# microsoft/M3P

Hardware: AMD Instinct MI355X
Metric: pre-train samples/sec (whole node), 12L/768d seq=128+36 (higher is better)
Workload: dtype bf16; 1 GPU; cfg2: 12L/768d/12h, 36 regions + 128 tokens, V=250002, 19 MLM targets/seq + ITM BCE, dropout 0.10, adam_inverse_sqrt + clip 5; per_gpu_batch=256, global_batch=256, seq_len=164, parallelism=dp1, prewarm_steps=36

## Files before the change

### include/m3p_hip.h

```cpp
#ifndef M3P_HIP_H
#define M3P_HIP_H

#include <stddef.h>
#include <stdint.h>

#ifdef __cplusplus
extern "C" {
#endif

#define M3P_API __attribute__((visibility("default")))

#define M3P_OK 0
#define M3P_EINVAL (-1)
#define M3P_ENOTIMPL (-2)
#define M3P_ENOMEM (-3)

M3P_API const char* m3p_version(void);


enum {
  M3P_EPI_NONE = 0,
  M3P_EPI_BIAS = 1,
  M3P_EPI_BIAS_GELU = 2,
  M3P_EPI_BIAS_DROP_RES = 3,
  M3P_EPI_RES = 4,
  M3P_EPI_DGELU = 5,
  M3P_EPI_MUL = 6,
  M3P_EPI_MULQ = 7,
  M3P_EPI_BIAS_GELUQ = 8,
  M3P_EPI_BIAS_LSE = 9
};

typedef struct M3PEpilogue {
  const float* bias;
  const void* aux;
  void* out2;
  float* colsum;
  int32_t ld_aux;
  int32_t ld_out2;
  int32_t scale_cols;
  float scale;
  float alpha;
  uint32_t seed;
  uint32_t thresh24;
  float inv_keep;
  const float* descale_a;
  const float* descale_b;
  void* out8;
  const float* scale8;
  float* amax8;
  int32_t ld_out8;
  int32_t out8_bf8;
  const int32_t* rng_rows;
  const void* row_ref;
} M3PEpilogue;

M3P_API int m3p_gemm_nt_bf16(const void* A, int lda, const void* W, int ldw, void* C, int ldc,
                             int M, int N, int K, int epilogue, const M3PEpilogue* ep, void* stream);

M3P_API int m3p_gemm_nt_fp8(const void* A8, int lda, int a_is_bf8, const void* W8, int ldw, void* C, int ldc,
                            int M, int N, int K, int epilogue, const M3PEpilogue* ep, void* stream);

M3P_API int m3p_quant_fp8(const void* src, int ld_src, void* dst, int ld_dst, int rows, int cols, const float* scale,
                          float* amax, int bf8, void* stream);

M3P_API int m3p_quant_fp8_batch(const long long* desc, int n_desc, int blocks_per_matrix, void* stream);

M3P_API int m3p_gemm_nt_streamk_f32(const void* A, int lda, const void* W, int ldw, float* C, int ldc,
                                    int M, int N, int K, float alpha, void* stream);
M3P_API int m3p_gemm_nn_streamk_f32(const void* A, int lda, const void* W, int ldw, int k_valid, float* C,
                                    int ldc, int M, int N, int K, float alpha, void* stream);
M3P_API int m3p_gemm_nn_w4_f32(const void* A, int lda, const void* W, int ldw, float* C, int ldc, int M, int N, int K, float alpha,
                               void* workspace, size_t workspace_bytes, void* stream);

M3P_API size_t m3p_gemm_wgrad_workspace_bytes(void);
M3P_API int m3p_gemm_wgrad_bf16(const void* dY, int lddy, const void* X, int ldx, float* dW, int lddw,
                                int M, int N, int K, float alpha, void* workspace, size_t workspace_bytes,
                                void* stream);
M3P_API int m3p_gemm_wgrad_store_bf16(const void* dY, int lddy, const void* X, int ldx, float* dW, int lddw, int M, int N, int K,
                                      float alpha, void* workspace, size_t workspace_bytes, void* stream);
M3P_API int m3p_gemm_wgrad_pair_bf16(const void* dYa, int lddya, const void* Xa, int ldxa, float* dWa, int lddwa, int Na, int Ka,
                                     const void* dYb, int lddyb, const void* Xb, int ldxb, float* dWb, int lddwb, int Nb, int Kb,
                                     int M, float alpha, void* workspace, size_t workspace_bytes, void* stream);


M3P_API int m3p_layernorm_fwd(const void* x, const float* gamma, const float* beta, const uint8_t* rowmask,
                              void* y, float* mean, float* rstd, int rows, int d, float eps, void* stream);

M3P_API int m3p_layernorm_bwd(const void* dy_a, const void* dy_b, const void* x, const float* gamma,
                              const float* mean, const float* rstd, const uint8_t* rowmask,
                              void* dx, void* dx_drop, float* dgamma, float* dbeta, float* dbias_drop,
                              int rows, int d, uint32_t seed, uint32_t thresh24, float inv_keep, void* stream);
M3P_API int m3p_layernorm_bwd_rows(const void* dy_a, const void* dy_b, const void* x, const float* gamma,
                                   const float* mean, const float* rstd, const uint8_t* rowmask,
                                   void* dx, void* dx_drop, float* dgamma, float* dbeta, float* dbias_drop,
                                   int rows, int d, uint32_t seed, uint32_t thresh24, float inv_keep,
                                   const int32_t* rng_rows, void* stream);


M3P_API int m3p_attn_fwd(const void* qkv, const int32_t* keylen, void* ctx, float* lse, uint64_t* keepmask,
                         int B, int S, int H, int dh, uint32_t seed, uint32_t thresh24, float inv_keep,
                         void* stream);

M3P_API int m3p_attn_bwd(const void* qkv, const int32_t* keylen, const void* ctx, const void* dctx,
                         const float* lse, const uint64_t* keepmask, void* dqkv, float* dbias_qkv, int B, int S,
                         int H, int dh, float qscale, uint32_t seed, uint32_t thresh24, float inv_keep,
                         void* stream);

M3P_API int m3p_attn_query_fwd(const void* q, int ld_q, const void* kv, long long kv_bstride, int ld_kv,
                               const int32_t* klen, void* ctx, int B, int Tq, int H, int dh, int Lk, int causal,
                               int pos0, void* stream);

M3P_API int m3p_attn_rows_fwd(const void* q, int ld_q, const void* kv, long long kv_bstride, int ld_kv, const int32_t* klen,
                              void* ctx, float* lse, int B, int Tq, int H, int dh, int Lk, int causal, int pos0,
                              uint32_t seed, uint32_t thresh24, float inv_keep, void* stream);
M3P_API int m3p_attn_rows_bwd(const void* q, int ld_q, const void* kv, long long kv_bstride, int ld_kv, const int32_t* klen,
                              const void* dctx, const float* lse, void* dq, int ld_dq, float* dkv, int B, int Tq, int H,
                              int dh, int Lk, int causal, int pos0, float qscale, uint32_t seed, uint32_t thresh24,
                              float inv_keep, void* stream);

M3P_API int m3p_attn_causal_fwd(const void* qkv, int ld_qkv, void* ctx, float* lse, int B, int T, int H, int dh,
                                uint32_t seed, uint32_t thresh24, float inv_keep, void* stream);
M3P_API int m3p_attn_causal_bwd(const void* qkv, int ld_qkv, const void* dctx, const float* lse, void* dqkv, int ld_dqkv,
                                int B, int T, int H, int dh, float qscale, uint32_t seed, uint32_t thresh24,
                                float inv_keep, void* stream);


M3P_API int m3p_cast_f32_bf16(const float* src, void* dst, long long n, void* stream);

M3P_API int m3p_embed_assemble_fwd(const int64_t* tok, const void* emb_bf16, const float* pos,
                                   const void* img_proj, const float* loc, const float* w_loc,
                                   const float* b_loc, const float* g_img, const float* be_img,
                                   const float* g_emb, const float* be_emb, const int32_t* totlen,
                                   void* h, void* z, float* mean_emb, float* rstd_emb, void* e,
                                   float* mean_img, float* rstd_img, int B, int T, int R, int d,
                                   uint32_t seed_img, uint32_t seed_emb, uint32_t thresh24, float inv_keep,
                                   const void* img_rows, void* stream);

M3P_API int m3p_embed_image_rows_fwd(const void* img_proj, const float* loc, const float* w_loc, const float* b_loc,
                                     const float* g_img, const float* be_img, void* e, float* mean_img,
                                     float* rstd_img, void* img_rows, int B, int R, int d, uint32_t seed_img,
                                     uint32_t thresh24, float inv_keep, void* stream);

M3P_API int m3p_embed_assemble_bwd(const void* dh, const void* z, const float* mean_emb, const float* rstd_emb,
                                   const float* g_emb, const void* e, const float* mean_img,
                                   const float* rstd_img, const float* g_img, const int64_t* tok,
                                   const int32_t* totlen, const float* loc, void* dz_scratch, void* de,
                                   float* d_g_emb, float* d_be_emb, float* d_pos, float* d_emb,
                                   void* d_tok_rows, float* d_g_img, float* d_be_img, float* d_b_img, float* d_b_loc,
                                   float* d_w_loc, int B, int T, int R, int d, int pad_index,
                                   uint32_t seed_img, uint32_t seed_emb, uint32_t thresh24, float inv_keep,
                                   int phase, void* stream);


M3P_API int m3p_gather_rows(const void* src, const int32_t* idx, void* dst, int n, int d, void* stream);
M3P_API int m3p_place_rows(const void* src, const int32_t* inv, void* dst, int rows, int d, int n, uint32_t fill_bits,
                           void* stream);
M3P_API int m3p_scatter_add_rows(const void* src, const int32_t* idx, void* dst, int n, int d, void* stream);
M3P_API int m3p_scatter_add_token_rows(const void* rows, int ld_rows, const int64_t* ids, float* dst, int n, int d,
                                       int pad_index, void* stream);

M3P_API int m3p_itm_score_fwd(const void* pre, const float* w2, const float* b2, float* pooled, float* scores, int B,
                              int d, void* stream);
M3P_API int m3p_itm_score_bwd(const float* dscores, const float* pooled, const float* w2, void* dpre16, void* dpreT16,
                              int ldt, float* db1, float* dw2, float* db2, int B, int d, void* stream);

M3P_API int m3p_ce_fwd_bwd(void* logits, int ld, int n_rows, int V, const int64_t* target, float* row_loss,
                           float* loss_sum, float loss_scale, float grad_scale, void* stream);

M3P_API int m3p_ce_lse_from_blocks(const void* stats, int n_blocks, int n_rows, const void* logits, int ld, const int64_t* target,
                                   float* row_loss, float* row_lse, void* scratch, void* stream);
M3P_API int m3p_ce_bwd_colsum(void* logits, int ld, int n_rows, int V, const int64_t* target, const float* row_lse,
                              float grad_scale, float* colsum, void* workspace, size_t workspace_bytes, void* stream);
M3P_API size_t m3p_ce_colsum_workspace_bytes(int ld, int n_rows);
M3P_API int m3p_ce_fwd_bwd_colsum(void* logits, int ld, int n_rows, int V, const int64_t* target, float* row_loss,
                                  float* row_lse, float grad_scale, float* colsum, void* workspace,
                                  size_t workspace_bytes, void* stream);

M3P_API int m3p_ce_shift_target(const void* h, const void* emb, const float* bias, const int64_t* target, float* row_t, void* row_ref,
                                int n_rows, int d, void* stream);
M3P_API int m3p_ce_shift_rows(const void* stats, int n_blocks, int n_rows, float grad_scale, float* row_loss, float* row_s,
                              float* row_q, void* scratch, void* stream);
M3P_API int m3p_ce_shift_colsum(const void* e, int ld, int n_rows, const float* row_s, float* colsum, void* workspace,
                                size_t workspace_bytes, void* stream);
M3P_API int m3p_ce_shift_scale_rows(const void* h, const float* row_s, const float* g, void* out, int n_rows, int d, void* stream);
M3P_API int m3p_ce_shift_target_rows(const void* h, const int64_t* target, const float* row_q, const float* g, float* demb, float* dbias,
                                     int n_rows, int d, void* stream);
M3P_API int m3p_ce_shift_dh(const float* dh32, const void* emb, const int64_t* target, const float* row_s, const float* row_q,
                            const float* g, void* dh, int n_rows, int d, void* stream);

M3P_API int m3p_ce_eval(const void* logits, int ld, int n_rows, int V, const int64_t* target, float* row_loss,
                        int32_t* row_argmax, void* stream);

M3P_API int m3p_colsum_bf16(const void* x, int ld, int n, int ncols, float* out, const float* scale_ptr,
                            void* stream);


M3P_API int m3p_sumsq_f32(const float* g, long long n, double* out, void* stream);

M3P_API int m3p_sumsq_ranges_f32(const float* base, const long long* starts, const long long* counts, int n_ranges, double* out,
                                 void* stream);

M3P_API int m3p_adam_step(float* p, float* g, float* m, float* v, void* w16, long long n, float lr, float beta1,
                          float beta2, float eps, float weight_decay, float step_size, const double* gnorm_sq,
                          float max_norm, float grad_scale, int zero_grad, void* stream);
M3P_API int m3p_adam_step_ranges(float* p, float* g, float* m, float* v, void* w16, const long long* starts,
                                 const long long* counts, const float* step_sizes, const int* zero_grad, int n_ranges,
                                 float lr, float beta1, float beta2, float eps, float weight_decay, const double* gnorm_sq,
                                 float max_norm, float grad_scale, void* stream);

M3P_API int m3p_gelu_fwd(const void* u, void* h, void* dh, long long n, void* stream);
M3P_API int m3p_gelu_fwd_gq(const void* u, void* h, void* gq, int M, int N, void* stream);
M3P_API int m3p_gelu_fwd_q8(const void* u, void* h, void* h8, long long n, const float* scale, float* amax, void* stream);

M3P_API int m3p_gelu_bwd(const void* dy, const void* u, void* du, long long n, void* stream);

M3P_API int m3p_mse_fwd_bwd(const void* pred, int ld_pred, const float* tgt, int ld_tgt, void* dpred, float* row_sq,
                            int rows, int cols, float grad_scale, void* stream);


M3P_API int m3p_dropout_rows(const void* x, int ldx, const void* res, int ldres, void* y, int ldy, int rows, int cols,
                             uint32_t rng_ld, uint32_t rng_col0, uint32_t seed, uint32_t thresh24, float inv_keep,
                             void* stream);

M3P_API int m3p_glu_fwd(const void* ab, int ld_ab, void* y, int rows, int d, void* stream);
M3P_API int m3p_glu_bwd(const void* ab, int ld_ab, const void* dy, void* dab, int rows, int d, void* stream);

M3P_API int m3p_transpose_batch_bf16(const long long* desc, int n_desc, int max_tiles, void* stream);

M3P_API int m3p_transpose_bf16(const void* src, void* dst, int rows, int cols, int ld_src, int ld_dst,
                               void* stream);

M3P_API int m3p_set_persistent_grid(int workgroups);
M3P_API int m3p_set_tile_queue(int32_t* counters, int n_slots);

enum {
  M3P_KERN_NT_SKINNY = 1,
  M3P_KERN_NT_W8 = 2,
  M3P_KERN_NT_W8_QUEUE = 3,
  M3P_KERN_NT_W4 = 4,
  M3P_KERN_NT_RING = 5,
  M3P_KERN_NT_128 = 6,
  M3P_KERN_WGRAD_W4_CHUNKS = 10,
  M3P_KERN_WGRAD_W4_TILES = 11,
  M3P_KERN_WGRAD_RING = 12,
  M3P_KERN_WGRAD_128 = 13
};
M3P_API int m3p_gemm_nt_plan(int M, int N, int K, int epilogue);
M3P_API int m3p_gemm_wgrad_plan(int M, int N, int K);

M3P_API void m3p_debug_set_variant(int v);
M3P_API void m3p_debug_attn_variant(int v);

M3P_API int m3p_seq_masks(const int64_t* lengths, const int64_t* lengths_b, int B, int S, int32_t* totlen,
                          uint8_t* rowmask, void* stream);
M3P_API int m3p_mask_to_rows(const uint8_t* mask, int n_mask, int inner, long long s0, long long s1, long long soff,
                             int d, int32_t* rows, int n_rows, void* stream);
M3P_API int m3p_cast_rows_f32_bf16(const float* in, long long s0, long long s1, int n0, int n1, int cols, void* out,
                                   void* stream);
M3P_API int m3p_scale_bf16_dev(const void* in, int in_is_f32, const float* g, void* out, long long n, void* stream);
M3P_API int m3p_axpy_dev_f32(float* dst, const float* src, const float* g, long long n, void* stream);
M3P_API int m3p_itm_loss_fwd_bwd(const float* scores, const int64_t* pos, int n_groups, int sample_n, float w_ce,
                                 float w_bce, float* loss, float* dscores, void* stream);

M3P_API int m3p_probe_mfma_16x16x32(const void* a_rowmajor_16x32, const void* b_colmajor_32x16,
                                    float* d_16x16, int* d_rowcol, void* stream);
M3P_API int m3p_probe_mfma_fp8_16x16x128(const void* a_16x128, const void* w_16x128, float* d_16x16, int a_is_bf8,
                                         void* stream);
M3P_API int m3p_probe_tr16(const void* tile_bf16_64x16, void* out_64x4, void* stream);
M3P_API int m3p_probe_permlane16_swap(void* out_2x64_u32, void* stream);

#ifdef __cplusplus
}
#endif
#endif
```

### m3p_amd/csrc/attention.hip

```cpp
#include "common.hpp"


namespace {

constexpr int ATTN_BWD_NW = 4;
constexpr int ATTN_BWD_WPS = 3;

static int g_attn_variant = 0;

template <int DH> struct AttnCfg {
  static constexpr int ROWB = DH * 2;
  static constexpr int CH = DH / 8;
  static constexpr int RPI = 1024 / ROWB;
  static constexpr int KK = DH / 32;
  static constexpr int NT = DH / 16;
  static __device__ __forceinline__ int swz(int chunk, int row) { return DH == 64 ? (chunk ^ (row & 7)) : chunk; }
};

__device__ __forceinline__ bf16x4 lds_tr16(const char* p) {
  s16x4 v = __builtin_amdgcn_ds_read_tr16_b64_v4i16((__attribute__((address_space(3))) s16x4*)(p));
  return __builtin_bit_cast(bf16x4, v);
}
__device__ __forceinline__ float row16_sum(float v) {
#define M3P_DPP_ADD(ctrl) v += __builtin_bit_cast(float, __builtin_amdgcn_update_dpp(0, __builtin_bit_cast(int, v), ctrl, 0xf, 0xf, true))
  M3P_DPP_ADD(0xB1);
  M3P_DPP_ADD(0x4E);
  M3P_DPP_ADD(0x124);
  M3P_DPP_ADD(0x128);
#undef M3P_DPP_ADD
  return v;
}
__device__ __forceinline__ uint32_t bit_to_mask(uint32_t bits, int r) {
  uint32_t o;
  switch (r) {
    case 0: asm("v_bfe_i32 %0, %1, 0, 1" : "=v"(o) : "v"(bits)); break;
    case 1: asm("v_bfe_i32 %0, %1, 1, 1" : "=v"(o) : "v"(bits)); break;
    case 2: asm("v_bfe_i32 %0, %1, 2, 1" : "=v"(o) : "v"(bits)); break;
    default: asm("v_bfe_i32 %0, %1, 3, 1" : "=v"(o) : "v"(bits)); break;
  }
  return o;
}
template <int CH>
__device__ __forceinline__ float chunks_sum(float v) {
#define M3P_DPP_ADD(ctrl) v += __builtin_bit_cast(float, __builtin_amdgcn_update_dpp(0, __builtin_bit_cast(int, v), ctrl, 0xf, 0xf, true))
  M3P_DPP_ADD(0xB1);
  M3P_DPP_ADD(0x4E);
  if (CH == 8) M3P_DPP_ADD(0x141);
#undef M3P_DPP_ADD
  return v;
}
__device__ __forceinline__ bf16x8 cat8(bf16x4 a, bf16x4 b) {
  return bf16x8{a[0], a[1], a[2], a[3], b[0], b[1], b[2], b[3]};
}

typedef unsigned int u32x2_t __attribute__((ext_vector_type(2)));
typedef unsigned int u32x4_t __attribute__((ext_vector_type(4)));
template <int NT>
__device__ __forceinline__ void store_row_widened(bf16* row, int fg, bool ok, const bf16x4 (&r)[NT]) {
  static_assert(NT % 2 == 0, "d-tiles are swapped in pairs");
  bf16* p = row + 8 * (fg >> 1) + 16 * (fg & 1);
#pragma unroll
  for (int n0 = 0; n0 < NT; n0 += 2) {
    u32x2_t x = __builtin_bit_cast(u32x2_t, r[n0]), y = __builtin_bit_cast(u32x2_t, r[n0 + 1]);
    asm volatile("s_nop 1\n\tv_permlane16_swap_b32 %0, %2\n\tv_permlane16_swap_b32 %1, %3"
                 : "+v"(x[0]), "+v"(x[1]), "+v"(y[0]), "+v"(y[1]));
    if (ok) *reinterpret_cast<u32x4_t*>(p + 16 * n0) = u32x4_t{x[0], x[1], y[0], y[1]};
  }
}

template <int DH>
__device__ __forceinline__ void stage_rows(const bf16* __restrict__ g, size_t ld, int S, int nrows, char* lds,
                                           int wid, int lane, int nwaves = 4) {
  using Cf = AttnCfg<DH>;
  const int rin = lane / Cf::CH, c = lane % Cf::CH;
  const int ninstr = (nrows + Cf::RPI - 1) / Cf::RPI;
  for (int i = wid; i < ninstr; i += nwaves) {
    const int row = i * Cf::RPI + rin;
    const int gr = min(row, S - 1);
    const int gc = Cf::swz(c, row);
    __builtin_amdgcn_global_load_lds(GLB_PTR(g + (size_t)gr * ld + gc * 8), LDS_PTR(lds + i * 1024), 16, 0, 0);
  }
}

template <int DH>
__device__ __forceinline__ void stage_rows_hidden(const bf16* __restrict__ g, size_t ld, int S, int nrows, char* lds,
                                                  int wid, int lane, int nwaves) {
  using Cf = AttnCfg<DH>;
  const int rin = lane / Cf::CH, c = lane % Cf::CH;
  const int ninstr = (nrows + Cf::RPI - 1) / Cf::RPI;
  const uint32_t lds0 = (uint32_t)(uintptr_t)(__attribute__((address_space(3))) char*)lds;
  for (int i = wid; i < ninstr; i += nwaves) {
    const int row = i * Cf::RPI + rin;
    const int gr = min(row, S - 1);
    const int gc = Cf::swz(c, row);
    const bf16* src = g + (size_t)gr * ld + gc * 8;
    const uint32_t dst = __builtin_amdgcn_readfirstlane(lds0 + (uint32_t)i * 1024u);
    asm volatile("s_mov_b32 m0, %1\n\ts_nop 0\n\tglobal_load_lds_dwordx4 %0, off" :: "v"(src), "s"(dst) : "memory", "m0");
  }
}

template <int DH, int KT, bool DROP, int NTC, int NW = 4, bool EVENS = false>
__global__ __launch_bounds__(NW * 64, NW == 8 ? 2 : 3)
void attn_fwd_kernel(const bf16* __restrict__ qkv, const int* __restrict__ keylen, bf16* __restrict__ ctx,
                     float* __restrict__ lse, unsigned long long* __restrict__ keepmask, int S, int H, int dmodel,
                     uint32_t seed, uint32_t thresh24, float inv_keep) {
  using Cf = AttnCfg<DH>;
  extern __shared__ __attribute__((aligned(16))) char smem[];
  const int tid = threadIdx.x, lane = tid & 63;
  const int wid = __builtin_amdgcn_readfirstlane(tid >> 6);
  const int b = blockIdx.x / H, h = blockIdx.x - b * H;
  const int nt = NTC ? NTC : (S + 15) >> 4;
  const int nk = (nt + 1) >> 1;
  const size_t ld = 3 * (size_t)dmodel;
  const bf16* Qg = qkv + (size_t)b * S * ld + h * DH;
  const bf16* Kg = Qg + dmodel;
  const bf16* Vg = Qg + 2 * dmodel;
  char* sK = smem;
  char* sV = smem + nt * 16 * Cf::ROWB;
  stage_rows<DH>(Kg, ld, S, nt * 16, sK, wid, lane, NW);
  stage_rows<DH>(Vg, ld, S, nk * 32, sV, wid, lane, NW);
  const int fq = lane & 15, fg = lane >> 4;
  const int wrot = (wid + (blockIdx.x >> 3)) & (NW - 1);
  bf16x8 qnext[Cf::KK];
  {
    const int qc0 = min(wrot * 16 + fq, S - 1);
#pragma unroll
    for (int kk = 0; kk < Cf::KK; ++kk)
      qnext[kk] = *reinterpret_cast<const bf16x8*>(Qg + (size_t)qc0 * ld + 32 * kk + 8 * fg);
  }
  const int klen = keylen[b];
  __syncthreads();

  int k_off[Cf::KK];
#pragma unroll
  for (int kk = 0; kk < Cf::KK; ++kk) k_off[kk] = fq * Cf::ROWB + Cf::swz(4 * kk + fg, fq) * 16;
  const int vrow = 4 * fg + (fq >> 2);
  int v_off[Cf::NT];
#pragma unroll
  for (int n = 0; n < Cf::NT; ++n)
    v_off[n] = vrow * Cf::ROWB + Cf::swz(2 * n + ((fq & 3) >> 1), vrow) * 16 + 8 * (fq & 1);

  for (int qb = wrot; qb < nt; qb += NW) {
    const int q = qb * 16 + fq;
    const int qc = min(q, S - 1);
    bf16x8 qf[Cf::KK];
#pragma unroll
    for (int kk = 0; kk < Cf::KK; ++kk) qf[kk] = qnext[kk];
    {
      const int qcn = min(q + 16 * NW, S - 1);
#pragma unroll
      for (int kk = 0; kk < Cf::KK; ++kk)
        qnext[kk] = *reinterpret_cast<const bf16x8*>(Qg + (size_t)qcn * ld + 32 * kk + 8 * fg);
    }

    f32x4 s[2 * KT];
#pragma unroll
    for (int t = 0; t < 2 * KT; ++t) s[t] = f32x4{0.f, 0.f, 0.f, 0.f};
#pragma unroll
    for (int kk = 0; kk < Cf::KK; ++kk) {
#pragma unroll
      for (int t = 0; t < 2 * KT; ++t)
        if (t < nt) {
          const bf16x8 kf = *reinterpret_cast<const bf16x8*>(sK + t * 16 * Cf::ROWB + k_off[kk]);
          s[t] = __builtin_amdgcn_mfma_f32_16x16x32_bf16(kf, qf[kk], s[t], 0, 0, 0);
        }
    }
    constexpr float kLog2e = 1.4426950408889634f;
    float mx = -INFINITY;
    int klen_it = klen;
    asm volatile("" : "+s"(klen_it));
#pragma unroll
    for (int t = 0; t < 2 * KT; ++t)
      if (t < nt) {
        if (16 * t + 16 > klen_it) {
#pragma unroll
          for (int r = 0; r < 4; ++r) s[t][r] = (16 * t + 4 * fg + r < klen_it) ? s[t][r] : -INFINITY;
        }
#pragma unroll
        for (int r = 0; r < 4; ++r) mx = fmaxf(mx, s[t][r]);
      }
    mx = fmaxf(mx, __shfl_xor(mx, 16, 64));
    mx = fmaxf(mx, __shfl_xor(mx, 32, 64));
    const float mx2 = mx * kLog2e;
    float sum = 0.f;
#pragma unroll
    for (int t = 0; t < 2 * KT; ++t)
      if (t < nt) {
#pragma unroll
        for (int r = 0; r < 4; ++r) {
          const float p = __builtin_amdgcn_exp2f(__builtin_fmaf(s[t][r], kLog2e, -mx2));
          s[t][r] = p;
          sum += p;
        }
      }
    sum += __shfl_xor(sum, 16, 64);
    sum += __shfl_xor(sum, 32, 64);
    const float inv = 1.0f / sum;
    const uint32_t rbase = (uint32_t)((b * H + h) * S + qc) * (uint32_t)S;
    const uint32_t thr16 = thresh24 >> 8;
    const bool even_rows = EVENS || (S & 1) == 0;
    unsigned long long* mrow = keepmask ? keepmask + ((size_t)(b * H + h) * nt + qb) * nt * 4 : nullptr;
    constexpr int MW = (8 * KT + 63) / 64;
    uint32_t mlo[MW], mhi[MW];
#pragma unroll
    for (int g = 0; g < MW; ++g) mlo[g] = mhi[g] = 0u;
    bf16x8 pf[KT];
#pragma unroll
    for (int kk = 0; kk < KT; ++kk) {
      float p[8];
      const float invk = DROP ? inv * inv_keep : inv;
      bool kq[8] = {true, true, true, true, true, true, true, true};
      if (DROP) {
#pragma unroll
        for (int hf = 0; hf < 2; ++hf) {
          const int t = 2 * kk + hf;
          if (t < nt) {
            const uint32_t base = rbase + (uint32_t)(16 * t + 4 * fg);
            bool k4[4];
            if (even_rows) {
              asm volatile("" ::: "memory");
              const uint32_t h0 = m3p_hash32(base >> 1, seed), h1 = m3p_hash32((base >> 1) + 1u, seed);
              k4[0] = (h0 & 0xFFFFu) >= thr16; k4[1] = (h0 >> 16) >= thr16;
              k4[2] = (h1 & 0xFFFFu) >= thr16; k4[3] = (h1 >> 16) >= thr16;
            } else {
              asm volatile("" ::: "memory");
              m3p_keep_run<4>(base, seed, thresh24, k4);
            }
#pragma unroll
            for (int r = 0; r < 4; ++r) kq[4 * hf + r] = k4[r];
          }
        }
      }
#pragma unroll
      for (int hf = 0; hf < 2; ++hf) {
        const int t = 2 * kk + hf;
        unsigned long long kw[4] = {0ull, 0ull, 0ull, 0ull};
#pragma unroll
        for (int r = 0; r < 4; ++r) {
          const int j = 4 * hf + r;
          float v = 0.f;
          if (t < nt) {
            v = s[t][r] * invk;
            if (DROP) {
              const bool keep = kq[j];
              kw[r] = __builtin_amdgcn_ballot_w64(keep);
              v = keep ? v : 0.f;
            }
          }
          p[j] = v;
        }
        if (DROP && t < nt) {
          asm("s_nop 3\n\tv_writelane_b32 %0, %2, %10\n\tv_writelane_b32 %1, %3, %10\n\tv_writelane_b32 %0, %4, %11\n\tv_writelane_b32 %1, %5, %11\n\t"
              "v_writelane_b32 %0, %6, %12\n\tv_writelane_b32 %1, %7, %12\n\tv_writelane_b32 %0, %8, %13\n\tv_writelane_b32 %1, %9, %13"
              : "+v"(mlo[(4 * t) >> 6]), "+v"(mhi[(4 * t) >> 6])
              : "s"((uint32_t)kw[0]), "s"((uint32_t)(kw[0] >> 32)), "s"((uint32_t)kw[1]), "s"((uint32_t)(kw[1] >> 32)),
                "s"((uint32_t)kw[2]), "s"((uint32_t)(kw[2] >> 32)), "s"((uint32_t)kw[3]), "s"((uint32_t)(kw[3] >> 32)),
                "i"((4 * t) & 63), "i"((4 * t + 1) & 63), "i"((4 * t + 2) & 63), "i"((4 * t + 3) & 63));
        }
      }
      pf[kk] = bf16x8{(bf16)p[0], (bf16)p[1], (bf16)p[2], (bf16)p[3], (bf16)p[4], (bf16)p[5], (bf16)p[6], (bf16)p[7]};
    }
    if (DROP && mrow) {
#pragma unroll
      for (int g = 0; g < MW; ++g)
        if (64 * g + lane < 4 * nt) mrow[64 * g + lane] = ((unsigned long long)mhi[g] << 32) | mlo[g];
    }
    f32x4 o[Cf::NT];
#pragma unroll
    for (int n = 0; n < Cf::NT; ++n) o[n] = f32x4{0.f, 0.f, 0.f, 0.f};
#pragma unroll
    for (int kk = 0; kk < KT; ++kk) {
      if (kk < nk) {
#pragma unroll
        for (int n = 0; n < Cf::NT; ++n) {
          const char* pv = sV + kk * 32 * Cf::ROWB + v_off[n];
          const bf16x8 vf = cat8(lds_tr16(pv), lds_tr16(pv + 16 * Cf::ROWB));
          o[n] = __builtin_amdgcn_mfma_f32_16x16x32_bf16(vf, pf[kk], o[n], 0, 0, 0);
        }
      }
    }
    {
      bf16x4 ob[Cf::NT];
#pragma unroll
      for (int n = 0; n < Cf::NT; ++n) ob[n] = bf16x4{(bf16)o[n][0], (bf16)o[n][1], (bf16)o[n][2], (bf16)o[n][3]};
      store_row_widened<Cf::NT>(ctx + (size_t)(b * S + min(q, S - 1)) * dmodel + h * DH, fg, q < S, ob);
      if (q < S && fg == 0) lse[(size_t)(b * H + h) * S + q] = mx + __logf(sum);
    }
  }
}

template <int DH, int KT, bool DROP, bool MASK, int NKC, int NTC, int NW = 4, int KB = 1, int KBQ = KB, bool ONEPASS = false>
__global__ __launch_bounds__(NW * 64, NTC == 11 ? ATTN_BWD_WPS : ((NW == 8 || KB == 2) ? 2 : 3))
void attn_bwd_kernel(const bf16* __restrict__ qkv, const int* __restrict__ keylen, const bf16* __restrict__ ctx,
                     const bf16* __restrict__ dctx, const float* __restrict__ lse,
                     const unsigned long long* __restrict__ keepmask, bf16* __restrict__ dqkv,
                     float* __restrict__ dbias_qkv, int S, int H, int dmodel, float qscale, uint32_t seed,
                     uint32_t thresh24, float inv_keep) {
  using Cf = AttnCfg<DH>;
  extern __shared__ __attribute__((aligned(16))) char smem[];
  const int tid = threadIdx.x, lane = tid & 63;
  const int wid = __builtin_amdgcn_readfirstlane(tid >> 6);
  const int b = blockIdx.x / H, h = blockIdx.x - b * H;
  const int wrot = (NW & (NW - 1)) ? wid : ((wid + (blockIdx.x >> 3)) & (NW - 1));
  const int nt = NTC ? NTC : ((S + 15) >> 4);
  const int nk = NKC ? NKC : ((S + 31) >> 5);
  const size_t ld = 3 * (size_t)dmodel;
  const int b_rd = b;
  const bf16* Qg = qkv + (size_t)b_rd * S * ld + h * DH;
  const bf16* Kg = Qg + dmodel;
  const bf16* Vg = Qg + 2 * dmodel;
  const bf16* Og = ctx + (size_t)b_rd * S * dmodel + h * DH;
  const bf16* dOg = dctx + (size_t)b_rd * S * dmodel + h * DH;
  bf16* dQg = dqkv + (size_t)b * S * ld + h * DH;
  bf16* dKg = dQg + dmodel;
  bf16* dVg = dQg + 2 * dmodel;
  const float* lse_bh = lse + (size_t)(b * H + h) * S;
  const int klen = keylen[b];
  const unsigned long long* mbh = MASK ? keepmask + (size_t)(b * H + h) * nt * nt * 4 : nullptr;

  const int tile_bytes = nk * 32 * Cf::ROWB;
  char* s0 = smem;
  char* s1 = smem + tile_bytes;
  float* sL = reinterpret_cast<float*>(smem + 2 * tile_bytes);
  float* sD = sL + nk * 32;
  const int fq = lane & 15, fg = lane >> 4;
  float* sB = sD + nk * 32;
  float* sBw = sB + wid * 3 * DH;
  constexpr int DSP = NTC * 32;
  char* sK = reinterpret_cast<char*>(sB + NW * 3 * DH);
  char* sDS = sK + tile_bytes;
  static_assert(!ONEPASS || (NKC == 6 && NTC == 11 && KB == 1 && DH == 64), "ONEPASS is the M3P-sequence instantiation");
  f32x4 bsum[Cf::NT];
#pragma unroll
  for (int n = 0; n < Cf::NT; ++n) bsum[n] = f32x4{0.f, 0.f, 0.f, 0.f};
  auto bias_acc = [&](int, int n, const bf16x4& v4) {
    bsum[n] += f32x4{(float)v4[0], (float)v4[1], (float)v4[2], (float)v4[3]};
  };
  auto bias_flush = [&](int part) {
#pragma unroll
    for (int n = 0; n < Cf::NT; ++n) {
      f32x4 x = bsum[n];
#pragma unroll
      for (int r = 0; r < 4; ++r) x[r] = row16_sum(x[r]);
      if (fq == 0) *reinterpret_cast<f32x4*>(sBw + part * DH + 16 * n + 4 * fg) = x;
      bsum[n] = f32x4{0.f, 0.f, 0.f, 0.f};
    }
  };

  int r_off[Cf::KK];
#pragma unroll
  for (int kk = 0; kk < Cf::KK; ++kk) r_off[kk] = fq * Cf::ROWB + Cf::swz(4 * kk + fg, fq) * 16;
  const int trow = 4 * fg + (fq >> 2);
  int t_off[Cf::NT];
#pragma unroll
  for (int n = 0; n < Cf::NT; ++n)
    t_off[n] = trow * Cf::ROWB + Cf::swz(2 * n + ((fq & 3) >> 1), trow) * 16 + 8 * (fq & 1);

#define PAD_TILE(t) (NTC ? (t) >= NTC : (!MASK && (t) >= nt))
  constexpr float kLog2e = 1.4426950408889634f;
  constexpr float kMasked = -1.0e30f;
  constexpr bool kDfromLds = NKC != 0;
  constexpr int kStageInstr = NKC * 32 / Cf::RPI;
  constexpr int kNIW = kDfromLds ? (kStageInstr + NW - 1) / NW : 1;
  bf16x8 orow[kNIW];
  if (kDfromLds) {
    const int rin = lane / Cf::CH, c = lane % Cf::CH;
#pragma unroll
    for (int j = 0; j < kNIW; ++j) {
      const int row = (wid + j * NW) * Cf::RPI + rin;
      orow[j] = *reinterpret_cast<const bf16x8*>(Og + (size_t)min(row, S - 1) * dmodel + Cf::swz(c, row) * 8);
    }
  }
  stage_rows<DH>(Qg, ld, S, nk * 32, s0, wid, lane, NW);
  stage_rows<DH>(dOg, (size_t)dmodel, S, nk * 32, s1, wid, lane, NW);
  if (ONEPASS) stage_rows<DH>(Kg, ld, S, nk * 32, sK, wid, lane, NW);
  bf16x8 kf[KB][Cf::KK], vf[KB][Cf::KK];
  auto load_kv = [&](int u, int kb) {
    const int keyc = min(kb * 16 + fq, S - 1);
#pragma unroll
    for (int kk = 0; kk < Cf::KK; ++kk) {
      kf[u][kk] = *reinterpret_cast<const bf16x8*>(Kg + (size_t)keyc * ld + 32 * kk + 8 * fg);
      vf[u][kk] = *reinterpret_cast<const bf16x8*>(Vg + (size_t)keyc * ld + 32 * kk + 8 * fg);
    }
  };
  constexpr bool kNextFrag = NKC != 0 && NTC != 0 && !(DROP && !MASK);
  bf16x8 kfn[KB][Cf::KK], vfn[KB][Cf::KK];
  auto load_kv_next = [&](int u, int kb) {
    const int keyc = min(kb * 16 + fq, S - 1);
#pragma unroll
    for (int kk = 0; kk < Cf::KK; ++kk) {
      kfn[u][kk] = *reinterpret_cast<const bf16x8*>(Kg + (size_t)keyc * ld + 32 * kk + 8 * fg);
      vfn[u][kk] = *reinterpret_cast<const bf16x8*>(Vg + (size_t)keyc * ld + 32 * kk + 8 * fg);
    }
  };
  if (wrot * KB < nt) {
#pragma unroll
    for (int u = 0; u < KB; ++u) load_kv(u, wrot * KB + u);
  }
  const float log2_inv_keep = DROP ? __builtin_amdgcn_logf(inv_keep) : 0.f;
  const float keep_prob = DROP ? __builtin_amdgcn_rcpf(inv_keep) : 1.f;
  for (int q = tid; q < nk * 32; q += NW * 64) {
    float dsum = 0.f, l = INFINITY;
    if (q < S) {
      if (!kDfromLds) {
        const bf16* op = Og + (size_t)q * dmodel;
        const bf16* dp = dOg + (size_t)q * dmodel;
#pragma unroll
        for (int c = 0; c < DH / 8; ++c) {
          const bf16x8 ov = *reinterpret_cast<const bf16x8*>(op + 8 * c);
          const bf16x8 dv = *reinterpret_cast<const bf16x8*>(dp + 8 * c);
#pragma unroll
          for (int e = 0; e < 8; ++e) dsum += (float)ov[e] * (float)dv[e];
        }
      }
      l = lse_bh[q] * kLog2e - log2_inv_keep;
    }
    if (!kDfromLds) sD[q] = dsum * keep_prob;
    sL[q] = l;
  }
  if (kDfromLds) {
    asm volatile("s_waitcnt vmcnt(0)" ::: "memory");
    const int rin = lane / Cf::CH, c = lane % Cf::CH;
#pragma unroll
    for (int j = 0; j < kNIW; ++j) {
      const int i = wid + j * NW;
      if (i < kStageInstr) {
        const bf16x8 dv = *reinterpret_cast<const bf16x8*>(s1 + i * 1024 + lane * 16);
        float part = 0.f;
#pragma unroll
        for (int e = 0; e < 8; ++e) part += (float)orow[j][e] * (float)dv[e];
        part = chunks_sum<Cf::CH>(part);
        const int row = i * Cf::RPI + rin;
        if (c == 0) sD[row] = row < S ? part * keep_prob : 0.f;
      }
    }
  }
  __syncthreads();

  constexpr bool kPreA = MASK && NKC != 0;
// ... 489 lines not shown
  for (;;) {
    const int b = hd / H, h = hd - b * H;
    bf16* dQg = dqkv + (size_t)b * S * ld + h * DH;
    const bf16* Kg = qkv + (size_t)b * S * ld + h * DH + dmodel;
    const int klen = keylen[b];
    float* sBh = sB + par * (NW * 3 * DH);
    __builtin_amdgcn_s_waitcnt(0x0F70);
    asm volatile("s_waitcnt vmcnt(0)" ::: "memory");
#pragma unroll
    for (int j = 0; j < kNIW; ++j) {
      const int i = wid + j * NW;
      if (i < kStageInstr) {
        const bf16x8 dvv = *reinterpret_cast<const bf16x8*>(s1 + i * 1024 + lane * 16);
        float part = 0.f;
#pragma unroll
        for (int e = 0; e < 8; ++e) part += (float)orow[j][e] * (float)dvv[e];
        part = chunks_sum<Cf::CH>(part);
        const int row = i * Cf::RPI + rin;
        if (c8 == 0) sD[row] = row < S ? part * keep_prob : 0.f;
      }
    }
    if (tid < NR) sL[tid] = tid < S ? lse_r * kLog2e - log2_inv_keep : INFINITY;
    if (MASK && lane < 4 * NTC) sMW[lane] = mw_req;
    asm volatile("s_waitcnt lgkmcnt(0)" ::: "memory");
    __builtin_amdgcn_s_barrier();
    asm volatile("" ::: "memory");
    if (prev_h >= 0 && dbias_qkv) bias_reduce(sB + (par ^ 1) * (NW * 3 * DH), prev_h);
    if (prev_h >= 0) store_head(dQg_prev);
    dQg_prev = dQg;
    stage_rows_hidden<DH>(Kg, ld, S, NR, sK, wid, lane, NW);
    if (wid < NTC) {
      const float kbias = (key < klen) ? 0.f : kMasked;
      f32x4 dv[Cf::NT], dk[Cf::NT];
#pragma unroll
      for (int n = 0; n < Cf::NT; ++n) dv[n] = dk[n] = f32x4{0.f, 0.f, 0.f, 0.f};
#pragma unroll
      for (int kq = 0; kq < NKC; ++kq) {
        f32x4 scA[2], dpA[2], dnegA[2];
#pragma unroll
        for (int hf = 0; hf < 2; ++hf) {
          const int t = 2 * kq + hf;
          dnegA[hf] = f32x4{-sD[16 * t + 4 * fg + 0], -sD[16 * t + 4 * fg + 1], -sD[16 * t + 4 * fg + 2], -sD[16 * t + 4 * fg + 3]};
          scA[hf] = f32x4{kbias, kbias, kbias, kbias};
          dpA[hf] = DROP ? f32x4{0.f, 0.f, 0.f, 0.f} : dnegA[hf];
        }
#pragma unroll
        for (int kk = 0; kk < Cf::KK; ++kk) {
#pragma unroll
          for (int hf = 0; hf < 2; ++hf) {
            const int t = 2 * kq + hf;
            if (PAD_TILE(t)) continue;
            const bf16x8 qf = *reinterpret_cast<const bf16x8*>(s0 + t * 16 * Cf::ROWB + r_off[kk]);
            const bf16x8 df = *reinterpret_cast<const bf16x8*>(s1 + t * 16 * Cf::ROWB + r_off[kk]);
            scA[hf] = __builtin_amdgcn_mfma_f32_16x16x32_bf16(qf, kf[kk], scA[hf], 0, 0, 0);
            dpA[hf] = __builtin_amdgcn_mfma_f32_16x16x32_bf16(df, vf[kk], dpA[hf], 0, 0, 0);
          }
        }
        f32x4 pd2[2], ds2[2];
#pragma unroll
        for (int hf = 0; hf < 2; ++hf) {
          const int t = 2 * kq + hf;
          if (PAD_TILE(t)) {
            pd2[hf] = ds2[hf] = f32x4{0.f, 0.f, 0.f, 0.f};
            continue;
          }
          uint32_t kbits = 0;
          if (MASK) kbits = (uint32_t)(sMW[4 * t + (fq & 3)] >> (4 * fg + 16 * (fq >> 2)));
#pragma unroll
          for (int r = 0; r < 4; ++r) {
            const int q = 16 * t + 4 * fg + r;
            const float p = __builtin_amdgcn_exp2f(__builtin_fmaf(scA[hf][r], kLog2e, -sL[q]));
            if (DROP) {
              const float pd = __builtin_bit_cast(float, __builtin_bit_cast(uint32_t, p) & bit_to_mask(kbits, r));
              pd2[hf][r] = pd;
              ds2[hf][r] = __builtin_fmaf(pd, dpA[hf][r], p * dnegA[hf][r]);
            } else {
              pd2[hf][r] = p;
              ds2[hf][r] = p * dpA[hf][r];
            }
          }
        }
        const bf16x8 pfrag = bf16x8{(bf16)pd2[0][0], (bf16)pd2[0][1], (bf16)pd2[0][2], (bf16)pd2[0][3],
                                    (bf16)pd2[1][0], (bf16)pd2[1][1], (bf16)pd2[1][2], (bf16)pd2[1][3]};
        const bf16x8 sfrag = bf16x8{(bf16)ds2[0][0], (bf16)ds2[0][1], (bf16)ds2[0][2], (bf16)ds2[0][3],
                                    (bf16)ds2[1][0], (bf16)ds2[1][1], (bf16)ds2[1][2], (bf16)ds2[1][3]};
#pragma unroll
        for (int hf = 0; hf < 2; ++hf) {
          if (PAD_TILE(2 * kq + hf)) continue;
          *reinterpret_cast<bf16x4*>(sDS + key * DSP + (32 * kq + 16 * hf + 4 * fg) * 2) =
              hf ? bf16x4{sfrag[4], sfrag[5], sfrag[6], sfrag[7]} : bf16x4{sfrag[0], sfrag[1], sfrag[2], sfrag[3]};
        }
#pragma unroll
        for (int n = 0; n < Cf::NT; ++n) {
          const char* pq = s0 + kq * 32 * Cf::ROWB + t_off[n];
          const char* pdo = s1 + kq * 32 * Cf::ROWB + t_off[n];
          const bf16x8 qT = cat8(lds_tr16(pq), lds_tr16(pq + 16 * Cf::ROWB));
          const bf16x8 dT = cat8(lds_tr16(pdo), lds_tr16(pdo + 16 * Cf::ROWB));
          dv[n] = __builtin_amdgcn_mfma_f32_16x16x32_bf16(dT, pfrag, dv[n], 0, 0, 0);
          dk[n] = __builtin_amdgcn_mfma_f32_16x16x32_bf16(qT, sfrag, dk[n], 0, 0, 0);
        }
        __builtin_amdgcn_sched_barrier(0);
      }
#pragma unroll
      for (int n = 0; n < Cf::NT; ++n) {
        kb4[n] = bf16x4{(bf16)dk[n][0], (bf16)dk[n][1], (bf16)dk[n][2], (bf16)dk[n][3]};
        vb4[n] = bf16x4{(bf16)dv[n][0], (bf16)dv[n][1], (bf16)dv[n][2], (bf16)dv[n][3]};
        if (dbias_qkv) bias_acc(n, key < S ? vb4[n] : bf16x4{0, 0, 0, 0});
      }
    }
    if (dbias_qkv) bias_flush(sBh + wid * 3 * DH, 2);
    __builtin_amdgcn_s_waitcnt(0);
    asm volatile("s_waitcnt vmcnt(0) lgkmcnt(0)" ::: "memory");
    __builtin_amdgcn_s_barrier();
    asm volatile("" ::: "memory");
    const int next = hd + gridDim.x;
    if (next < nheads) request_head(next);
    if (wid < NTC) {
      f32x4 dq[Cf::NT];
#pragma unroll
      for (int n = 0; n < Cf::NT; ++n) dq[n] = f32x4{0.f, 0.f, 0.f, 0.f};
      const char* pds = sDS + trow * DSP + wid * 32 + (fq & 3) * 8;
#pragma unroll
      for (int kq = 0; kq < NKC; ++kq) {
        const bf16x4 lo = lds_tr16(pds + (32 * kq) * DSP);
        const bf16x4 hi = PAD_TILE(2 * kq + 1) ? bf16x4{0, 0, 0, 0} : lds_tr16(pds + (32 * kq + 16) * DSP);
        const bf16x8 sfr = cat8(lo, hi);
#pragma unroll
        for (int n = 0; n < Cf::NT; ++n) {
          const char* pk = sK + kq * 32 * Cf::ROWB + t_off[n];
          const bf16x8 kT = cat8(lds_tr16(pk), lds_tr16(pk + 16 * Cf::ROWB));
          dq[n] = __builtin_amdgcn_mfma_f32_16x16x32_bf16(kT, sfr, dq[n], 0, 0, 0);
        }
      }
#pragma unroll
      for (int n = 0; n < Cf::NT; ++n) {
        qb4[n] = bf16x4{(bf16)(dq[n][0] * qscale), (bf16)(dq[n][1] * qscale), (bf16)(dq[n][2] * qscale), (bf16)(dq[n][3] * qscale)};
        if (dbias_qkv) bias_acc(n, key < S ? qb4[n] : bf16x4{0, 0, 0, 0});
      }
    }
    if (dbias_qkv) bias_flush(sBh + wid * 3 * DH, 0);
    prev_h = h;
    par ^= 1;
    if (next >= nheads) break;
    hd = next;
  }
  store_head(dQg_prev);
  if (dbias_qkv) {
    __syncthreads();
    bias_reduce(sB + (par ^ 1) * (NW * 3 * DH), prev_h);
  }
#undef PAD_TILE
}

template <int DH>
int launch_fwd(const bf16* qkv, const int* keylen, bf16* ctx, float* lse, unsigned long long* keepmask, int B, int S, int H,
               int dmodel, uint32_t seed, uint32_t thresh24, float inv_keep, hipStream_t st) {
  const int nt = (S + 15) / 16, nk = (S + 31) / 32;
  const size_t lds = (size_t)(nt * 16 + nk * 32) * DH * 2;
  const bool wide = 2 * lds > 160 * 1024;
#define M3P_ATTN_FWD(KT)                                                                                        \
  do {                                                                                                          \
    constexpr int NW0 = (KT == 16) ? 8 : 4;    \
    auto kern = thresh24 ? attn_fwd_kernel<DH, KT, true, 0, NW0> : attn_fwd_kernel<DH, KT, false, 0, NW0>;       \
    if (nt == 11 && KT == 6) kern = thresh24 ? ((S & 1) ? attn_fwd_kernel<DH, 6, true, 11> : attn_fwd_kernel<DH, 6, true, 11, 4, true>) \
                                             : attn_fwd_kernel<DH, 6, false, 11>; \
    if (wide) kern = thresh24 ? attn_fwd_kernel<DH, KT, true, 0, 8> : attn_fwd_kernel<DH, KT, false, 0, 8>;       \
    hipError_t e = hipFuncSetAttribute((const void*)kern, hipFuncAttributeMaxDynamicSharedMemorySize, (int)lds); \
    if (e != hipSuccess) return (int)e;                                                                         \
    hipLaunchKernelGGL(kern, dim3(B* H), dim3((wide || NW0 == 8) ? 512 : 256), lds, st, qkv, keylen, ctx, lse, keepmask, S, H, dmodel, seed, \
                       thresh24, inv_keep);                                                                     \
  } while (0)
  if (nk <= 6) M3P_ATTN_FWD(6);
  else if (nk <= 12) M3P_ATTN_FWD(12);
  else if (nk <= 16) M3P_ATTN_FWD(16);
  else return M3P_EINVAL;
#undef M3P_ATTN_FWD
  M3P_CHECK_LAUNCH();
  return M3P_OK;
}

template <int DH>
int launch_bwd(const bf16* qkv, const int* keylen, const bf16* ctx, const bf16* dctx, const float* lse,
               const unsigned long long* keepmask, bf16* dqkv, float* dbias, int B, int S, int H, int dmodel, float qscale,
               uint32_t seed, uint32_t thresh24, float inv_keep, hipStream_t st) {
  const int nk = (S + 31) / 32;
  const bool wide = (size_t)2 * ((size_t)2 * nk * 32 * DH * 2) > 160 * 1024;
  const bool m3p_seq = nk == 6 && (S + 15) / 16 == 11;
  const bool onepass = m3p_seq && DH == 64 && (!thresh24 || keepmask) && !(g_attn_variant & 1);
  const int nwaves = wide ? 8 : (onepass ? 12 : (m3p_seq ? ATTN_BWD_NW : 4));
  const size_t lds = (size_t)2 * nk * 32 * DH * 2 + (size_t)2 * nk * 32 * sizeof(float) + 3 * nwaves * DH * sizeof(float) +
                     (onepass ? (size_t)nk * 32 * DH * 2 + (size_t)11 * 16 * 11 * 32 : 0);
#define M3P_ATTN_BWD(KT, DROP, MASK)                                                                            \
  do {                                                                                                          \
    auto kern = attn_bwd_kernel<DH, KT, DROP, MASK, 0, 0>;                                                      \
    if (wide) kern = attn_bwd_kernel<DH, KT, DROP, MASK, 0, 0, 8>;                                              \
    if (nk == 6) kern = attn_bwd_kernel<DH, KT, DROP, MASK, 6, 0>;                                              \
    if (m3p_seq) kern = attn_bwd_kernel<DH, KT, DROP, MASK, 6, 11, ATTN_BWD_NW, 1, 1>;                                \
    if constexpr (DH == 64 && (MASK || !DROP)) { if (onepass) kern = attn_bwd_kernel<DH, KT, DROP, MASK, 6, 11, 12, 1, 1, true>; } \
    hipError_t e = hipFuncSetAttribute((const void*)kern, hipFuncAttributeMaxDynamicSharedMemorySize, (int)lds); \
    if (e != hipSuccess) return (int)e;                                                                         \
    hipLaunchKernelGGL(kern, dim3(B* H), dim3(nwaves * 64), lds, st, qkv, keylen, ctx, dctx, lse, keepmask, dqkv, dbias, S, H, \
                       dmodel, qscale, seed, thresh24, inv_keep);                                               \
  } while (0)
  if (nk > 16) return M3P_EINVAL;
  if constexpr (DH == 64) {
    if (onepass && !(g_attn_variant & 2)) {
      int dev = 0, n_cu = 0;
      if (hipGetDevice(&dev) != hipSuccess || hipDeviceGetAttribute(&n_cu, hipDeviceAttributeMultiprocessorCount, dev) != hipSuccess || n_cu <= 0)
        n_cu = 256;
      const size_t ldsp = (size_t)3 * 192 * 128 + (size_t)11 * 16 * 11 * 32 + 2 * 192 * sizeof(float) + 2 * 12 * 3 * 64 * sizeof(float) + 12 * 48 * 8;
      auto kp = thresh24 ? attn_bwd_p_kernel<true, true> : attn_bwd_p_kernel<false, false>;
      if (hipFuncSetAttribute((const void*)kp, hipFuncAttributeMaxDynamicSharedMemorySize, (int)ldsp) == hipSuccess) {
        const int nheads = B * H;
        hipLaunchKernelGGL(kp, dim3(nheads < n_cu ? nheads : n_cu), dim3(768), ldsp, st, qkv, keylen, ctx, dctx, lse, keepmask, dqkv, dbias,
                           S, H, dmodel, nheads, qscale, inv_keep);
        M3P_CHECK_LAUNCH();
        return M3P_OK;
      }
      (void)hipGetLastError();
    }
  }
  if (!thresh24) M3P_ATTN_BWD(16, false, false);
  else M3P_ATTN_BWD(16, true, true);
#undef M3P_ATTN_BWD
  M3P_CHECK_LAUNCH();
  return M3P_OK;
}

}

extern "C" {

void m3p_debug_attn_variant(int v) { g_attn_variant = v; }

int m3p_attn_fwd(const void* qkv, const int32_t* keylen, void* ctx, float* lse, uint64_t* keepmask, int B, int S, int H, int dh,
                 uint32_t seed, uint32_t thresh24, float inv_keep, void* stream) {
  if (B <= 0 || S <= 0 || H <= 0 || S > 512) return M3P_EINVAL;
  if (((uintptr_t)qkv & 15) || ((uintptr_t)ctx & 7)) return M3P_EINVAL;
  const int dmodel = H * dh;
  hipStream_t st = (hipStream_t)stream;
  if (dh == 64) return launch_fwd<64>((const bf16*)qkv, keylen, (bf16*)ctx, lse, (unsigned long long*)keepmask, B, S, H, dmodel, seed, thresh24, inv_keep, st);
  if (dh == 32) return launch_fwd<32>((const bf16*)qkv, keylen, (bf16*)ctx, lse, (unsigned long long*)keepmask, B, S, H, dmodel, seed, thresh24, inv_keep, st);
  return M3P_EINVAL;
}

int m3p_attn_bwd(const void* qkv, const int32_t* keylen, const void* ctx, const void* dctx, const float* lse,
                 const uint64_t* keepmask, void* dqkv, float* dbias_qkv, int B, int S, int H, int dh, float qscale,
                 uint32_t seed, uint32_t thresh24, float inv_keep, void* stream) {
  if (B <= 0 || S <= 0 || H <= 0 || S > 512) return M3P_EINVAL;
  if (thresh24 && !keepmask) return M3P_EINVAL;
  if (((uintptr_t)qkv & 15) || ((uintptr_t)ctx & 15) || ((uintptr_t)dctx & 15) || ((uintptr_t)dqkv & 7)) return M3P_EINVAL;
  const int dmodel = H * dh;
  hipStream_t st = (hipStream_t)stream;
  if (dh == 64)
    return launch_bwd<64>((const bf16*)qkv, keylen, (const bf16*)ctx, (const bf16*)dctx, lse, (const unsigned long long*)keepmask, (bf16*)dqkv, dbias_qkv, B, S, H,
                          dmodel, qscale, seed, thresh24, inv_keep, st);
  if (dh == 32)
    return launch_bwd<32>((const bf16*)qkv, keylen, (const bf16*)ctx, (const bf16*)dctx, lse, (const unsigned long long*)keepmask, (bf16*)dqkv, dbias_qkv, B, S, H,
                          dmodel, qscale, seed, thresh24, inv_keep, st);
  return M3P_EINVAL;
}

}
```

### m3p_amd/csrc/heads.hip

```cpp
#include "common.hpp"
#include <hip/amd_detail/amd_hip_unsafe_atomics.h>

namespace {

__global__ __launch_bounds__(256) void gather_rows_kernel(const bf16* __restrict__ src, const int32_t* __restrict__ idx,
                                                          bf16* __restrict__ dst, int n, int d) {
  const int nchunk = d >> 2;
  const size_t total = (size_t)n * nchunk;
  for (size_t i = (size_t)blockIdx.x * blockDim.x + threadIdx.x; i < total; i += (size_t)gridDim.x * blockDim.x) {
    const int r = (int)(i / nchunk), c = (int)(i - (size_t)r * nchunk);
    *reinterpret_cast<bf16x4*>(dst + (size_t)r * d + 4 * c) =
        *reinterpret_cast<const bf16x4*>(src + (size_t)idx[r] * d + 4 * c);
  }
}
__global__ __launch_bounds__(256) void place_rows_kernel(const bf16* __restrict__ src, const int32_t* __restrict__ inv,
                                                         bf16* __restrict__ dst, int rows, int d, int n, uint32_t fill2) {
  typedef unsigned int u32x4 __attribute__((ext_vector_type(4)));
  const int nchunk = d >> 3;
  const size_t total = (size_t)rows * nchunk;
  const u32x4 fv = u32x4{fill2, fill2, fill2, fill2};
  for (size_t i = (size_t)blockIdx.x * blockDim.x + threadIdx.x; i < total; i += (size_t)gridDim.x * blockDim.x) {
    const int r = (int)(i / nchunk), c = (int)(i - (size_t)r * nchunk);
    const int j = inv[r];
    u32x4 v = fv;
    if (j >= 0 && j < n) v = *reinterpret_cast<const u32x4*>(src + (size_t)j * d + 8 * c);
    *reinterpret_cast<u32x4*>(dst + (size_t)r * d + 8 * c) = v;
  }
}
__global__ __launch_bounds__(256) void scatter_add_rows_kernel(const bf16* __restrict__ src, const int32_t* __restrict__ idx,
                                                               bf16* __restrict__ dst, int n, int d) {
  const int nchunk = d >> 2;
  const size_t total = (size_t)n * nchunk;
  for (size_t i = (size_t)blockIdx.x * blockDim.x + threadIdx.x; i < total; i += (size_t)gridDim.x * blockDim.x) {
    const int r = (int)(i / nchunk), c = (int)(i - (size_t)r * nchunk);
    bf16* p = dst + (size_t)idx[r] * d + 4 * c;
    Vec4<bf16>::store(p, Vec4<bf16>::load(p) + Vec4<bf16>::load(src + (size_t)r * d + 4 * c));
  }
}

__global__ __launch_bounds__(256) void scatter_add_token_rows_kernel(const bf16* __restrict__ rows, int ld_rows, const int64_t* __restrict__ ids,
                                                                     float* __restrict__ dst, int n, int d, int pad_index) {
  const int lane = threadIdx.x & 63;
  const int wave = (int)((blockIdx.x * blockDim.x + threadIdx.x) >> 6), nwave = (int)((gridDim.x * blockDim.x) >> 6);
  for (int r = wave; r < n; r += nwave) {
    const int64_t id = ids[r];
    if (id == pad_index) continue;
    const bf16* src = rows + (size_t)r * ld_rows;
    float* out = dst + (size_t)id * d;
    for (int e = lane; e < d; e += 64) {
      const float v = (float)src[e];
      if (v != 0.f) unsafeAtomicAdd(out + e, v);
    }
  }
}

__global__ __launch_bounds__(1024) void ce_fwd_bwd_kernel(bf16* __restrict__ logits, int ld, int V,
                                                          const int64_t* __restrict__ target, float* __restrict__ row_loss,
                                                          float* __restrict__ loss_sum, float loss_scale, float gscale) {
  __shared__ float s_m[16], s_s[16];
  constexpr float kLog2e = 1.4426950408889634f;
  const int row = blockIdx.x, tid = threadIdx.x, lane = tid & 63, wib = tid >> 6;
  bf16* lr = logits + (size_t)row * ld;
  const int nchunk = ld >> 3;
  float m = -INFINITY, s = 0.f;
  for (int c = tid; c < nchunk; c += 1024) {
    const bf16x8 v = *reinterpret_cast<const bf16x8*>(lr + 8 * c);
    float x[8];
    float gm = -INFINITY;
#pragma unroll
    for (int j = 0; j < 8; ++j) {
      x[j] = (8 * c + j < V) ? (float)v[j] : -INFINITY;
      gm = fmaxf(gm, x[j]);
    }
    if (gm > m) {
      s *= __builtin_amdgcn_exp2f((m - gm) * kLog2e);
      m = gm;
    }
    const float mb = m * kLog2e;
#pragma unroll
    for (int j = 0; j < 8; ++j) s += __builtin_amdgcn_exp2f(__builtin_fmaf(x[j], kLog2e, -mb));
  }
#pragma unroll
  for (int o = 32; o > 0; o >>= 1) {
    const float m2 = __shfl_xor(m, o, 64), s2 = __shfl_xor(s, o, 64);
    const float mm = fmaxf(m, m2);
    s = (m == -INFINITY ? 0.f : s * __expf(m - mm)) + (m2 == -INFINITY ? 0.f : s2 * __expf(m2 - mm));
    m = mm;
  }
  if (lane == 0) { s_m[wib] = m; s_s[wib] = s; }
  __syncthreads();
  float M = -INFINITY;
#pragma unroll
  for (int w = 0; w < 16; ++w) M = fmaxf(M, s_m[w]);
  float Ssum = 0.f;
#pragma unroll
  for (int w = 0; w < 16; ++w) Ssum += (s_m[w] == -INFINITY) ? 0.f : s_s[w] * __expf(s_m[w] - M);
  const float lse = M + __logf(Ssum);
  const int64_t tgt = target[row];
  if (tid == 0) {
    const float l = lse - (float)lr[tgt];
    row_loss[row] = l;
    if (loss_sum) unsafeAtomicAdd(loss_sum, l * loss_scale);
  }
  __syncthreads();
  const float lb = lse * kLog2e;
  for (int c = tid; c < nchunk; c += 1024) {
    const bf16x8 v = *reinterpret_cast<const bf16x8*>(lr + 8 * c);
    bf16x8 g;
#pragma unroll
    for (int j = 0; j < 8; ++j) {
      const int col = 8 * c + j;
      float p = (col < V) ? __builtin_amdgcn_exp2f(__builtin_fmaf((float)v[j], kLog2e, -lb)) : 0.f;
      if (col == tgt) p -= 1.f;
      g[j] = (bf16)(p * gscale);
    }
    *reinterpret_cast<bf16x8*>(lr + 8 * c) = g;
  }
}

__global__ __launch_bounds__(1024) void ce_stats_kernel(const bf16* __restrict__ logits, int ld, int V, const int64_t* __restrict__ target,
                                                        float* __restrict__ row_loss, float* __restrict__ row_lse) {
  __shared__ float s_m[16], s_s[16];
  constexpr float kLog2e = 1.4426950408889634f;
  const int row = blockIdx.x, tid = threadIdx.x, lane = tid & 63, wib = tid >> 6;
  const bf16* lr = logits + (size_t)row * ld;
  const int nchunk = ld >> 3;
  float m = -INFINITY, s = 0.f;
  for (int c = tid; c < nchunk; c += 1024) {
    const bf16x8 v = *reinterpret_cast<const bf16x8*>(lr + 8 * c);
    float x[8];
    float gm = -INFINITY;
#pragma unroll
    for (int j = 0; j < 8; ++j) {
      x[j] = (8 * c + j < V) ? (float)v[j] : -INFINITY;
      gm = fmaxf(gm, x[j]);
    }
    if (gm > m) {
      s *= __builtin_amdgcn_exp2f((m - gm) * kLog2e);
      m = gm;
    }
    const float mb = m * kLog2e;
#pragma unroll
    for (int j = 0; j < 8; ++j) s += __builtin_amdgcn_exp2f(__builtin_fmaf(x[j], kLog2e, -mb));
  }
#pragma unroll
  for (int o = 32; o > 0; o >>= 1) {
    const float m2 = __shfl_xor(m, o, 64), s2 = __shfl_xor(s, o, 64);
    const float mm = fmaxf(m, m2);
    s = (m == -INFINITY ? 0.f : s * __expf(m - mm)) + (m2 == -INFINITY ? 0.f : s2 * __expf(m2 - mm));
    m = mm;
  }
  if (lane == 0) { s_m[wib] = m; s_s[wib] = s; }
  __syncthreads();
  if (tid == 0) {
    float M = -INFINITY;
    for (int w = 0; w < 16; ++w) M = fmaxf(M, s_m[w]);
    float Ssum = 0.f;
    for (int w = 0; w < 16; ++w) Ssum += (s_m[w] == -INFINITY) ? 0.f : s_s[w] * __expf(s_m[w] - M);
    const float lse = M + __logf(Ssum);
    row_lse[row] = lse;
    row_loss[row] = lse - (float)lr[target[row]];
  }
}

constexpr int CE_RB = 64, CE_CB = 2048;
constexpr int CE_LSE_SPLIT = 32;
__device__ __forceinline__ void lse_fold(float& m, float& s, float m2, float s2) {
  const float mm = fmaxf(m, m2);
  const float a = (m == -INFINITY) ? 0.f : s * __expf(m - mm);
  const float b = (m2 == -INFINITY) ? 0.f : s2 * __expf(m2 - mm);
  m = mm;
  s = a + b;
}
constexpr int CE_NO_COL = 0x7fffffff;
__device__ __forceinline__ void argmax_fold(float m, int& i, float m2, int i2) {
  if (m2 > m || (m2 == m && i2 < i)) i = i2;
}
__global__ __launch_bounds__(1024) void ce_eval_kernel(const bf16* __restrict__ logits, int ld, int V, const int64_t* __restrict__ target,
                                                       float* __restrict__ row_loss, int32_t* __restrict__ row_argmax) {
// ... 289 lines not shown
  }
}

}

extern "C" {

int m3p_ce_shift_target(const void* h, const void* emb, const float* bias, const int64_t* target, float* row_t, void* row_ref,
                        int n_rows, int d, void* stream) {
  if (n_rows <= 0 || d <= 0 || (d % 4) != 0 || !h || !emb || !bias || !target || !row_t || !row_ref || ((uintptr_t)h & 7) ||
      ((uintptr_t)emb & 7) || ((uintptr_t)row_ref & 7))
    return M3P_EINVAL;
  hipLaunchKernelGGL(ce_shift_target_kernel, dim3((n_rows + 3) / 4), dim3(256), 0, (hipStream_t)stream, (const bf16*)h, (const bf16*)emb,
                     bias, target, row_t, (CeRowRef*)row_ref, n_rows, d);
  M3P_CHECK_LAUNCH();
  return M3P_OK;
}

int m3p_ce_shift_rows(const void* stats, int n_blocks, int n_rows, float grad_scale, float* row_loss, float* row_s, float* row_q,
                      void* scratch, void* stream) {
  if (n_blocks <= 0 || n_rows <= 0 || (n_rows % 64) != 0 || !stats || !row_loss || !row_s || !row_q || !scratch)
    return M3P_EINVAL;
  hipStream_t st = (hipStream_t)stream;
  hipLaunchKernelGGL(ce_shift_partial_kernel, dim3(n_rows / 64, CE_LSE_SPLIT), dim3(256), 0, st, (const float*)stats, n_blocks, n_rows,
                     (float*)scratch);
  hipLaunchKernelGGL(ce_shift_final_kernel, dim3((n_rows + 255) / 256), dim3(256), 0, st, (const float*)scratch, n_rows, grad_scale,
                     row_loss, row_s, row_q);
  M3P_CHECK_LAUNCH();
  return M3P_OK;
}

int m3p_ce_shift_colsum(const void* e, int ld, int n_rows, const float* row_s, float* colsum, void* workspace, size_t workspace_bytes,
                        void* stream) {
  if (n_rows <= 0 || ld <= 0 || (ld % 8) != 0 || !e || !row_s || !colsum || !workspace || ((uintptr_t)e & 15) ||
      ((uintptr_t)colsum & 15) || ((uintptr_t)workspace & 15))
    return M3P_EINVAL;
  if (workspace_bytes < m3p_ce_colsum_workspace_bytes(ld, n_rows)) return M3P_EINVAL;
  hipStream_t st = (hipStream_t)stream;
  const int groups = (n_rows + CE_RB - 1) / CE_RB;
  hipLaunchKernelGGL(ce_shift_colsum_tile_kernel, dim3((ld + CE_CB - 1) / CE_CB, groups), dim3(256), 0, st, (const bf16*)e, ld, n_rows,
                     row_s, (float*)workspace);
  if (hipMemsetAsync(colsum, 0, (size_t)ld * sizeof(float), st) != hipSuccess) return M3P_EINVAL;
  hipLaunchKernelGGL(ce_colsum_reduce_kernel, dim3((ld / 4 + 255) / 256, groups >= 16 ? 8 : 1), dim3(256), 0, st,
                     (const float*)workspace, ld, groups, colsum);
  M3P_CHECK_LAUNCH();
  return M3P_OK;
}

static int ce_shift_blocks(size_t total) { return (int)((total + 255) / 256 < 2048 ? (total + 255) / 256 : 2048); }

int m3p_ce_shift_scale_rows(const void* h, const float* row_s, const float* g, void* out, int n_rows, int d, void* stream) {
  if (n_rows <= 0 || d <= 0 || (d % 4) != 0 || !h || !row_s || !g || !out || ((uintptr_t)h & 7) || ((uintptr_t)out & 7)) return M3P_EINVAL;
  hipLaunchKernelGGL(ce_shift_scale_rows_kernel, dim3(ce_shift_blocks((size_t)n_rows * (d / 4))), dim3(256), 0, (hipStream_t)stream,
                     (const bf16*)h, row_s, g, (bf16*)out, n_rows, d);
  M3P_CHECK_LAUNCH();
  return M3P_OK;
}

int m3p_ce_shift_target_rows(const void* h, const int64_t* target, const float* row_q, const float* g, float* demb, float* dbias,
                             int n_rows, int d, void* stream) {
  if (n_rows <= 0 || d <= 0 || !h || !target || !row_q || !g || !demb || !dbias) return M3P_EINVAL;
  const int blocks = (n_rows + 3) / 4 < 4096 ? (n_rows + 3) / 4 : 4096;
  hipLaunchKernelGGL(ce_shift_target_rows_kernel, dim3(blocks), dim3(256), 0, (hipStream_t)stream, (const bf16*)h, target, row_q, g, demb,
                     dbias, n_rows, d);
  M3P_CHECK_LAUNCH();
  return M3P_OK;
}

int m3p_ce_shift_dh(const float* dh32, const void* emb, const int64_t* target, const float* row_s, const float* row_q, const float* g,
                    void* dh, int n_rows, int d, void* stream) {
  if (n_rows <= 0 || d <= 0 || (d % 4) != 0 || !dh32 || !emb || !target || !row_s || !row_q || !g || !dh || ((uintptr_t)dh32 & 15) ||
      ((uintptr_t)emb & 7) || ((uintptr_t)dh & 7))
    return M3P_EINVAL;
  hipLaunchKernelGGL(ce_shift_dh_kernel, dim3(ce_shift_blocks((size_t)n_rows * (d / 4))), dim3(256), 0, (hipStream_t)stream, dh32,
                     (const bf16*)emb, target, row_s, row_q, g, (bf16*)dh, n_rows, d);
  M3P_CHECK_LAUNCH();
  return M3P_OK;
}

size_t m3p_ce_colsum_workspace_bytes(int ld, int n_rows) {
  return (size_t)((n_rows + CE_RB - 1) / CE_RB) * (size_t)ld * sizeof(float);
}

int m3p_ce_fwd_bwd_colsum(void* logits, int ld, int n_rows, int V, const int64_t* target, float* row_loss, float* row_lse,
                          float grad_scale, float* colsum, void* workspace, size_t workspace_bytes, void* stream) {
  if (n_rows <= 0 || V <= 0 || ld < V || (ld % 8) != 0 || ((uintptr_t)logits & 15) || ((uintptr_t)colsum & 15) ||
      ((uintptr_t)workspace & 15))
    return M3P_EINVAL;
  if (workspace_bytes < m3p_ce_colsum_workspace_bytes(ld, n_rows)) return M3P_EINVAL;
  hipLaunchKernelGGL(ce_stats_kernel, dim3(n_rows), dim3(1024), 0, (hipStream_t)stream, (const bf16*)logits, ld, V, target, row_loss, row_lse);
  return m3p_ce_bwd_colsum(logits, ld, n_rows, V, target, row_lse, grad_scale, colsum, workspace, workspace_bytes, stream);
}

int m3p_ce_lse_from_blocks(const void* stats, int n_blocks, int n_rows, const void* logits, int ld, const int64_t* target,
                           float* row_loss, float* row_lse, void* scratch, void* stream) {
  if (n_blocks <= 0 || n_rows <= 0 || (n_rows % 64) != 0 || !stats || !logits || !target || !row_loss || !row_lse || !scratch ||
      ((uintptr_t)stats & 7) || ((uintptr_t)scratch & 7))
    return M3P_EINVAL;
  hipStream_t st = (hipStream_t)stream;
  hipLaunchKernelGGL(ce_lse_partial_kernel, dim3(n_rows / 64, CE_LSE_SPLIT), dim3(256), 0, st, (const float2*)stats, n_blocks, n_rows,
                     (float2*)scratch);
  hipLaunchKernelGGL(ce_lse_final_kernel, dim3((n_rows + 255) / 256), dim3(256), 0, st, (const float2*)scratch, n_rows,
                     (const bf16*)logits, ld, target, row_loss, row_lse);
  M3P_CHECK_LAUNCH();
  return M3P_OK;
}

int m3p_ce_bwd_colsum(void* logits, int ld, int n_rows, int V, const int64_t* target, const float* row_lse,
                      float grad_scale, float* colsum, void* workspace, size_t workspace_bytes, void* stream) {
  if (n_rows <= 0 || V <= 0 || ld < V || (ld % 8) != 0 || ((uintptr_t)logits & 15) || ((uintptr_t)colsum & 15) ||
      ((uintptr_t)workspace & 15) || !row_lse)
    return M3P_EINVAL;
  if (workspace_bytes < m3p_ce_colsum_workspace_bytes(ld, n_rows)) return M3P_EINVAL;
  hipStream_t st = (hipStream_t)stream;
  const int groups = (n_rows + CE_RB - 1) / CE_RB;
  hipLaunchKernelGGL(ce_grad_tile_kernel, dim3((ld + CE_CB - 1) / CE_CB, groups), dim3(256), 0, st, (bf16*)logits, ld, n_rows, V,
                     target, (const float*)row_lse, grad_scale, (float*)workspace);
  if (hipMemsetAsync(colsum, 0, (size_t)ld * sizeof(float), st) != hipSuccess) return M3P_EINVAL;
  hipLaunchKernelGGL(ce_colsum_reduce_kernel, dim3((ld / 4 + 255) / 256, groups >= 16 ? 8 : 1), dim3(256), 0, st,
                     (const float*)workspace, ld, groups, colsum);
  M3P_CHECK_LAUNCH();
  return M3P_OK;
}

int m3p_colsum_bf16(const void* x, int ld, int n, int ncols, float* out, const float* scale_ptr, void* stream) {
  if (n <= 0 || ncols <= 0 || (ld % 4) != 0 || ld < ((ncols + 3) / 4) * 4) return M3P_EINVAL;
  const int c4 = (ncols + 3) / 4;
  int ysplit = 1;
  while (ysplit < 64 && ((c4 + 255) / 256) * ysplit < 1024 && n / (ysplit * 2) >= 16) ysplit *= 2;
  hipLaunchKernelGGL(colsum_kernel, dim3((c4 + 255) / 256, ysplit), dim3(256), 0, (hipStream_t)stream, (const bf16*)x, ld,
                     n, ncols, out, scale_ptr);
  M3P_CHECK_LAUNCH();
  return M3P_OK;
}

int m3p_gather_rows(const void* src, const int32_t* idx, void* dst, int n, int d, void* stream) {
  if (n <= 0) return M3P_OK;
  if ((d % 4) != 0) return M3P_EINVAL;
  const size_t total = (size_t)n * (d / 4);
  const int blocks = (int)((total + 255) / 256 < 2048 ? (total + 255) / 256 : 2048);
  hipLaunchKernelGGL(gather_rows_kernel, dim3(blocks), dim3(256), 0, (hipStream_t)stream, (const bf16*)src, idx, (bf16*)dst, n, d);
  M3P_CHECK_LAUNCH();
  return M3P_OK;
}

int m3p_place_rows(const void* src, const int32_t* inv, void* dst, int rows, int d, int n, uint32_t fill_bits, void* stream) {
  if (rows <= 0) return M3P_OK;
  if (d <= 0 || (d % 8) != 0 || n < 0 || !inv || !dst || (n > 0 && !src) || ((uintptr_t)src & 15) || ((uintptr_t)dst & 15))
    return M3P_EINVAL;
  const size_t total = (size_t)rows * (d / 8);
  const int blocks = (int)((total + 255) / 256 < 8192 ? (total + 255) / 256 : 8192);
  const uint32_t f = fill_bits & 0xFFFFu;
  hipLaunchKernelGGL(place_rows_kernel, dim3(blocks), dim3(256), 0, (hipStream_t)stream, (const bf16*)src, inv, (bf16*)dst, rows, d, n,
                     f | (f << 16));
  M3P_CHECK_LAUNCH();
  return M3P_OK;
}

int m3p_scatter_add_rows(const void* src, const int32_t* idx, void* dst, int n, int d, void* stream) {
  if (n <= 0) return M3P_OK;
  if ((d % 4) != 0) return M3P_EINVAL;
  const size_t total = (size_t)n * (d / 4);
  const int blocks = (int)((total + 255) / 256 < 2048 ? (total + 255) / 256 : 2048);
  hipLaunchKernelGGL(scatter_add_rows_kernel, dim3(blocks), dim3(256), 0, (hipStream_t)stream, (const bf16*)src, idx, (bf16*)dst, n, d);
  M3P_CHECK_LAUNCH();
  return M3P_OK;
}

int m3p_scatter_add_token_rows(const void* rows, int ld_rows, const int64_t* ids, float* dst, int n, int d, int pad_index, void* stream) {
  if (n <= 0) return M3P_OK;
  if (d <= 0 || ld_rows < d) return M3P_EINVAL;
  const int blocks = (n + 3) / 4 < 4096 ? (n + 3) / 4 : 4096;
  hipLaunchKernelGGL(scatter_add_token_rows_kernel, dim3(blocks), dim3(256), 0, (hipStream_t)stream, (const bf16*)rows, ld_rows, ids,
                     dst, n, d, pad_index);
  M3P_CHECK_LAUNCH();
  return M3P_OK;
}

int m3p_ce_fwd_bwd(void* logits, int ld, int n_rows, int V, const int64_t* target, float* row_loss, float* loss_sum,
                   float loss_scale, float grad_scale, void* stream) {
  if (n_rows <= 0 || V <= 0 || ld < V || (ld % 8) != 0 || ((uintptr_t)logits & 15)) return M3P_EINVAL;
  hipLaunchKernelGGL(ce_fwd_bwd_kernel, dim3(n_rows), dim3(1024), 0, (hipStream_t)stream, (bf16*)logits, ld, V, target,
                     row_loss, loss_sum, loss_scale, grad_scale);
  M3P_CHECK_LAUNCH();
  return M3P_OK;
}

int m3p_ce_eval(const void* logits, int ld, int n_rows, int V, const int64_t* target, float* row_loss, int32_t* row_argmax, void* stream) {
  if (n_rows <= 0 || V <= 0 || ld < V || (ld % 8) != 0 || !logits || ((uintptr_t)logits & 15) || !target || !row_loss || !row_argmax)
    return M3P_EINVAL;
  hipLaunchKernelGGL(ce_eval_kernel, dim3(n_rows), dim3(1024), 0, (hipStream_t)stream, (const bf16*)logits, ld, V, target, row_loss,
                     row_argmax);
  M3P_CHECK_LAUNCH();
  return M3P_OK;
}

}
```

### m3p_amd/functional.py

```python
import math
import os
from collections import OrderedDict

import torch

from . import lib as L
from . import fp8 as fp8mod
from . import ops
from . import rng

BF16 = torch.bfloat16
ALIGN = 64
BUCKET_ALIGN = 64 * 8


def _round_up(n, a):
    return (n + a - 1) // a * a


_VOCAB_FULL_TILES = os.environ.get('M3P_VOCAB_FULL_TILES', '1') != '0'
_GELU_GRAD_IN_FWD = os.environ.get('M3P_GELU_GRAD_IN_FWD', '0') != '0'
_GELU_BYTE_GRAD = int(os.environ.get('M3P_GELU_BYTE_GRAD', '2'))
_CE_FUSED_LSE = os.environ.get('M3P_CE_FUSED_LSE', '1') != '0'
_VOCAB_DGRAD_W4 = os.environ.get('M3P_VOCAB_DGRAD_W4', '1') != '0'
# ... 250 lines not shown

class ArenaCrossWeights:

    def __init__(self, ar):
        n = ar.model.n_layers
        self.q = [ar.xattn(i, 'q') for i in range(n)]
        self.kv = [ar.xattn(i, 'kv') for i in range(n)]
        self.out = [ar.w('encoder_attn.%d.out_lin.weight' % i) for i in range(n)]
        self.bq = [ar.xattn(i, 'bq') for i in range(n)]
        self.bkv = [ar.xattn(i, 'bkv') for i in range(n)]
        self.bo = [ar.p('encoder_attn.%d.out_lin.bias' % i) for i in range(n)]


_REF_SITE0 = 1 << 20


def _transposed(w):
    wt = torch.empty((w.shape[1], w.shape[0]), dtype=BF16, device=w.device)
    ops.transpose_bf16(w, wt)
    return wt


def refiner_fwd(model, x, keylen, B, R, seed_step, p):
    ar = model.arena()
    d, H = model.dim, model.n_heads
    dh = d // H
    M = B * R
    qscale = 1.0 / math.sqrt(dh)
    seed = lambda i, k: rng.stream_seed(model.base_seed, seed_step, _REF_SITE0 + 8 * i + k)
    layers = []
    for i in range(model.n_refine_layers):
        pre = 'refine_embeddings.layers.%d.' % i
        xn, mean_a, rstd_a = ops.layernorm_fwd(x, ar.p(pre + 'sublayer.0.norm.weight'), ar.p(pre + 'sublayer.0.norm.bias'))
        qkv = ops.gemm_nt(xn, ar.ref_qkv_w16(i), L.EPI_BIAS, bias=ar.ref_qkv_bias(i), scale_cols=d, scale=qscale)
        ctxt, lse, kmask = ops.attn_fwd(qkv, keylen, B, R, H, dh, seed=seed(i, 0), p_drop=p, want_mask=True)
        cat = torch.empty((M, 2 * d), dtype=BF16, device=x.device)
        ops.dropout_rows(ctxt, p, seed(i, 1), out=cat[:, :d], rng_ld=2 * d, rng_col0=0)
        ops.dropout_rows(xn, p, seed(i, 1), out=cat[:, d:], rng_ld=2 * d, rng_col0=d)
        ab = ops.gemm_nt(cat, ar.w(pre + 'self_attn.aoa_layer.0.weight'), L.EPI_BIAS,
                         bias=ar.p(pre + 'self_attn.aoa_layer.0.bias'))
        x1 = ops.dropout_rows(ops.glu_fwd(ab), p, seed(i, 2), res=x)
        xn2, mean_b, rstd_b = ops.layernorm_fwd(x1, ar.p(pre + 'sublayer.1.norm.weight'), ar.p(pre + 'sublayer.1.norm.bias'))
        u = torch.empty((M, 4 * d), dtype=BF16, device=x.device)
        hact = ops.gemm_nt(xn2, ar.w(pre + 'feed_forward.lin1.weight'), L.EPI_BIAS_GELU,
                           bias=ar.p(pre + 'feed_forward.lin1.bias'), out2=u)
        t = ops.gemm_nt(hact, ar.w(pre + 'feed_forward.lin2.weight'), L.EPI_BIAS, bias=ar.p(pre + 'feed_forward.lin2.bias'))
        if p > 0:
            ops.dropout_rows(t, p, seed(i, 3), out=t)
        x2 = ops.dropout_rows(t, p, seed(i, 4), res=x1)
        layers.append((x, mean_a, rstd_a, xn, qkv, ctxt, lse, kmask, cat, ab, x1, mean_b, rstd_b, xn2, u, hact))
        x = x2
    out, mean_f, rstd_f = ops.layernorm_fwd(x, ar.p('refine_embeddings.norm.weight'), ar.p('refine_embeddings.norm.bias'))
    return out, (layers, x, mean_f, rstd_f)


def refiner_bwd(model, dout, saved, keylen, B, R, seed_step, p):
    ar = model.arena()
    d, H = model.dim, model.n_heads
    dh = d // H
    seed = lambda i, k: rng.stream_seed(model.base_seed, seed_step, _REF_SITE0 + 8 * i + k)
    layers, x_last, mean_f, rstd_f = saved
    dx, _ = ops.layernorm_bwd(dout, None, x_last, ar.p('refine_embeddings.norm.weight'), mean_f, rstd_f, None,
                              ar.g('refine_embeddings.norm.weight'), ar.g('refine_embeddings.norm.bias'))
    for i in reversed(range(model.n_refine_layers)):
        pre = 'refine_embeddings.layers.%d.' % i
        (x, mean_a, rstd_a, xn, qkv, ctxt, lse, kmask, cat, ab, x1, mean_b, rstd_b, xn2, u, hact) = layers[i]
        layers[i] = None
        dt = ops.dropout_rows(dx, p, seed(i, 4))
        if p > 0:
            ops.dropout_rows(dt, p, seed(i, 3), out=dt)
        ops.colsum(dt, d, ar.g(pre + 'feed_forward.lin2.bias'))
        ops.gemm_wgrad(dt, hact, ar.g(pre + 'feed_forward.lin2.weight'))
        du = ops.gemm_nt(dt, _transposed(ar.w(pre + 'feed_forward.lin2.weight')), L.EPI_DGELU, aux=u,
                         colsum=ar.g(pre + 'feed_forward.lin1.bias'))
        ops.gemm_wgrad(du, xn2, ar.g(pre + 'feed_forward.lin1.weight'))
        dxn2 = ops.gemm_nt(du, _transposed(ar.w(pre + 'feed_forward.lin1.weight')), L.EPI_NONE)
        dln, _ = ops.layernorm_bwd(dxn2, None, x1, ar.p(pre + 'sublayer.1.norm.weight'), mean_b, rstd_b, None,
                                   ar.g(pre + 'sublayer.1.norm.weight'), ar.g(pre + 'sublayer.1.norm.bias'))
        dx1 = ops.dropout_rows(dln, 0.0, 0, res=dx)
        del dt, du, dxn2, dln, u, hact, xn2
        dy = ops.dropout_rows(dx1, p, seed(i, 2))
        dab = ops.glu_bwd(ab, dy)
        ops.colsum(dab, 2 * d, ar.g(pre + 'self_attn.aoa_layer.0.bias'))
        ops.gemm_wgrad(dab, cat, ar.g(pre + 'self_attn.aoa_layer.0.weight'))
        dcat = ops.gemm_nt(dab, _transposed(ar.w(pre + 'self_attn.aoa_layer.0.weight')), L.EPI_NONE)
        dctx = ops.dropout_rows(dcat[:, :d], p, seed(i, 1), rng_ld=2 * d, rng_col0=0)
        dxn_cat = ops.dropout_rows(dcat[:, d:], p, seed(i, 1), rng_ld=2 * d, rng_col0=d)
        dqkv = ops.attn_bwd(qkv, keylen, ctxt, dctx, lse, B, R, H, dh, dbias_qkv=ar.ref_qkv_bias(i, grad=True),
                            seed=seed(i, 0), p_drop=p, keepmask=kmask)
        ops.gemm_wgrad(dqkv, xn, ar.ref_qkv_wgrad(i))
        dxn = ops.gemm_nt(dqkv, _transposed(ar.ref_qkv_w16(i)), L.EPI_RES, aux=dxn_cat)
        dln, _ = ops.layernorm_bwd(dxn, None, x, ar.p(pre + 'sublayer.0.norm.weight'), mean_a, rstd_a, None,
                                   ar.g(pre + 'sublayer.0.norm.weight'), ar.g(pre + 'sublayer.0.norm.bias'))
        dx = ops.dropout_rows(dln, 0.0, 0, res=dx1)
        del dy, dab, dcat, dctx, dxn_cat, dqkv, dxn, dln, dx1
    ar.touch(*[n for n in ar.names if n.startswith('refine_embeddings.')])
    return dx


class GradSink:

    def __init__(self):
        self.buf = None

    def rows(self, like):
        if self.buf is None:
            self.buf = torch.zeros_like(like)
        assert self.buf.shape == like.shape
        return self.buf

    def take(self):
        buf, self.buf = self.buf, None
        return buf


def _sink_of(tensor, base):
    root = tensor._base if tensor._is_view() else tensor
    sink = getattr(root, '_m3p_sink', None) if root is not None else None
    if sink is None or base is None or not torch.is_grad_enabled():
        return None
    if root.dim() != 2 or not root.is_contiguous() or root.storage_offset() != 0 or tuple(root.shape) != tuple(base.shape):
        return None
    return sink


def first_rows_sink(model, tensor):
    d = model.dim
    if tensor.dim() != 3 or tensor.dtype != BF16 or not tensor._is_view():
        return None, None, None
    st, soff = tensor.stride(), tensor.storage_offset()
    if st[2] != 1 or st[0] % d or soff % d:
        return None, None, None
    with torch.no_grad():
        base = torch.as_strided(tensor, (tensor.untyped_storage().nbytes() // 2 // d, d), (d, 1), 0)
    sink = _sink_of(tensor, base)
    if sink is None:
        return None, None, None
    cache = model.__dict__.setdefault('_first_rows_cache', {})
    key = (tensor.shape[0], st[0], soff, tensor.device)
    rows = cache.get(key)
    if rows is None:
        rows = ((soff + torch.arange(tensor.shape[0], device=tensor.device, dtype=torch.int64) * st[0]) // d).to(torch.int32)
        cache.clear()
        cache[key] = rows
    return sink, base, rows


N_ENC_ARGS = 17

ROW_TILE = 256
COMPACT_MIN_ROWS = 4096


def compact_rows_eligible(n_rows, M):
    if n_rows <= 0:
        return 0
    n = _round_up(n_rows, ROW_TILE)
    return n if (n >= COMPACT_MIN_ROWS and 2 * n <= M) else 0


class OutputRows:

    def __init__(self, flags):
        flags = torch.as_tensor(flags).reshape(-1).cpu()
        if flags.dtype != torch.bool:
            flags = flags != 0
        self.flags = flags
        self.M = int(flags.numel())
        sel = torch.nonzero(flags).view(-1)
        self.n_rows = int(sel.numel())
        self.n = compact_rows_eligible(self.n_rows, self.M)
        self.idx = self.idx64 = self.inv = None
        if self.n:
            pad = torch.nonzero(~flags).view(-1)[:self.n - self.n_rows]
            idx = torch.cat([sel, pad]).to(torch.int32)
            inv = torch.full((self.M,), -1, dtype=torch.int32)
            inv[sel] = torch.arange(self.n_rows, dtype=torch.int32)
            self._host = (idx, inv)

    @classmethod
    def from_masks(cls, B, S, R, first=True, pred_mask=None, region_labels=None):
        flags = torch.zeros((B, S), dtype=torch.bool)
        if first:
            flags[:, 0] = True
        if pred_mask is not None:
            flags[:, R:] |= torch.as_tensor(pred_mask).cpu().reshape(S - R, B).t() != 0
        if region_labels is not None and R > 0:
            flags[:, :R] |= torch.as_tensor(region_labels).cpu().reshape(B, R) != -1
        return cls(flags)

    def to(self, device):
        if self.n and self.idx is None:
            from .utils import to_cuda
            with torch.cuda.device(device):
                self.idx, self.inv = to_cuda(*self._host)
            self.idx64 = self.idx.long()
        assert self.idx is None or self.idx.device == torch.device(device), 'an OutputRows serves one pass on one device'
        return self


class EncoderFn(torch.autograd.Function):

    @staticmethod
    def forward(ctx, anchor, model, x, lengths, x_img, lengths_img, image_loc, p_drop, p_attn, seed_step, p_refine=None,
                track=False, text_embed=None, langs=None, h0=None, positions=None, out_rows=None):
        ar = model.arena()
        ready = model.ddp_hook.params_ready if model.ddp_hook is not None else (lambda key: None)
        ar.refresh(wait_params=False)
        ready('vocab')
        ready('embed')
        dev = ar.device
        d, H, nL = model.dim, model.n_heads, model.n_layers
        dh = d // H
        seed = lambda kind, i=0: rng.stream_seed(model.base_seed, seed_step, _site(kind, i))
        if h0 is not None:
            assert x is None and x_img is None and text_embed is None and langs is None and positions is None
            B = lengths.shape[0]
            S = h0.shape[0] // B
            T, R, M = S, 0, B * S
            totlen, rowmask = ops.seq_masks(lengths.to(device=dev, dtype=torch.int64).contiguous(), None, B, S)
            h = h0.detach().to(BF16).contiguous()
            ximg16 = loc = emb_saved = img_rows = img_saved = ref_saved = keylen_img = tok = None
        else:
            h = None
            T, B = x.shape
            R = 0 if x_img is None else x_img.shape[0]
            S = R + T
            M = B * S
            x = x.to(dev).contiguous()
        if h is None:
            table, tok = ar.w('embeddings.weight'), x
            if text_embed is not None:
                assert tuple(text_embed.shape) == (B, T, d), (tuple(text_embed.shape), (B, T, d))
                table = text_embed.detach().to(device=dev, dtype=BF16).contiguous().view(B * T, d)
                tok = (torch.arange(B, device=dev, dtype=torch.int64) * T)[None, :] + \
                    torch.arange(T, device=dev, dtype=torch.int64)[:, None]
                tok = tok.contiguous()
            if langs is not None or positions is not None:
                assert text_embed is None and R == 0
                rows = table[x.t()].float()
                if langs is not None:
                    langs = langs.to(dev).contiguous()
                    rows = rows + ar.p('cross_lang_embeddings.weight')[langs.t()]
                if positions is not None:
                    positions = positions.to(dev).contiguous()
                    assert positions.size() == (T, B)
                    ptab = ar.p('position_embeddings.weight')
                    rows = rows + ptab[positions.t()] - ptab[:T][None, :, :]
                table = rows.to(BF16).reshape(B * T, d).contiguous()
                tok = ((torch.arange(B, device=dev, dtype=torch.int64) * T)[None, :] +
                       torch.arange(T, device=dev, dtype=torch.int64)[:, None]).contiguous()
            totlen, rowmask = ops.seq_masks(lengths.to(device=dev, dtype=torch.int64).contiguous(),
                                            None if R == 0 else lengths_img.to(device=dev, dtype=torch.int64).contiguous(), B, S)

            ximg16 = img_proj = loc = None
            if R > 0:
                xi = x_img.detach().to(dev)
                if xi.dtype == torch.float32 and xi.stride(2) == 1 and xi.stride(0) % 4 == 0 and xi.stride(1) % 4 == 0:
                    ximg16 = ops.cast_rows_bf16(xi)
                else:
                    ximg16 = ops.cast_bf16(xi.contiguous().view(R * B, 2048))
                loc = image_loc.contiguous().float()
                img_proj = ops.gemm_nt(ximg16, ar.w('image_embeddings.image_embeddings.weight'), L.EPI_BIAS,
                                       bias=ar.p('image_embeddings.image_embeddings.bias'))
            img_rows = img_saved = ref_saved = keylen_img = None
            if p_refine is not None and R > 0:
                rows, img_saved = ops.embed_image_rows_fwd(
                    img_proj, loc, ar.p('image_embeddings.image_location_embeddings.weight'),
                    ar.p('image_embeddings.image_location_embeddings.bias'), ar.p('image_embeddings.LayerNorm.weight'),
                    ar.p('image_embeddings.LayerNorm.bias'), B, R, d, seed_img=seed('img'), p_drop=p_drop)
                keylen_img = lengths_img.to(device=dev, dtype=torch.int32).contiguous()
                img_rows, ref_saved = refiner_fwd(model, rows, keylen_img, B, R, seed_step, p_refine)
            h, emb_saved = ops.embed_assemble_fwd(
                tok, table, ar.p('position_embeddings.weight'), img_proj, loc,
                ar.p('image_embeddings.image_location_embeddings.weight'),
                ar.p('image_embeddings.image_location_embeddings.bias'),
                ar.p('image_embeddings.LayerNorm.weight'), ar.p('image_embeddings.LayerNorm.bias'),
                ar.p('layer_norm_emb.weight'), ar.p('layer_norm_emb.bias'), totlen, B, T, R, d,
                seed_img=seed('img'), seed_emb=seed('emb'), p_drop=p_drop, img_rows=img_rows, img_saved=img_saved)

        saved_layers = []
        qscale = 1.0 / math.sqrt(dh)
        st8 = model.fp8_state() if model.fp8 else None
        if st8 is not None:
            assert M % 256 == 0, 'the fp8 GEMM takes whole 256-row tiles (B * S %% 256 == 0): M = %d' % M
            if model.training:
                st8.roll()
            ready(None)
            st8.quant_weights(ar)

        def lin(xin, i, xsite, wsite, w16, epi, pre8=None, **kw):
            if st8 is None or wsite not in fp8mod.FWD_SITES:
                return ops.gemm_nt(xin, w16, epi, **kw)
            x8, dxs = pre8 if pre8 is not None else st8.quant(xin, i, xsite)
            w8, _, dws = st8.weights[(i, wsite)]
            return ops.gemm_nt_fp8(x8, w8, epi, descale_a=dxs, descale_b=dws, **kw)

        rows_c = None
        if out_rows is not None and out_rows.n and track and st8 is None and nL > 0 and d % 8 == 0 \
                and ops.gq_eligible(M, 4 * d) == ops.gq_eligible(out_rows.n, 4 * d):
            assert out_rows.M == M, 'out_rows was built for %d rows, this pass has %d' % (out_rows.M, M)
            rows_c = out_rows.to(dev)

        for i in range(nL):
            a, f = 'attentions.%d.' % i, 'ffns.%d.' % i
            ready(('layer', i))
            qkv = lin(h, i, 'x', 'wqkv', ar.qkv_w16(i), L.EPI_BIAS, bias=ar.qkv_bias(i), scale_cols=d, scale=qscale)
            ctxt, lse, kmask = ops.attn_fwd(qkv, totlen, B, S, H, dh, seed=seed('attn_p', i), p_drop=p_attn,
                                            want_mask=True)
            lse = (lse, kmask)
            compact = rows_c is not None and i == nL - 1
            Mi, ctx_in, res_in, mask_i, rr, ctx_c = M, ctxt, h, rowmask, {}, None
            if compact:
                Mi, rr = rows_c.n, dict(rng_rows=rows_c.idx)
                ctx_in = ctx_c = ops.gather_rows(ctxt, rows_c.idx, Mi, d)
                res_in = ops.gather_rows(h, rows_c.idx, Mi, d)
                mask_i = rowmask[rows_c.idx64]
            pre1 = lin(ctx_in, i, 'ctx', 'wout', ar.w(a + 'out_lin.weight'), L.EPI_BIAS_DROP_RES, bias=ar.p(a + 'out_lin.bias'),
                       aux=res_in, seed=seed('attn_out', i), p_drop=p_drop, **rr)
            x1, mean1, rstd1 = ops.layernorm_fwd(pre1, ar.p('layer_norm1.%d.weight' % i), ar.p('layer_norm1.%d.bias' % i))
            hact8 = None
            u_holds_grad = False
            if (st8 is None or 'w1' not in fp8mod.FWD_SITES) and not _GELU_GRAD_IN_FWD and _GELU_BYTE_GRAD == 2 and track \
                    and ops.gq_eligible(Mi, 4 * d):
                u = torch.empty((Mi * 4 * d,), dtype=torch.uint8, device=dev)
                o8 = {}
                if st8 is not None and 'w2' in fp8mod.FWD_SITES:
                    kh = st8.index(i, 'hact')
                    if st8.seen[kh]:
                        o8 = dict(out8=torch.empty((M, 4 * d), dtype=torch.uint8, device=dev), scale8=st8.scale[kh:kh + 1],
                                  amax8=st8.amax[kh:kh + 1])
                hact = ops.gemm_nt(x1, ar.w(f + 'lin1.weight'), L.EPI_BIAS_GELUQ, bias=ar.p(f + 'lin1.bias'), out2=u, **o8)
                if o8:
                    hact8 = (o8['out8'], st8.descale[kh:kh + 1])
                elif st8 is not None and 'w2' in fp8mod.FWD_SITES:
                    st8._first_use(hact, kh)
                u_holds_grad = 'q'
            elif Mi >= 1024 or st8 is not None:
                u = lin(x1, i, 'x1', 'w1', ar.w(f + 'lin1.weight'), L.EPI_BIAS, bias=ar.p(f + 'lin1.bias'))
                if st8 is not None and 'w2' in fp8mod.FWD_SITES and 'w2' not in fp8mod.BWD_SITES and not _GELU_GRAD_IN_FWD:
                    hact, hact8 = st8.gelu_quant(u, i)
                elif st8 is None and not _GELU_GRAD_IN_FWD and _GELU_BYTE_GRAD and track and ops.gq_eligible(Mi, 4 * d):
                    hact, u = ops.gelu_fwd_gq(u)
                    u_holds_grad = 'q'
                else:
                    u_holds_grad = _GELU_GRAD_IN_FWD or (st8 is not None and 'w2' in fp8mod.BWD_SITES)
                    hact = ops.gelu_fwd(u, grad_inplace=u_holds_grad)
            else:
                u = torch.empty((Mi, 4 * d), dtype=BF16, device=dev)
                hact = ops.gemm_nt(x1, ar.w(f + 'lin1.weight'), L.EPI_BIAS_GELU, bias=ar.p(f + 'lin1.bias'), out2=u)
            pre2 = lin(hact, i, 'hact', 'w2', ar.w(f + 'lin2.weight'), L.EPI_BIAS_DROP_RES, bias=ar.p(f + 'lin2.bias'),
                       aux=x1, seed=seed('ffn', i), p_drop=p_drop, pre8=hact8, **rr)
            h_next, mean2, rstd2 = ops.layernorm_fwd(pre2, ar.p('layer_norm2.%d.weight' % i),
                                                     ar.p('layer_norm2.%d.bias' % i), mask_i)
            if track:
                saved_layers.append((h, qkv, ctxt, lse, pre1, mean1, rstd1, x1, u, hact, pre2, mean2, rstd2, ctx_c, mask_i))
            if compact:
                h_next = ops.place_rows(h_next, rows_c.inv, M, ops.BF16_NAN_BITS)
            h = h_next

        ctx.model = model
        ctx.dims = (B, T, R, S, d, H, dh, nL)
        ctx.drop = (p_drop, p_attn, seed_step)
        ctx.u_holds_grad = nL > 0 and u_holds_grad
        ctx.rows_c = rows_c
        ctx.saved = (tok if text_embed is not None else x, totlen, rowmask, ximg16, loc, emb_saved, saved_layers)
        ctx.refine = (ref_saved, keylen_img, p_refine)
        ctx.input_grads = (R > 0 and x_img.requires_grad and track, text_embed is not None)
        ctx.langs = langs
        ctx.positions = positions
        ctx.h0_mode = None if h0 is None else h0.dtype
        hook = model.ddp_hook
        ctx.track = bool(track) and hook is not None
        ctx.tok_rows_max = hook.encoder_forward(0 if h0 is not None else T * B) if ctx.track else None
        ctx.set_materialize_grads(False)
        ctx.sink = GradSink()
        model._pending_sink = ctx.sink
        return h

    @staticmethod
    def backward(ctx, dout):
        model = ctx.model
        ar = model.arena()
        B, T, R, S, d, H, dh, nL = ctx.dims
        M = B * S
        p_drop, p_attn, seed_step = ctx.drop
        x, totlen, rowmask, ximg16, loc, emb_saved, saved_layers = ctx.saved
        ctx.saved = None
        rows_c = ctx.rows_c
        seed = lambda kind, i=0: rng.stream_seed(model.base_seed, seed_step, _site(kind, i))
        ref_saved, keylen_img, p_refine = ctx.refine
        ctx.refine = None
        hook = model.ddp_hook if ctx.track else None
        if model.ddp_hook is not None:
            model.ddp_hook.params_ready(None)
        sunk = ctx.sink.take()
        if dout is None and sunk is None:
            if hook is not None:
                hook.encoder_backward_end()
            return (None,) * N_ENC_ARGS
        if dout is None:
            dh_ = sunk
        else:
            dh_ = dout.contiguous()
            if dh_.dtype != BF16:
                dh_ = dh_.to(BF16)
            if sunk is not None:
                dh_ = dh_ + sunk.view_as(dh_)
        last = hook.encoder_backward_begin() if hook is not None else True
        st8 = model.fp8_state() if model.fp8 else None

        def dgrad(g, i, gsite, wsite, wt16, epi, pre8=None, **kw):
            if st8 is None or wsite not in fp8mod.BWD_SITES:
                return ops.gemm_nt(g, wt16, epi, **kw)
            g8, dgs = pre8 if pre8 is not None else st8.quant(g, i, gsite)
            _, wt8, dws = st8.weights[(i, wsite)]
            return ops.gemm_nt_fp8(g8, wt8, epi, a_is_bf8=True, descale_a=dgs, descale_b=dws, **kw)

        for i in reversed(range(nL)):
            a, f = 'attentions.%d.' % i, 'ffns.%d.' % i
            (h_in, qkv, ctxt, lse, pre1, mean1, rstd1, x1, u, hact, pre2, mean2, rstd2, ctx_c, mask_i) = saved_layers[i]
            saved_layers[i] = None
            compact = rows_c is not None and i == nL - 1
            rr = {}
            if compact:
                rr = dict(rng_rows=rows_c.idx)
                dh_ = ops.gather_rows(dh_.view(M, d), rows_c.idx, rows_c.n, d)
            dpre2, dY2 = ops.layernorm_bwd(dh_, None, pre2, ar.p('layer_norm2.%d.weight' % i), mean2, rstd2, mask_i,
                                           ar.g('layer_norm2.%d.weight' % i), ar.g('layer_norm2.%d.bias' % i),
                                           dbias_drop=ar.g(f + 'lin2.bias'), want_drop=p_drop > 0,
                                           seed=seed('ffn', i), p_drop=p_drop, **rr)
            if dY2 is None:
                dY2 = dpre2
            ops.gemm_wgrad(dY2, hact, ar.g(f + 'lin2.weight'))
            du8 = None
            if ctx.u_holds_grad == 'q':
                o8 = {}
                if st8 is not None and 'w1' in fp8mod.BWD_SITES:
                    kd = st8.index(i, 'du')
                    if st8.seen[kd]:
                        o8 = dict(out8=torch.empty((M, 4 * d), dtype=torch.uint8, device=dY2.device), scale8=st8.scale[kd:kd + 1],
                                  amax8=st8.amax[kd:kd + 1], out8_bf8=True)
                dU = ops.gemm_nt(dY2, ar.wt[('lin2', i)], L.EPI_MULQ, aux=u, colsum=ar.g(f + 'lin1.bias'), **o8)
                if o8:
                    du8 = (o8['out8'], st8.descale[kd:kd + 1])
                elif st8 is not None and 'w1' in fp8mod.BWD_SITES:
                    st8._first_use(dU, kd)
            else:
                dU = dgrad(dY2, i, 'dy2', 'w2', ar.wt[('lin2', i)], L.EPI_MUL if ctx.u_holds_grad else L.EPI_DGELU, aux=u,
                           colsum=ar.g(f + 'lin1.bias'))
            del hact, u, pre2
            ops.gemm_wgrad(dU, x1, ar.g(f + 'lin1.weight'))
            dx1 = dgrad(dU, i, 'du', 'w1', ar.wt[('lin1', i)], L.EPI_RES, aux=dpre2, pre8=du8)
            del dU, dpre2, dY2
            dpre1, dAO = ops.layernorm_bwd(dx1, None, pre1, ar.p('layer_norm1.%d.weight' % i), mean1, rstd1, None,
                                           ar.g('layer_norm1.%d.weight' % i), ar.g('layer_norm1.%d.bias' % i),
                                           dbias_drop=ar.g(a + 'out_lin.bias'), want_drop=p_drop > 0,
                                           seed=seed('attn_out', i), p_drop=p_drop, **rr)
            if dAO is None:
                dAO = dpre1
            dctx = dgrad(dAO, i, 'dao', 'wout', ar.wt[('out', i)], L.EPI_NONE)
            if compact:
                ops.gemm_wgrad(dAO, ctx_c, ar.g(a + 'out_lin.weight'))
                dctx = ops.place_rows(dctx, rows_c.inv, M, 0)
                dpre1 = ops.place_rows(dpre1, rows_c.inv, M, 0)
            dqkv = ops.attn_bwd(qkv, totlen, ctxt, dctx, lse[0], B, S, H, dh, dbias_qkv=ar.qkv_bias(i, grad=True),
                                seed=seed('attn_p', i), p_drop=p_attn, keepmask=lse[1])
            if compact:
                ops.gemm_wgrad(dqkv, h_in, ar.qkv_wgrad(i))
            else:
                ops.gemm_wgrad_pair(dqkv, h_in, ar.qkv_wgrad(i), dAO, ctxt, ar.g(a + 'out_lin.weight'))
            dh_ = dgrad(dqkv, i, 'dqkv', 'wqkv', ar.wt[('qkv', i)], L.EPI_RES, aux=dpre1)
            del dqkv, dctx, dAO, dpre1, dx1
            ar.touch_layer(i)
            if hook is not None:
                hook.layer_done(i, last)
        if ctx.h0_mode is not None:
            if hook is not None:
                hook.embed_done(last, ids=None, rows=None, n_max=ctx.tok_rows_max)
            return (None,) * 14 + (dh_.to(ctx.h0_mode), None, None)
        want_dximg, has_text_embed = ctx.input_grads
        langs, positions = ctx.langs, ctx.positions
        tok_rows = None
        if has_text_embed or langs is not None or positions is not None or (hook is not None and hook.active):
            tok_rows = torch.empty((T * B, d), dtype=BF16, device=dh_.device)
        grads = dict(
            d_g_emb=ar.g('layer_norm_emb.weight'), d_be_emb=ar.g('layer_norm_emb.bias'),
            d_pos=ar.g('position_embeddings.weight'), d_emb=ar.g('embeddings.weight'),
            d_g_img=ar.g('image_embeddings.LayerNorm.weight'), d_be_img=ar.g('image_embeddings.LayerNorm.bias'),
            d_b_img=ar.g('image_embeddings.image_embeddings.bias'),
            d_b_loc=ar.g('image_embeddings.image_location_embeddings.bias'),
            d_w_loc=ar.g('image_embeddings.image_location_embeddings.weight'))
        de = ops.embed_assemble_bwd(dh_, emb_saved, ar.p('layer_norm_emb.weight'),
                                    ar.p('image_embeddings.LayerNorm.weight'), x, totlen, loc, grads, B, T, R, d,
                                    -1 if has_text_embed else model.pad_index, seed_img=seed('img'), seed_emb=seed('emb'), p_drop=p_drop,
                                    img_rows_bwd=None if ref_saved is None else
                                    (lambda g: refiner_bwd(model, g, ref_saved, keylen_img, B, R, seed_step, p_refine)),
                                    tok_rows=tok_rows)
        ar.touch('layer_norm_emb.weight', 'layer_norm_emb.bias', 'position_embeddings.weight')
        if not has_text_embed:
            ar.touch('embeddings.weight')
        d_ximg = d_text = None
        if R > 0:
            ops.gemm_wgrad(de, ximg16, ar.g('image_embeddings.image_embeddings.weight'))
            ar.touch(*[n for n in ar.names if n.startswith('image_embeddings.')])
            if want_dximg:
                d_ximg = ops.gemm_nt(de, _transposed(ar.w('image_embeddings.image_embeddings.weight')), L.EPI_NONE)
                d_ximg = d_ximg.view(R, B, 2048).float()
        if has_text_embed:
            d_text = tok_rows.view(T, B, d).transpose(0, 1).float()
            tok_rows = None
        if langs is not None:
            npad = (model.n_langs + 7) // 8 * 8
            onehot = torch.zeros((T * B, npad), dtype=BF16, device=tok_rows.device)
            onehot.scatter_(1, langs.view(-1, 1), 1.0)
            dl = torch.zeros((npad, d), dtype=torch.float32, device=tok_rows.device)
            ops.gemm_wgrad(onehot, tok_rows, dl)
            ar.g('cross_lang_embeddings.weight').add_(dl[:model.n_langs])
            ar.touch('cross_lang_embeddings.weight')
        if positions is not None:
            gpos = ar.g('position_embeddings.weight')
            rows32 = tok_rows.float()
            gpos.index_add_(0, positions.reshape(-1), rows32)
            gpos[:T].sub_(rows32.view(T, B, d).sum(dim=1))
        if (langs is not None or positions is not None) and (hook is None or not hook.active):
            ops.scatter_add_token_rows(tok_rows, x.contiguous().view(-1), ar.g('embeddings.weight'), model.pad_index)
            tok_rows = None
        if hook is not None:
            hook.embed_done(last, ids=x if tok_rows is not None else None, rows=tok_rows, n_max=ctx.tok_rows_max)
        return (None, None, None, None, d_ximg, None, None, None, None, None, None, None, d_text, None, None, None, None)


class ImageStreamFn(torch.autograd.Function):

    @staticmethod
    def forward(ctx, anchor, model, x_img, lengths, image_loc, langs, p_drop, seed_step, p_refine=None, track=False):
        ar = model.arena()
        ar.refresh()
        dev = ar.device
        d = model.dim
        R, B = x_img.shape[0], x_img.shape[1]
        seed = lambda kind: rng.stream_seed(model.base_seed, seed_step, _site(kind))
        ximg16 = ops.cast_bf16(x_img.to(dev).contiguous().view(R * B, 2048))
        loc = image_loc.to(dev).contiguous().float()
        img_proj = ops.gemm_nt(ximg16, ar.w('image_embeddings.image_embeddings.weight'), L.EPI_BIAS,
                               bias=ar.p('image_embeddings.image_embeddings.bias'))
        rows, img_saved = ops.embed_image_rows_fwd(
            img_proj, loc, ar.p('image_embeddings.image_location_embeddings.weight'),
            ar.p('image_embeddings.image_location_embeddings.bias'), ar.p('image_embeddings.LayerNorm.weight'),
            ar.p('image_embeddings.LayerNorm.bias'), B, R, d, seed_img=seed('img'), p_drop=p_drop)
        if langs is not None:
            langs = langs.to(dev).contiguous()
            rows = (rows.float() + ar.p('cross_lang_embeddings.weight')[langs.t()].reshape(B * R, d)).to(BF16)
        totlen = lengths.to(device=dev, dtype=torch.int32).contiguous()
        mask = (torch.arange(R, device=dev, dtype=torch.int32)[None, :] < totlen[:, None]).reshape(B * R, 1)
        h0 = ops.dropout_rows(rows, p_drop, seed('emb')) * mask.to(BF16)
        ref_saved = None
        if p_refine is not None:
            h0, ref_saved = refiner_fwd(model, h0.contiguous(), totlen, B, R, seed_step, p_refine)
        ctx.model = model
        ctx.saved = (ximg16, loc, img_saved, totlen, mask, langs, ref_saved)
        ctx.meta = (B, R, d, p_drop, seed_step, p_refine)
        ctx.x_img_meta = (x_img.dtype, x_img.device) if x_img.requires_grad else None
        ctx.hook = model.ddp_hook if track else None
        if ctx.hook is not None:
            ctx.hook.stream_forward()
        return h0

    @staticmethod
    def backward(ctx, dh0):
        model = ctx.model
        ar = model.arena()
        ximg16, loc, img_saved, totlen, mask, langs, ref_saved = ctx.saved
        ctx.saved = None
        B, R, d, p_drop, seed_step, p_refine = ctx.meta
        seed = lambda kind: rng.stream_seed(model.base_seed, seed_step, _site(kind))
        if ref_saved is not None:
            dh0 = refiner_bwd(model, dh0.to(BF16).contiguous(), ref_saved, totlen, B, R, seed_step, p_refine)
            ar.touch(*[n for n in ar.names if n.startswith('refine_embeddings.')])
        g = (dh0.to(BF16) * mask.to(BF16)).contiguous()
        d_rows = ops.dropout_rows(g, p_drop, seed('emb'))
        if langs is not None:
            npad = (model.n_langs + 7) // 8 * 8
            onehot = torch.zeros((B * R, npad), dtype=BF16, device=g.device)
            onehot.scatter_(1, langs.t().reshape(-1, 1), 1.0)
            dl = torch.zeros((npad, d), dtype=torch.float32, device=g.device)
            ops.gemm_wgrad(onehot, d_rows, dl)
            ar.g('cross_lang_embeddings.weight').add_(dl[:model.n_langs])
            ar.touch('cross_lang_embeddings.weight')
        grads = dict(d_g_img=ar.g('image_embeddings.LayerNorm.weight'), d_be_img=ar.g('image_embeddings.LayerNorm.bias'),
                     d_b_img=ar.g('image_embeddings.image_embeddings.bias'),
                     d_b_loc=ar.g('image_embeddings.image_location_embeddings.bias'),
                     d_w_loc=ar.g('image_embeddings.image_location_embeddings.weight'))
        de = ops.embed_image_rows_bwd(d_rows, img_saved, ar.p('image_embeddings.LayerNorm.weight'), loc, totlen, grads, B, R, d,
                                      seed_img=seed('img'), p_drop=p_drop)
        ops.gemm_wgrad(de, ximg16, ar.g('image_embeddings.image_embeddings.weight'))
        ar.touch(*[n for n in ar.names if n.startswith('image_embeddings.')])
        d_ximg = None
        if ctx.x_img_meta is not None:
            d_rows = ops.gemm_nt(de, _transposed(ar.w('image_embeddings.image_embeddings.weight')), L.EPI_NONE)
            d_ximg = d_rows.view(R, B, 2048).to(device=ctx.x_img_meta[1], dtype=ctx.x_img_meta[0])
        if ctx.hook is not None:
            ctx.hook.stream_backward_end()
        return (None, None, d_ximg) + (None,) * 7


N_DEC_ARGS = 12

CAUSAL_TILED_MIN_T = 32


class DecoderFn(torch.autograd.Function):

    @staticmethod
# ... 586 lines not shown
```

### m3p_amd/lib.py

```python
import ctypes as C
import os

import torch

_HERE = os.path.dirname(os.path.abspath(__file__))
LIB_PATH = os.environ.get('M3P_HIP_LIB') or os.path.join(_HERE, 'libm3p_hip.so')

EPI_NONE, EPI_BIAS, EPI_BIAS_GELU, EPI_BIAS_DROP_RES, EPI_RES, EPI_DGELU, EPI_MUL, EPI_MULQ, EPI_BIAS_GELUQ, EPI_BIAS_LSE = range(10)
KERN_NT_SKINNY, KERN_NT_W8, KERN_NT_W8_QUEUE, KERN_NT_W4, KERN_NT_RING, KERN_NT_128 = range(1, 7)
KERN_WGRAD_W4_CHUNKS, KERN_WGRAD_W4_TILES, KERN_WGRAD_RING, KERN_WGRAD_128 = range(10, 14)


class M3PError(RuntimeError):
    pass


class Epilogue(C.Structure):
    _fields_ = [
        ('bias', C.c_void_p), ('aux', C.c_void_p), ('out2', C.c_void_p), ('colsum', C.c_void_p),
        ('ld_aux', C.c_int32), ('ld_out2', C.c_int32), ('scale_cols', C.c_int32), ('scale', C.c_float),
        ('alpha', C.c_float), ('seed', C.c_uint32), ('thresh24', C.c_uint32), ('inv_keep', C.c_float),
        ('descale_a', C.c_void_p), ('descale_b', C.c_void_p),
        ('out8', C.c_void_p), ('scale8', C.c_void_p), ('amax8', C.c_void_p), ('ld_out8', C.c_int32), ('out8_bf8', C.c_int32),
        ('rng_rows', C.c_void_p),
        ('row_ref', C.c_void_p),
    ]


_p, _i, _f, _u32 = C.c_void_p, C.c_int, C.c_float, C.c_uint32

SIGNATURES = {
    'm3p_version': (C.c_char_p, []),
    'm3p_gemm_nt_bf16': (_i, [_p, _i, _p, _i, _p, _i, _i, _i, _i, _i, C.POINTER(Epilogue), _p]),
    'm3p_gemm_nt_fp8': (_i, [_p, _i, _i, _p, _i, _p, _i, _i, _i, _i, _i, C.POINTER(Epilogue), _p]),
    'm3p_quant_fp8': (_i, [_p, _i, _p, _i, _i, _i, _p, _p, _i, _p]),
    'm3p_quant_fp8_batch': (_i, [_p, _i, _i, _p]),
    'm3p_gemm_nt_streamk_f32': (_i, [_p, _i, _p, _i, _p, _i, _i, _i, _i, _f, _p]),
    'm3p_gemm_nn_streamk_f32': (_i, [_p, _i, _p, _i, _i, _p, _i, _i, _i, _i, _f, _p]),
    'm3p_gemm_nn_w4_f32': (_i, [_p, _i, _p, _i, _p, _i, _i, _i, _i, _f, _p, C.c_size_t, _p]),
    'm3p_gemm_wgrad_workspace_bytes': (C.c_size_t, []),
    'm3p_gemm_wgrad_bf16': (_i, [_p, _i, _p, _i, _p, _i, _i, _i, _i, _f, _p, C.c_size_t, _p]),
    'm3p_gemm_wgrad_store_bf16': (_i, [_p, _i, _p, _i, _p, _i, _i, _i, _i, _f, _p, C.c_size_t, _p]),
    'm3p_gemm_wgrad_pair_bf16': (_i, [_p, _i, _p, _i, _p, _i, _i, _i, _p, _i, _p, _i, _p, _i, _i, _i, _i, _f, _p, C.c_size_t, _p]),
    'm3p_layernorm_fwd': (_i, [_p, _p, _p, _p, _p, _p, _p, _i, _i, _f, _p]),
    'm3p_layernorm_bwd': (_i, [_p, _p, _p, _p, _p, _p, _p, _p, _p, _p, _p, _p, _i, _i, _u32, _u32, _f, _p]),
    'm3p_layernorm_bwd_rows': (_i, [_p, _p, _p, _p, _p, _p, _p, _p, _p, _p, _p, _p, _i, _i, _u32, _u32, _f, _p, _p]),
    'm3p_attn_fwd': (_i, [_p, _p, _p, _p, _p, _i, _i, _i, _i, _u32, _u32, _f, _p]),
    'm3p_attn_bwd': (_i, [_p, _p, _p, _p, _p, _p, _p, _p, _i, _i, _i, _i, _f, _u32, _u32, _f, _p]),
    'm3p_attn_query_fwd': (_i, [_p, _i, _p, C.c_longlong, _i, _p, _p, _i, _i, _i, _i, _i, _i, _i, _p]),
    'm3p_attn_rows_fwd': (_i, [_p, _i, _p, C.c_longlong, _i, _p, _p, _p, _i, _i, _i, _i, _i, _i, _i, _u32, _u32, _f, _p]),
    'm3p_attn_rows_bwd': (_i, [_p, _i, _p, C.c_longlong, _i, _p, _p, _p, _p, _i, _p, _i, _i, _i, _i, _i, _i, _i, _f, _u32, _u32, _f, _p]),
    'm3p_attn_causal_fwd': (_i, [_p, _i, _p, _p, _i, _i, _i, _i, _u32, _u32, _f, _p]),
    'm3p_attn_causal_bwd': (_i, [_p, _i, _p, _p, _p, _i, _i, _i, _i, _i, _f, _u32, _u32, _f, _p]),
    'm3p_cast_f32_bf16': (_i, [_p, _p, C.c_longlong, _p]),
    'm3p_embed_assemble_fwd': (_i, [_p] * 19 + [_i, _i, _i, _i, _u32, _u32, _u32, _f, _p, _p]),
    'm3p_embed_image_rows_fwd': (_i, [_p] * 10 + [_i, _i, _i, _u32, _u32, _f, _p]),
    'm3p_embed_assemble_bwd': (_i, [_p] * 24 + [_i, _i, _i, _i, _i, _u32, _u32, _u32, _f, _i, _p]),
    'm3p_dropout_rows': (_i, [_p, _i, _p, _i, _p, _i, _i, _i, _u32, _u32, _u32, _u32, _f, _p]),
    'm3p_glu_fwd': (_i, [_p, _i, _p, _i, _i, _p]),
    'm3p_glu_bwd': (_i, [_p, _i, _p, _p, _i, _i, _p]),
    'm3p_gather_rows': (_i, [_p, _p, _p, _i, _i, _p]),
    'm3p_place_rows': (_i, [_p, _p, _p, _i, _i, _i, _u32, _p]),
    'm3p_scatter_add_rows': (_i, [_p, _p, _p, _i, _i, _p]),
    'm3p_scatter_add_token_rows': (_i, [_p, _i, _p, _p, _i, _i, _i, _p]),
    'm3p_ce_fwd_bwd': (_i, [_p, _i, _i, _i, _p, _p, _p, _f, _f, _p]),
    'm3p_ce_colsum_workspace_bytes': (C.c_size_t, [_i, _i]),
    'm3p_ce_fwd_bwd_colsum': (_i, [_p, _i, _i, _i, _p, _p, _p, _f, _p, _p, C.c_size_t, _p]),
    'm3p_ce_lse_from_blocks': (_i, [_p, _i, _i, _p, _i, _p, _p, _p, _p, _p]),
    'm3p_ce_bwd_colsum': (_i, [_p, _i, _i, _i, _p, _p, _f, _p, _p, C.c_size_t, _p]),
    'm3p_ce_shift_target': (_i, [_p, _p, _p, _p, _p, _p, _i, _i, _p]),
    'm3p_ce_shift_rows': (_i, [_p, _i, _i, _f, _p, _p, _p, _p, _p]),
    'm3p_ce_shift_colsum': (_i, [_p, _i, _i, _p, _p, _p, C.c_size_t, _p]),
    'm3p_ce_shift_scale_rows': (_i, [_p, _p, _p, _p, _i, _i, _p]),
    'm3p_ce_shift_target_rows': (_i, [_p, _p, _p, _p, _p, _p, _i, _i, _p]),
    'm3p_ce_shift_dh': (_i, [_p, _p, _p, _p, _p, _p, _p, _i, _i, _p]),
    'm3p_ce_eval': (_i, [_p, _i, _i, _i, _p, _p, _p, _p]),
    'm3p_colsum_bf16': (_i, [_p, _i, _i, _i, _p, _p, _p]),
    'm3p_sumsq_f32': (_i, [_p, C.c_longlong, _p, _p]),
    'm3p_sumsq_ranges_f32': (_i, [_p, _p, _p, _i, _p, _p]),
    'm3p_adam_step': (_i, [_p, _p, _p, _p, _p, C.c_longlong, _f, _f, _f, _f, _f, _f, _p, _f, _f, _i, _p]),
    'm3p_adam_step_ranges': (_i, [_p, _p, _p, _p, _p, _p, _p, _p, _p, _i, _f, _f, _f, _f, _f, _p, _f, _f, _p]),
    'm3p_itm_score_fwd': (_i, [_p, _p, _p, _p, _p, _i, _i, _p]),
    'm3p_itm_score_bwd': (_i, [_p, _p, _p, _p, _p, _i, _p, _p, _p, _i, _i, _p]),
    'm3p_gelu_bwd': (_i, [_p, _p, _p, C.c_longlong, _p]),
    'm3p_mse_fwd_bwd': (_i, [_p, _i, _p, _i, _p, _p, _i, _i, _f, _p]),
    'm3p_gelu_fwd': (_i, [_p, _p, _p, C.c_longlong, _p]),
    'm3p_gelu_fwd_gq': (_i, [_p, _p, _p, _i, _i, _p]),
    'm3p_gelu_fwd_q8': (_i, [_p, _p, _p, C.c_longlong, _p, _p, _p]),
    'm3p_transpose_batch_bf16': (_i, [_p, _i, _i, _p]),
    'm3p_transpose_bf16': (_i, [_p, _p, _i, _i, _i, _i, _p]),
    'm3p_set_persistent_grid': (_i, [_i]),
    'm3p_set_tile_queue': (_i, [_p, _i]),
    'm3p_gemm_nt_plan': (_i, [_i, _i, _i, _i]),
    'm3p_gemm_wgrad_plan': (_i, [_i, _i, _i]),
    'm3p_debug_set_variant': (None, [_i]),
    'm3p_debug_attn_variant': (None, [_i]),
    'm3p_seq_masks': (_i, [_p, _p, _i, _i, _p, _p, _p]),
    'm3p_mask_to_rows': (_i, [_p, _i, _i, C.c_longlong, C.c_longlong, C.c_longlong, _i, _p, _i, _p]),
    'm3p_cast_rows_f32_bf16': (_i, [_p, C.c_longlong, C.c_longlong, _i, _i, _i, _p, _p]),
    'm3p_scale_bf16_dev': (_i, [_p, _i, _p, _p, C.c_longlong, _p]),
    'm3p_axpy_dev_f32': (_i, [_p, _p, _p, C.c_longlong, _p]),
    'm3p_itm_loss_fwd_bwd': (_i, [_p, _p, _i, _i, _f, _f, _p, _p, _p]),
    'm3p_probe_mfma_16x16x32': (_i, [_p, _p, _p, _p, _p]),
    'm3p_probe_mfma_fp8_16x16x128': (_i, [_p, _p, _p, _i, _p]),
    'm3p_probe_tr16': (_i, [_p, _p, _p]),
    'm3p_probe_permlane16_swap': (_i, [_p, _p]),
}

_lib = None


def load():
    global _lib
    if _lib is not None:
        return _lib
    if not os.path.exists(LIB_PATH):
        raise M3PError('libm3p_hip.so not found at %s — build it first (make -C m3p_amd/csrc); '
                       'there is no fallback path' % LIB_PATH)
    lib = C.CDLL(LIB_PATH)
    for name, (res, args) in SIGNATURES.items():
        fn = getattr(lib, name)
        fn.restype = res
        fn.argtypes = args
    _lib_tq = os.environ.get('M3P_TILE_QUEUE', '0') != '0'
    _lib = lib
    if _lib_tq and torch.cuda.is_available():
        from . import ops
        ops.set_tile_queue(True)
    return lib


def check(code, what):
    if code != 0:
        kind = {-1: 'M3P_EINVAL (bad shape/alignment)', -2: 'M3P_ENOTIMPL', -3: 'M3P_ENOMEM'}.get(code, 'hipError_t %d' % code)
        raise M3PError('%s failed: %s' % (what, kind))


def ptr(t):
    return None if t is None else t.data_ptr()


def stream():
    return torch.cuda.current_stream().cuda_stream


def num_cus():
    n = torch.cuda.get_device_properties(torch.cuda.current_device()).multi_processor_count
    return max(n - n % 8, 8)


def thresh24(p):
    return int(round(float(p) * (1 << 24)))
```

### m3p_amd/ops.py

```python
import ctypes as C
import os

import torch

from . import lib as L

BF16 = torch.bfloat16
_DEBUG_CHECKS = os.environ.get('M3P_DEBUG_CHECKS') == '1'

PROFILE = None
_EPI_NAMES = ['gemm_nt/none', 'gemm_nt/bias', 'gemm_nt/bias_gelu', 'gemm_nt/bias_drop_res', 'gemm_nt/res',
              'gemm_nt/dgelu', 'gemm_nt/mul', 'gemm_nt/mulq', 'gemm_nt/bias_geluq', 'gemm_nt/bias_lse']


PROFILE_ONLY = None


def _prof_begin(key=None):
    if PROFILE is None or (PROFILE_ONLY is not None and key != PROFILE_ONLY):
        return None
    e = torch.cuda.Event(enable_timing=True)
    e.record()
    return e

# ... 119 lines not shown
    _chk_bf16(a, w)
    M, K = a.shape
    N = w.shape[0]
    assert w.shape[1] == K and out_f32.dtype == torch.float32 and out_f32.shape == (M, N)
    e0 = _prof_begin(('gemm_nt/streamk', M, N, K))
    rc = L.load().m3p_gemm_nt_streamk_f32(a.data_ptr(), a.stride(0), w.data_ptr(), w.stride(0), out_f32.data_ptr(),
                                          out_f32.stride(0), M, N, K, alpha, L.stream())
    L.check(rc, 'm3p_gemm_nt_streamk_f32')
    _prof_end(e0, ('gemm_nt/streamk', M, N, K))
    return out_f32


def gemm_nn_streamk(a, w_kn, out_f32, alpha=1.0):
    _chk_bf16(a, w_kn)
    M, K = a.shape
    k_valid, N = w_kn.shape
    assert k_valid <= K and out_f32.dtype == torch.float32 and out_f32.shape == (M, N) and w_kn.stride(1) == 1
    e0 = _prof_begin(('gemm_nt/streamk', M, N, K))
    rc = L.load().m3p_gemm_nn_streamk_f32(a.data_ptr(), a.stride(0), w_kn.data_ptr(), w_kn.stride(0), k_valid,
                                          out_f32.data_ptr(), out_f32.stride(0), M, N, K, alpha, L.stream())
    L.check(rc, 'm3p_gemm_nn_streamk_f32')
    _prof_end(e0, ('gemm_nt/streamk', M, N, K))
    return out_f32


def gemm_nn(a, w_kn, out_f32, alpha=1.0, k_rows_readable=None):
    _chk_bf16(a, w_kn)
    M, K = a.shape
    k_valid, N = w_kn.shape
    if (k_rows_readable or k_valid) >= K and M % 256 == 0 and N % 256 == 0 and K % 64 == 0 and K >= 4096:
        assert out_f32.dtype == torch.float32 and out_f32.shape == (M, N) and w_kn.stride(1) == 1
        e0 = _prof_begin(('gemm_nn/w4', M, N, K))
        ws = _wgrad_workspace(a.device)
        rc = L.load().m3p_gemm_nn_w4_f32(a.data_ptr(), a.stride(0), w_kn.data_ptr(), w_kn.stride(0), out_f32.data_ptr(),
                                         out_f32.stride(0), M, N, K, alpha, ws.data_ptr(), ws.numel(), L.stream())
        if rc == 0:
            _prof_end(e0, ('gemm_nn/w4', M, N, K))
            return out_f32
        if rc != -2:
            L.check(rc, 'm3p_gemm_nn_w4_f32')
    return gemm_nn_streamk(a, w_kn, out_f32, alpha)


_WGRAD_WS = {}


def _wgrad_workspace(device):
    key = (device.index, torch.cuda.current_stream(device).cuda_stream)
    ws = _WGRAD_WS.get(key)
    if ws is None:
        ws = _WGRAD_WS[key] = torch.empty(int(L.load().m3p_gemm_wgrad_workspace_bytes()), dtype=torch.uint8, device=device)
    return ws


def gemm_wgrad(dy, x, dw, alpha=1.0, n=None, k=None, dw_is_zero=False, report_store=False, must_store=False):
    _chk_bf16(dy, x)
    assert dw.dtype == torch.float32 and dw.stride(-1) == 1
    M = dy.shape[0]
    N = dy.shape[1] if n is None else n
    K = x.shape[1] if k is None else k
    assert x.shape[0] == M and dw.shape[0] >= N and dw.shape[1] >= K
    e0 = _prof_begin(('gemm_wgrad', M, N, K))
    ws = _wgrad_workspace(dy.device)
    if dw_is_zero:
        rc = L.load().m3p_gemm_wgrad_store_bf16(dy.data_ptr(), dy.stride(0), x.data_ptr(), x.stride(0), dw.data_ptr(),
                                                dw.stride(0), M, N, K, alpha, ws.data_ptr(), ws.numel(), L.stream())
        if rc == 0:
            _prof_end(e0, ('gemm_wgrad', M, N, K))
            return True if report_store else dw
        if rc != -2:
            L.check(rc, 'm3p_gemm_wgrad_store_bf16')
        if must_store:
            raise L.M3PError('m3p_gemm_wgrad_store_bf16 declined (M3P_ENOTIMPL) a store the caller depends on: dw is not physically zero')
    rc = L.load().m3p_gemm_wgrad_bf16(dy.data_ptr(), dy.stride(0), x.data_ptr(), x.stride(0), dw.data_ptr(),
                                      dw.stride(0), M, N, K, alpha, ws.data_ptr(), ws.numel(), L.stream())
    L.check(rc, 'm3p_gemm_wgrad_bf16')
    _prof_end(e0, ('gemm_wgrad', M, N, K))
    return False if report_store else dw


def gemm_wgrad_pair(dy_a, x_a, dw_a, dy_b, x_b, dw_b, alpha=1.0):
    _chk_bf16(dy_a, x_a, dy_b, x_b)
    assert dw_a.dtype == torch.float32 and dw_b.dtype == torch.float32 and dw_a.stride(-1) == 1 and dw_b.stride(-1) == 1
    M = dy_a.shape[0]
    assert x_a.shape[0] == M and dy_b.shape[0] == M and x_b.shape[0] == M
    Na, Ka, Nb, Kb = dy_a.shape[1], x_a.shape[1], dy_b.shape[1], x_b.shape[1]
    assert dw_a.shape[0] >= Na and dw_a.shape[1] >= Ka and dw_b.shape[0] >= Nb and dw_b.shape[1] >= Kb
    e0 = _prof_begin(('gemm_wgrad_pair', M, Na + Nb, Ka))
    ws = _wgrad_workspace(dy_a.device)
    rc = L.load().m3p_gemm_wgrad_pair_bf16(dy_a.data_ptr(), dy_a.stride(0), x_a.data_ptr(), x_a.stride(0), dw_a.data_ptr(), dw_a.stride(0),
                                           Na, Ka, dy_b.data_ptr(), dy_b.stride(0), x_b.data_ptr(), x_b.stride(0), dw_b.data_ptr(),
                                           dw_b.stride(0), Nb, Kb, M, alpha, ws.data_ptr(), ws.numel(), L.stream())
    L.check(rc, 'm3p_gemm_wgrad_pair_bf16')
    _prof_end(e0, ('gemm_wgrad_pair', M, Na + Nb, Ka))


def layernorm_fwd(x, gamma, beta, rowmask=None, eps=1e-12):
    _chk_bf16(x)
    rows, d = x.shape
    assert x.is_contiguous()
    y = torch.empty_like(x)
    mean = torch.empty(rows, dtype=torch.float32, device=x.device)
    rstd = torch.empty(rows, dtype=torch.float32, device=x.device)
    rc = L.load().m3p_layernorm_fwd(x.data_ptr(), gamma.data_ptr(), beta.data_ptr(), L.ptr(rowmask), y.data_ptr(),
                                    mean.data_ptr(), rstd.data_ptr(), rows, d, eps, L.stream())
    L.check(rc, 'm3p_layernorm_fwd')
    return y, mean, rstd


def layernorm_bwd(dy_a, dy_b, x, gamma, mean, rstd, rowmask, dgamma, dbeta, dbias_drop=None,
                  want_drop=False, seed=0, p_drop=0.0, rng_rows=None):
    _chk_bf16(dy_a, dy_b, x)
    rows, d = x.shape
    if rng_rows is not None:
        assert rng_rows.dtype == torch.int32 and rng_rows.is_cuda and rng_rows.is_contiguous() and rng_rows.numel() == rows
    dx = torch.empty_like(x)
    dx_drop = torch.empty_like(x) if want_drop else None
    rc = L.load().m3p_layernorm_bwd_rows(dy_a.data_ptr(), L.ptr(dy_b), x.data_ptr(), gamma.data_ptr(), mean.data_ptr(),
                                         rstd.data_ptr(), L.ptr(rowmask), dx.data_ptr(), L.ptr(dx_drop),
                                         dgamma.data_ptr(), dbeta.data_ptr(), L.ptr(dbias_drop), rows, d, seed,
                                         L.thresh24(p_drop), 1.0 / (1.0 - p_drop) if p_drop > 0 else 1.0,
                                         L.ptr(rng_rows), L.stream())
    L.check(rc, 'm3p_layernorm_bwd_rows')
    return dx, dx_drop


def attn_fwd(qkv, keylen, B, S, H, dh, seed=0, p_drop=0.0, want_mask=False):
    _chk_bf16(qkv)
    assert qkv.is_contiguous() and qkv.shape == (B * S, 3 * H * dh) and keylen.dtype == torch.int32
    ctx = torch.empty((B * S, H * dh), dtype=BF16, device=qkv.device)
    lse = torch.empty((B, H, S), dtype=torch.float32, device=qkv.device)
    mask = None
    if want_mask and p_drop > 0:
        nt = (S + 15) // 16
        mask = torch.empty((B * H, nt, nt, 4), dtype=torch.int64, device=qkv.device)
    rc = L.load().m3p_attn_fwd(qkv.data_ptr(), keylen.data_ptr(), ctx.data_ptr(), lse.data_ptr(), L.ptr(mask), B, S, H, dh,
                               seed, L.thresh24(p_drop), 1.0 / (1.0 - p_drop) if p_drop > 0 else 1.0, L.stream())
    L.check(rc, 'm3p_attn_fwd')
    return (ctx, lse, mask) if want_mask else (ctx, lse)


def attn_bwd(qkv, keylen, ctx, dctx, lse, B, S, H, dh, dbias_qkv=None, seed=0, p_drop=0.0, keepmask=None):
    _chk_bf16(qkv, ctx, dctx)
    assert dctx.is_contiguous() and ctx.is_contiguous()
    assert p_drop == 0 or keepmask is not None, 'attention backward with dropout needs the keep words of the forward pass'
    dqkv = torch.empty_like(qkv)
    rc = L.load().m3p_attn_bwd(qkv.data_ptr(), keylen.data_ptr(), ctx.data_ptr(), dctx.data_ptr(), lse.data_ptr(),
                               L.ptr(keepmask), dqkv.data_ptr(), L.ptr(dbias_qkv), B, S, H, dh, 1.0 / (dh ** 0.5), seed,
                               L.thresh24(p_drop), 1.0 / (1.0 - p_drop) if p_drop > 0 else 1.0, L.stream())
    L.check(rc, 'm3p_attn_bwd')
    return dqkv


def attn_query_fwd(q, kv, klen, B, Tq, H, dh, Lk, causal=False, pos0=0):
    _chk_bf16(q, kv)
    assert q.stride(1) == 1 and kv.dim() == 3 and kv.stride(2) == 1 and kv.shape[0] == B and kv.shape[1] >= Lk
    ctx = torch.empty((B * Tq, H * dh), dtype=BF16, device=q.device)
    rc = L.load().m3p_attn_query_fwd(q.data_ptr(), q.stride(0), kv.data_ptr(), kv.stride(0), kv.stride(1), L.ptr(klen),
                                     ctx.data_ptr(), B, Tq, H, dh, Lk, 1 if causal else 0, pos0, L.stream())
    L.check(rc, 'm3p_attn_query_fwd')
    return ctx


def attn_rows_fwd(q, kv, klen, B, Tq, H, dh, Lk, causal=False, seed=0, p_drop=0.0):
    _chk_bf16(q, kv)
    assert q.stride(1) == 1 and kv.dim() == 3 and kv.stride(2) == 1 and kv.shape[0] == B and kv.shape[1] >= Lk
    ctx = torch.empty((B * Tq, H * dh), dtype=BF16, device=q.device)
    lse = torch.empty((B, H, Tq), dtype=torch.float32, device=q.device)
    rc = L.load().m3p_attn_rows_fwd(q.data_ptr(), q.stride(0), kv.data_ptr(), kv.stride(0), kv.stride(1), L.ptr(klen),
                                    ctx.data_ptr(), lse.data_ptr(), B, Tq, H, dh, Lk, 1 if causal else 0, 0, seed,
                                    L.thresh24(p_drop), 1.0 / (1.0 - p_drop) if p_drop > 0 else 1.0, L.stream())
    L.check(rc, 'm3p_attn_rows_fwd')
    return ctx, lse


def attn_rows_bwd(q, kv, klen, dctx, lse, B, Tq, H, dh, Lk, qscale, causal=False, seed=0, p_drop=0.0, dq_out=None):
    _chk_bf16(q, kv, dctx)
    assert dctx.is_contiguous()
    d = H * dh
    dq = dq_out if dq_out is not None else torch.empty((B * Tq, d), dtype=BF16, device=q.device)
    dkv = torch.zeros((B, Lk, 2 * d), dtype=torch.float32, device=q.device)
    rc = L.load().m3p_attn_rows_bwd(q.data_ptr(), q.stride(0), kv.data_ptr(), kv.stride(0), kv.stride(1), L.ptr(klen),
                                    dctx.data_ptr(), lse.data_ptr(), dq.data_ptr(), dq.stride(0), dkv.data_ptr(), B, Tq, H, dh, Lk,
                                    1 if causal else 0, 0, qscale, seed, L.thresh24(p_drop),
                                    1.0 / (1.0 - p_drop) if p_drop > 0 else 1.0, L.stream())
    L.check(rc, 'm3p_attn_rows_bwd')
    return dq, dkv


def attn_causal_fwd(qkv, B, T, H, dh, seed=0, p_drop=0.0, out=None):
    _chk_bf16(qkv)
    assert qkv.dim() == 2 and qkv.stride(1) == 1 and qkv.shape[0] == B * T and qkv.shape[1] >= 3 * H * dh
    if out is not None:
        ctx, lse = out
        assert ctx.dtype == BF16 and ctx.is_contiguous() and ctx.shape == (B * T, H * dh)
        assert lse.dtype == torch.float32 and lse.is_contiguous() and lse.shape == (B, H, T)
    else:
        ctx = torch.empty((B * T, H * dh), dtype=BF16, device=qkv.device)
        lse = torch.empty((B, H, T), dtype=torch.float32, device=qkv.device)
    rc = L.load().m3p_attn_causal_fwd(qkv.data_ptr(), qkv.stride(0), ctx.data_ptr(), lse.data_ptr(), B, T, H, dh, seed,
                                      L.thresh24(p_drop), 1.0 / (1.0 - p_drop) if p_drop > 0 else 1.0, L.stream())
    if rc == -2:
        return None
    L.check(rc, 'm3p_attn_causal_fwd')
    return ctx, lse


def attn_causal_bwd(qkv, dctx, lse, B, T, H, dh, qscale, seed=0, p_drop=0.0, out=None):
    _chk_bf16(qkv, dctx)
    assert qkv.dim() == 2 and qkv.stride(1) == 1 and qkv.shape[0] == B * T and dctx.is_contiguous()
    assert dctx.shape == (B * T, H * dh) and lse.dtype == torch.float32 and lse.is_contiguous() and lse.shape == (B, H, T)
    if out is not None:
        dqkv = out
        assert dqkv.dtype == BF16 and dqkv.stride(1) == 1 and dqkv.shape == (B * T, 3 * H * dh)
    else:
        dqkv = torch.empty((B * T, 3 * H * dh), dtype=BF16, device=qkv.device)
    rc = L.load().m3p_attn_causal_bwd(qkv.data_ptr(), qkv.stride(0), dctx.data_ptr(), lse.data_ptr(), dqkv.data_ptr(),
                                      dqkv.stride(0), B, T, H, dh, qscale, seed, L.thresh24(p_drop),
                                      1.0 / (1.0 - p_drop) if p_drop > 0 else 1.0, L.stream())
    if rc == -2:
        return None
    L.check(rc, 'm3p_attn_causal_bwd')
    return dqkv


def cast_bf16(x):
    if x.dtype == BF16:
        return x
    assert x.dtype == torch.float32 and x.is_contiguous() and x.numel() % 4 == 0
    out = torch.empty(x.shape, dtype=BF16, device=x.device)
    L.check(L.load().m3p_cast_f32_bf16(x.data_ptr(), out.data_ptr(), x.numel(), L.stream()), 'm3p_cast_f32_bf16')
    return out


_TILE_QUEUE = {}


def set_tile_queue(enable=True, slots=4096):
    dev = torch.cuda.current_device()
    if not enable:
        L.check(L.load().m3p_set_tile_queue(None, 0), 'm3p_set_tile_queue')
        _TILE_QUEUE.pop(dev, None)
        return
    pool = torch.zeros(slots * 8, dtype=torch.int32, device='cuda')
    torch.cuda.current_stream().synchronize()
    L.check(L.load().m3p_set_tile_queue(pool.data_ptr(), slots), 'm3p_set_tile_queue')
    _TILE_QUEUE[dev] = pool


def cast_f32_bf16_into(src, dst):
    assert src.dtype == torch.float32 and dst.dtype == BF16 and src.is_contiguous() and dst.is_contiguous()
    assert src.numel() == dst.numel() and src.numel() % 4 == 0
    L.check(L.load().m3p_cast_f32_bf16(src.data_ptr(), dst.data_ptr(), src.numel(), L.stream()), 'm3p_cast_f32_bf16')


def cast_rows_bf16(x):
    assert x.dim() == 3 and x.dtype == torch.float32 and x.stride(2) == 1
    n0, n1, cols = x.shape
    out = torch.empty((n0 * n1, cols), dtype=BF16, device=x.device)
    L.check(L.load().m3p_cast_rows_f32_bf16(x.data_ptr(), x.stride(0), x.stride(1), n0, n1, cols, out.data_ptr(), L.stream()),
            'm3p_cast_rows_f32_bf16')
    return out


def seq_masks(lengths, lengths_b, B, S):
    dev = lengths.device
    assert lengths.dtype == torch.int64 and lengths.is_contiguous() and lengths.numel() == B
    if lengths_b is not None:
        assert lengths_b.dtype == torch.int64 and lengths_b.is_contiguous() and lengths_b.numel() == B and lengths_b.device == dev
    totlen = torch.empty((B,), dtype=torch.int32, device=dev)
    rowmask = torch.empty((B * S,), dtype=torch.uint8, device=dev)
    L.check(L.load().m3p_seq_masks(lengths.data_ptr(), L.ptr(lengths_b), B, S, totlen.data_ptr(), rowmask.data_ptr(), L.stream()),
            'm3p_seq_masks')
    return totlen, rowmask


def mask_to_rows(mask, inner, s0, s1, soff, d, n_rows):
    m = mask.reshape(-1)
    if m.dtype == torch.bool:
        m = m.view(torch.uint8)
    assert m.dtype == torch.uint8 and m.is_contiguous()
    rows = torch.empty((n_rows,), dtype=torch.int32, device=m.device)
    if _DEBUG_CHECKS:
        assert int(m.sum().item()) == n_rows, 'mask holds %d True entries, the caller counted %d' % (int(m.sum().item()), n_rows)
    L.check(L.load().m3p_mask_to_rows(m.data_ptr(), m.numel(), inner, s0, s1, soff, d, rows.data_ptr(), n_rows, L.stream()),
            'm3p_mask_to_rows')
    return rows


def scale_bf16_dev(x, g):
    assert x.is_contiguous() and x.dtype in (BF16, torch.float32) and g.dtype == torch.float32 and g.numel() == 1
    out = torch.empty(x.shape, dtype=BF16, device=x.device)
    L.check(L.load().m3p_scale_bf16_dev(x.data_ptr(), int(x.dtype == torch.float32), g.data_ptr(), out.data_ptr(), x.numel(),
                                        L.stream()), 'm3p_scale_bf16_dev')
    return out


def axpy_dev(dst, src, g):
    assert dst.dtype == src.dtype == g.dtype == torch.float32 and dst.is_contiguous() and src.is_contiguous()
    assert dst.numel() == src.numel()
    L.check(L.load().m3p_axpy_dev_f32(dst.data_ptr(), src.data_ptr(), g.data_ptr(), dst.numel(), L.stream()), 'm3p_axpy_dev_f32')


def itm_loss_fwd_bwd(scores, pos, sample_n, w_ce, w_bce):
    sc = scores.reshape(-1)
    assert sc.dtype == torch.float32 and sc.is_contiguous() and pos.dtype == torch.int64 and pos.is_contiguous()
    G = pos.numel()
    assert sc.numel() == G * sample_n, (sc.numel(), G, sample_n)
    loss = torch.empty((1,), dtype=torch.float32, device=sc.device)
    dsc = torch.empty_like(sc)
    L.check(L.load().m3p_itm_loss_fwd_bwd(sc.data_ptr(), pos.data_ptr(), G, sample_n, float(w_ce), float(w_bce), loss.data_ptr(),
                                          dsc.data_ptr(), L.stream()), 'm3p_itm_loss_fwd_bwd')
    return loss, dsc


def _drop_args(p):
    return L.thresh24(p), (1.0 / (1.0 - p) if p > 0 else 1.0)


def embed_assemble_fwd(tok, emb16, pos, img_proj, loc, w_loc, b_loc, g_img, be_img, g_emb, be_emb, totlen,
                       B, T, R, d, seed_img=0, seed_emb=0, p_drop=0.0, img_rows=None, img_saved=None):
    dev = emb16.device
    S = R + T
    h = torch.empty((B * S, d), dtype=BF16, device=dev)
    z = torch.empty((B * S, d), dtype=BF16, device=dev)
    mean_e = torch.empty(B * S, dtype=torch.float32, device=dev)
    rstd_e = torch.empty(B * S, dtype=torch.float32, device=dev)
    if img_rows is not None:
        assert img_rows.dtype == BF16 and img_rows.is_contiguous() and img_rows.shape == (B * R, d)
        e, mean_i, rstd_i = img_saved
    else:
        e = torch.empty((max(R * B, 1), d), dtype=BF16, device=dev)
        mean_i = torch.empty(max(R * B, 1), dtype=torch.float32, device=dev)
        rstd_i = torch.empty(max(R * B, 1), dtype=torch.float32, device=dev)
    th, ik = _drop_args(p_drop)
    rc = L.load().m3p_embed_assemble_fwd(
        tok.data_ptr(), emb16.data_ptr(), pos.data_ptr(), L.ptr(img_proj), L.ptr(loc), w_loc.data_ptr(),
        b_loc.data_ptr(), g_img.data_ptr(), be_img.data_ptr(), g_emb.data_ptr(), be_emb.data_ptr(), totlen.data_ptr(),
        h.data_ptr(), z.data_ptr(), mean_e.data_ptr(), rstd_e.data_ptr(), e.data_ptr(), mean_i.data_ptr(),
        rstd_i.data_ptr(), B, T, R, d, seed_img, seed_emb, th, ik, L.ptr(img_rows), L.stream())
    L.check(rc, 'm3p_embed_assemble_fwd')
    return h, (z, mean_e, rstd_e, e, mean_i, rstd_i)


def embed_image_rows_fwd(img_proj, loc, w_loc, b_loc, g_img, be_img, B, R, d, seed_img=0, p_drop=0.0):
    dev = img_proj.device
    e = torch.empty((R * B, d), dtype=BF16, device=dev)
    mean_i = torch.empty(R * B, dtype=torch.float32, device=dev)
    rstd_i = torch.empty(R * B, dtype=torch.float32, device=dev)
    rows = torch.empty((B * R, d), dtype=BF16, device=dev)
    th, ik = _drop_args(p_drop)
    rc = L.load().m3p_embed_image_rows_fwd(img_proj.data_ptr(), loc.data_ptr(), w_loc.data_ptr(), b_loc.data_ptr(),
                                           g_img.data_ptr(), be_img.data_ptr(), e.data_ptr(), mean_i.data_ptr(),
                                           rstd_i.data_ptr(), rows.data_ptr(), B, R, d, seed_img, th, ik, L.stream())
    L.check(rc, 'm3p_embed_image_rows_fwd')
    return rows, (e, mean_i, rstd_i)


def embed_image_rows_bwd(d_rows, img_saved, g_img, loc, totlen, grads, B, R, d, seed_img=0, p_drop=0.0):
    e, mean_i, rstd_i = img_saved
    assert d_rows.dtype == BF16 and d_rows.is_contiguous() and d_rows.shape == (B * R, d)
    de = torch.empty_like(e)
    th, ik = _drop_args(p_drop)
    dummy = d_rows.data_ptr()
    args = (dummy, dummy, mean_i.data_ptr(), rstd_i.data_ptr(), g_img.data_ptr(), e.data_ptr(), mean_i.data_ptr(),
            rstd_i.data_ptr(), g_img.data_ptr(), dummy, totlen.data_ptr(), loc.data_ptr(), d_rows.data_ptr(), de.data_ptr(),
            grads['d_g_img'].data_ptr(), grads['d_be_img'].data_ptr(), grads['d_g_img'].data_ptr(), grads['d_g_img'].data_ptr(),
            None, grads['d_g_img'].data_ptr(), grads['d_be_img'].data_ptr(), grads['d_b_img'].data_ptr(),
            grads['d_b_loc'].data_ptr(), grads['d_w_loc'].data_ptr(), B, 0, R, d, -1, seed_img, 0, th, ik)
    L.check(L.load().m3p_embed_assemble_bwd(*args, 2, L.stream()), 'm3p_embed_assemble_bwd')
    return de


def embed_assemble_bwd(dh, saved, g_emb, g_img, tok, totlen, loc, grads, B, T, R, d, pad_index,
                       seed_img=0, seed_emb=0, p_drop=0.0, img_rows_bwd=None, tok_rows=None):
    z, mean_e, rstd_e, e, mean_i, rstd_i = saved
    dz = torch.empty_like(z)
    de = torch.empty_like(e)
    th, ik = _drop_args(p_drop)
    if tok_rows is not None:
        assert tok_rows.dtype == BF16 and tok_rows.is_contiguous() and tok_rows.shape == (T * B, d)
    args = (dh.data_ptr(), z.data_ptr(), mean_e.data_ptr(), rstd_e.data_ptr(), g_emb.data_ptr(), e.data_ptr(),
            mean_i.data_ptr(), rstd_i.data_ptr(), g_img.data_ptr(), tok.data_ptr(), totlen.data_ptr(), L.ptr(loc),
            dz.data_ptr(), de.data_ptr(), grads['d_g_emb'].data_ptr(), grads['d_be_emb'].data_ptr(),
            grads['d_pos'].data_ptr(), grads['d_emb'].data_ptr(), L.ptr(tok_rows), grads['d_g_img'].data_ptr(),
            grads['d_be_img'].data_ptr(), grads['d_b_img'].data_ptr(), grads['d_b_loc'].data_ptr(),
            grads['d_w_loc'].data_ptr(), B, T, R, d, pad_index, seed_img, seed_emb, th, ik)
    if img_rows_bwd is not None:
        L.check(L.load().m3p_embed_assemble_bwd(*args, 1, L.stream()), 'm3p_embed_assemble_bwd')
        dz_img = dz.view(B, R + T, d)[:, :R, :]
        dz_img.copy_(img_rows_bwd(dz_img.contiguous().view(B * R, d)).view(B, R, d))
        L.check(L.load().m3p_embed_assemble_bwd(*args, 2, L.stream()), 'm3p_embed_assemble_bwd')
        return de
    L.check(L.load().m3p_embed_assemble_bwd(*args, 0, L.stream()), 'm3p_embed_assemble_bwd')
    return de


def scatter_add_token_rows(rows, ids, dst, pad_index):
    _chk_bf16(rows)
    assert ids.dtype == torch.int64 and dst.dtype == torch.float32 and rows.stride(1) == 1 and ids.is_contiguous()
    n, d = rows.shape
    assert ids.numel() == n and dst.shape[1] == d and dst.stride(0) == d
    L.check(L.load().m3p_scatter_add_token_rows(rows.data_ptr(), rows.stride(0), ids.data_ptr(), dst.data_ptr(), n, d, int(pad_index),
                                                L.stream()), 'm3p_scatter_add_token_rows')


def gather_rows(src_base, idx, n, d):
    out = torch.empty((n, d), dtype=BF16, device=idx.device)
    L.check(L.load().m3p_gather_rows(src_base.data_ptr(), idx.data_ptr(), out.data_ptr(), n, d, L.stream()), 'm3p_gather_rows')
    return out


BF16_NAN_BITS = 0x7FC0


def place_rows(src, inv, rows, fill_bits=0):
    _chk_bf16(src)
    n, d = src.shape
    assert src.is_contiguous() and inv.dtype == torch.int32 and inv.is_cuda and inv.is_contiguous() and inv.numel() == rows
    out = torch.empty((rows, d), dtype=BF16, device=src.device)
    L.check(L.load().m3p_place_rows(src.data_ptr(), inv.data_ptr(), out.data_ptr(), rows, d, n, int(fill_bits), L.stream()),
            'm3p_place_rows')
    return out


def scatter_add_rows(src, idx, dst_base, n, d):
    L.check(L.load().m3p_scatter_add_rows(src.data_ptr(), idx.data_ptr(), dst_base.data_ptr(), n, d, L.stream()),
            'm3p_scatter_add_rows')


def ce_fwd_bwd(logits, V, target, loss_scale, grad_scale):
    n, ld = logits.shape[0], logits.stride(0)
    row_loss = torch.empty(n, dtype=torch.float32, device=logits.device)
    assert target.dtype == torch.int64
    rc = L.load().m3p_ce_fwd_bwd(logits.data_ptr(), ld, n, V, target.data_ptr(), row_loss.data_ptr(),
                                 None, loss_scale, grad_scale, L.stream())
    L.check(rc, 'm3p_ce_fwd_bwd')
    loss_sum = (row_loss.sum() * loss_scale).reshape(1)
    return loss_sum, row_loss


_CE_WS = {}


def ce_fwd_bwd_colsum(logits, V, target, loss_scale, grad_scale):
    n, ld = logits.shape[0], logits.stride(0)
    dev = logits.device
    row_loss = torch.empty(n, dtype=torch.float32, device=dev)
    row_lse = torch.empty(n, dtype=torch.float32, device=dev)
    cs = torch.empty(ld, dtype=torch.float32, device=dev)
    need = L.load().m3p_ce_colsum_workspace_bytes(ld, n)
    ws = _CE_WS.get(dev)
    if ws is None or ws.numel() < need:
        ws = _CE_WS[dev] = torch.empty(need, dtype=torch.uint8, device=dev)
    assert target.dtype == torch.int64
    rc = L.load().m3p_ce_fwd_bwd_colsum(logits.data_ptr(), ld, n, V, target.data_ptr(), row_loss.data_ptr(), row_lse.data_ptr(),
                                        grad_scale, cs.data_ptr(), ws.data_ptr(), ws.numel(), L.stream())
    L.check(rc, 'm3p_ce_fwd_bwd_colsum')
    return (row_loss.sum() * loss_scale).reshape(1), row_loss, cs


def ce_from_block_stats(logits, V, target, stats, loss_scale, grad_scale):
    n, ld = logits.shape[0], logits.stride(0)
    dev = logits.device
    row_loss = torch.empty(n, dtype=torch.float32, device=dev)
    row_lse = torch.empty(n, dtype=torch.float32, device=dev)
    cs = torch.empty(ld, dtype=torch.float32, device=dev)
    scratch = torch.empty((32, n, 2), dtype=torch.float32, device=dev)
    assert target.dtype == torch.int64 and stats.dtype == torch.float32 and stats.shape[1] == n
    L.check(L.load().m3p_ce_lse_from_blocks(stats.data_ptr(), stats.shape[0], n, logits.data_ptr(), ld, target.data_ptr(),
                                            row_loss.data_ptr(), row_lse.data_ptr(), scratch.data_ptr(), L.stream()),
            'm3p_ce_lse_from_blocks')
    need = L.load().m3p_ce_colsum_workspace_bytes(ld, n)
    ws = _CE_WS.get(dev)
    if ws is None or ws.numel() < need:
        ws = _CE_WS[dev] = torch.empty(need, dtype=torch.uint8, device=dev)
    L.check(L.load().m3p_ce_bwd_colsum(logits.data_ptr(), ld, n, V, target.data_ptr(), row_lse.data_ptr(), grad_scale, cs.data_ptr(),
                                       ws.data_ptr(), ws.numel(), L.stream()), 'm3p_ce_bwd_colsum')
    return (row_loss.sum() * loss_scale).reshape(1), row_loss, cs


def ce_shift_target(h, emb, bias, target):
    _chk_bf16(h, emb)
    n, d = h.shape
    assert h.is_contiguous() and emb.stride(0) == d and emb.stride(1) == 1 and bias.dtype == torch.float32 and bias.is_contiguous()
    assert target.dtype == torch.int64 and target.is_contiguous() and target.numel() == n
    row_t = torch.empty(n, dtype=torch.float32, device=h.device)
    row_ref = torch.empty((n, 2), dtype=torch.int32, device=h.device)
    L.check(L.load().m3p_ce_shift_target(h.data_ptr(), emb.data_ptr(), bias.data_ptr(), target.data_ptr(), row_t.data_ptr(),
                                         row_ref.data_ptr(), n, d, L.stream()), 'm3p_ce_shift_target')
    return row_t, row_ref


def ce_shift_from_block_sums(e, stats, loss_scale, grad_scale):
    n, ld = e.shape[0], e.stride(0)
    dev = e.device
    assert stats.dtype == torch.float32 and stats.is_contiguous() and stats.shape[1] == n
    row_loss = torch.empty(n, dtype=torch.float32, device=dev)
    row_s = torch.empty(n, dtype=torch.float32, device=dev)
    row_q = torch.empty(n, dtype=torch.float32, device=dev)
    scratch = torch.empty((32, n), dtype=torch.float32, device=dev)
    L.check(L.load().m3p_ce_shift_rows(stats.data_ptr(), stats.shape[0], n, grad_scale, row_loss.data_ptr(), row_s.data_ptr(),
                                       row_q.data_ptr(), scratch.data_ptr(), L.stream()), 'm3p_ce_shift_rows')
    cs = torch.empty(ld, dtype=torch.float32, device=dev)
    need = L.load().m3p_ce_colsum_workspace_bytes(ld, n)
    ws = _CE_WS.get(dev)
    if ws is None or ws.numel() < need:
        ws = _CE_WS[dev] = torch.empty(need, dtype=torch.uint8, device=dev)
    L.check(L.load().m3p_ce_shift_colsum(e.data_ptr(), ld, n, row_s.data_ptr(), cs.data_ptr(), ws.data_ptr(), ws.numel(), L.stream()),
            'm3p_ce_shift_colsum')
    return (row_loss.sum() * loss_scale).reshape(1), row_loss, row_s, row_q, cs


def ce_shift_scale_rows(h, row_s, g):
    _chk_bf16(h)
    assert h.is_contiguous() and row_s.dtype == g.dtype == torch.float32 and row_s.numel() == h.shape[0] and g.numel() == 1
    out = torch.empty_like(h)
    L.check(L.load().m3p_ce_shift_scale_rows(h.data_ptr(), row_s.data_ptr(), g.data_ptr(), out.data_ptr(), h.shape[0], h.shape[1],
                                             L.stream()), 'm3p_ce_shift_scale_rows')
    return out


def ce_shift_target_rows(h, target, row_q, g, demb, dbias):
    _chk_bf16(h)
    n, d = h.shape
    assert h.is_contiguous() and target.dtype == torch.int64 and target.numel() == n and row_q.dtype == g.dtype == torch.float32
    assert demb.dtype == dbias.dtype == torch.float32 and demb.shape[1] == d and demb.stride(0) == d and dbias.is_contiguous()
    L.check(L.load().m3p_ce_shift_target_rows(h.data_ptr(), target.data_ptr(), row_q.data_ptr(), g.data_ptr(), demb.data_ptr(),
                                              dbias.data_ptr(), n, d, L.stream()), 'm3p_ce_shift_target_rows')


def ce_shift_dh(dh32, emb, target, row_s, row_q, g):
    _chk_bf16(emb)
    n, d = dh32.shape
    assert dh32.dtype == torch.float32 and dh32.is_contiguous() and emb.stride(0) == d and emb.stride(1) == 1
    assert target.dtype == torch.int64 and target.numel() == n and row_s.dtype == row_q.dtype == g.dtype == torch.float32
    out = torch.empty((n, d), dtype=BF16, device=dh32.device)
    L.check(L.load().m3p_ce_shift_dh(dh32.data_ptr(), emb.data_ptr(), target.data_ptr(), row_s.data_ptr(), row_q.data_ptr(),
                                     g.data_ptr(), out.data_ptr(), n, d, L.stream()), 'm3p_ce_shift_dh')
    return out


def ce_eval(logits, V, target):
    _chk_bf16(logits)
    assert logits.dim() == 2 and logits.stride(1) == 1 and target.dtype == torch.int64 and target.is_contiguous()
    n, ld = logits.shape[0], logits.stride(0)
    assert target.numel() == n and ld >= V
    row_loss = torch.empty(n, dtype=torch.float32, device=logits.device)
    row_argmax = torch.empty(n, dtype=torch.int32, device=logits.device)
    L.check(L.load().m3p_ce_eval(logits.data_ptr(), ld, n, V, target.data_ptr(), row_loss.data_ptr(), row_argmax.data_ptr(),
                                 L.stream()), 'm3p_ce_eval')
    return row_loss, row_argmax


def colsum(x, ncols, out, scale=None):
    rc = L.load().m3p_colsum_bf16(x.data_ptr(), x.stride(0), x.shape[0], ncols, out.data_ptr(), L.ptr(scale), L.stream())
    L.check(rc, 'm3p_colsum_bf16')


def sumsq(g, out):
    L.check(L.load().m3p_sumsq_f32(g.data_ptr(), g.numel(), out.data_ptr(), L.stream()), 'm3p_sumsq_f32')


def sumsq_ranges(buf, ranges, out):
    ranges = [(int(a), int(b)) for a, b in ranges if b > a]
    if not ranges:
        return
    if len(ranges) == 1:
        return sumsq(buf[ranges[0][0]:ranges[0][1]], out)
    n = len(ranges)
    starts = (C.c_longlong * n)(*[a for a, _ in ranges])
    counts = (C.c_longlong * n)(*[b - a for a, b in ranges])
    L.check(L.load().m3p_sumsq_ranges_f32(buf.data_ptr(), starts, counts, n, out.data_ptr(), L.stream()), 'm3p_sumsq_ranges_f32')


def adam_step(p, g, m, v, w16, lr, beta1, beta2, eps, weight_decay, step_size, gnorm_sq=None, max_norm=0.0,
              grad_scale=1.0, zero_grad=True):
    n = p.numel()
# ... 150 lines not shown
```

Before: 8122 sequences/s.

## Compute last-layer attention only for selected query rows via qsel kernels

Adds query-selected attention forward and backward kernels so the final layer computes Q, context and LSE only for the compacted rows that feed the loss, while K/V still cover all positions. The model path projects Q only for selected rows and skips the full attention plus gather steps, and the backward writes dQ compactly and places it into the full dQKV buffer. This removes wasted attention work for unused query rows in the last layer. In exchange it adds new kernels, padding logic, and more complex dropout-mask indexing that must match the forward.

```diff
diff --git a/include/m3p_hip.h b/include/m3p_hip.h
--- a/include/m3p_hip.h
+++ b/include/m3p_hip.h
@@ -107,6 +107,15 @@
                          int H, int dh, float qscale, uint32_t seed, uint32_t thresh24, float inv_keep,
                          void* stream);
 
+#define M3P_QSEL_ROW_PAD 256
+M3P_API int m3p_attn_qsel_fwd(const void* q_c, int ld_q, const void* kv, int ld_kv, const int32_t* keylen, const int32_t* qrow,
+                              const int32_t* seq_start, void* ctx_c, float* lse_c, uint64_t* keepwords, int B, int S, int H,
+                              int dh, int n_rows, uint32_t seed, uint32_t thresh24, float inv_keep, void* stream);
+M3P_API int m3p_attn_qsel_bwd(const void* q_c, int ld_q, const void* kv, int ld_kv, const int32_t* keylen, const int32_t* qrow,
+                              const int32_t* seq_start, const void* ctx_c, const void* dctx_c, const float* lse_c,
+                              const uint64_t* keepwords, void* dq_c, int ld_dq, void* dkv, int ld_dkv, float* dbias_qkv, int B,
+                              int S, int H, int dh, int n_rows, float qscale, uint32_t thresh24, float inv_keep, void* stream);
+
 M3P_API int m3p_attn_query_fwd(const void* q, int ld_q, const void* kv, long long kv_bstride, int ld_kv,
                                const int32_t* klen, void* ctx, int B, int Tq, int H, int dh, int Lk, int causal,
                                int pos0, void* stream);
@@ -156,6 +165,8 @@
 M3P_API int m3p_gather_rows(const void* src, const int32_t* idx, void* dst, int n, int d, void* stream);
 M3P_API int m3p_place_rows(const void* src, const int32_t* inv, void* dst, int rows, int d, int n, uint32_t fill_bits,
                            void* stream);
+M3P_API int m3p_place_rows_ld(const void* src, const int32_t* inv, void* dst, int ld_dst, int rows, int d, int n,
+                              uint32_t fill_bits, void* stream);
 M3P_API int m3p_scatter_add_rows(const void* src, const int32_t* idx, void* dst, int n, int d, void* stream);
 M3P_API int m3p_scatter_add_token_rows(const void* rows, int ld_rows, const int64_t* ids, float* dst, int n, int d,
                                        int pad_index, void* stream);
diff --git a/m3p_amd/csrc/attention.hip b/m3p_amd/csrc/attention.hip
--- a/m3p_amd/csrc/attention.hip
+++ b/m3p_amd/csrc/attention.hip
@@ -99,11 +99,18 @@
   }
 }
 
-template <int DH, int KT, bool DROP, int NTC, int NW = 4, bool EVENS = false>
+struct QSelArgs {
+  const bf16* kv;
+  const int* qrow;
+  const int* seq_start;
+  int ld_q, ld_kv, n_rows, n_pad;
+};
+
+template <int DH, int KT, bool DROP, int NTC, int NW = 4, bool EVENS = false, bool QSEL = false>
 __global__ __launch_bounds__(NW * 64, NW == 8 ? 2 : 3)
 void attn_fwd_kernel(const bf16* __restrict__ qkv, const int* __restrict__ keylen, bf16* __restrict__ ctx,
                      float* __restrict__ lse, unsigned long long* __restrict__ keepmask, int S, int H, int dmodel,
-                     uint32_t seed, uint32_t thresh24, float inv_keep) {
+                     uint32_t seed, uint32_t thresh24, float inv_keep, QSelArgs qs) {
   using Cf = AttnCfg<DH>;
   extern __shared__ __attribute__((aligned(16))) char smem[];
   const int tid = threadIdx.x, lane = tid & 63;
@@ -111,10 +118,25 @@
   const int b = blockIdx.x / H, h = blockIdx.x - b * H;
   const int nt = NTC ? NTC : (S + 15) >> 4;
   const int nk = (nt + 1) >> 1;
-  const size_t ld = 3 * (size_t)dmodel;
-  const bf16* Qg = qkv + (size_t)b * S * ld + h * DH;
-  const bf16* Kg = Qg + dmodel;
-  const bf16* Vg = Qg + 2 * dmodel;
+  const size_t ld = QSEL ? (size_t)qs.ld_kv : 3 * (size_t)dmodel;
+  const size_t ldq = QSEL ? (size_t)qs.ld_q : ld;
+  int e0 = 0, cnt = S;
+  if constexpr (QSEL) {
+    e0 = qs.seq_start[b];
+    cnt = qs.seq_start[b + 1] - e0;
+    if (b == gridDim.x / H - 1) {
+      const int npad = qs.n_pad - qs.n_rows;
+      for (int i = tid; i < npad * Cf::CH; i += NW * 64)
+        *reinterpret_cast<u32x4_t*>(ctx + (size_t)(qs.n_rows + i / Cf::CH) * dmodel + h * DH + 8 * (i % Cf::CH)) = u32x4_t{0u, 0u, 0u, 0u};
+      for (int i = tid; i < npad; i += NW * 64) lse[(size_t)h * qs.n_pad + qs.n_rows + i] = 0.f;
+    }
+    if (cnt <= 0) return;
+  }
+  const int nqb = QSEL ? (cnt + 15) >> 4 : nt;
+  const bf16* Qg = QSEL ? qkv + (size_t)e0 * ldq + h * DH : qkv + (size_t)b * S * ld + h * DH;
+  const bf16* Kg = QSEL ? qs.kv + (size_t)b * S * ld + h * DH : Qg + dmodel;
+  const bf16* Vg = Kg + dmodel;
+  const int qlast = QSEL ? cnt - 1 : S - 1;
   char* sK = smem;
   char* sV = smem + nt * 16 * Cf::ROWB;
   stage_rows<DH>(Kg, ld, S, nt * 16, sK, wid, lane, NW);
@@ -122,11 +144,13 @@
   const int fq = lane & 15, fg = lane >> 4;
   const int wrot = (wid + (blockIdx.x >> 3)) & (NW - 1);
   bf16x8 qnext[Cf::KK];
+  int snext = 0;
   {
-    const int qc0 = min(wrot * 16 + fq, S - 1);
+    const int qc0 = min(wrot * 16 + fq, qlast);
 #pragma unroll
     for (int kk = 0; kk < Cf::KK; ++kk)
-      qnext[kk] = *reinterpret_cast<const bf16x8*>(Qg + (size_t)qc0 * ld + 32 * kk + 8 * fg);
+      qnext[kk] = *reinterpret_cast<const bf16x8*>(Qg + (size_t)qc0 * ldq + 32 * kk + 8 * fg);
+    if constexpr (QSEL) snext = qs.qrow[e0 + qc0] - b * S;
   }
   const int klen = keylen[b];
   __syncthreads();
@@ -140,17 +164,18 @@
   for (int n = 0; n < Cf::NT; ++n)
     v_off[n] = vrow * Cf::ROWB + Cf::swz(2 * n + ((fq & 3) >> 1), vrow) * 16 + 8 * (fq & 1);
 
-  for (int qb = wrot; qb < nt; qb += NW) {
+  for (int qb = wrot; qb < nqb; qb += NW) {
     const int q = qb * 16 + fq;
-    const int qc = min(q, S - 1);
+    const int qc = QSEL ? snext : min(q, S - 1);
     bf16x8 qf[Cf::KK];
 #pragma unroll
     for (int kk = 0; kk < Cf::KK; ++kk) qf[kk] = qnext[kk];
     {
-      const int qcn = min(q + 16 * NW, S - 1);
+      const int qcn = min(q + 16 * NW, qlast);
 #pragma unroll
       for (int kk = 0; kk < Cf::KK; ++kk)
-        qnext[kk] = *reinterpret_cast<const bf16x8*>(Qg + (size_t)qcn * ld + 32 * kk + 8 * fg);
+        qnext[kk] = *reinterpret_cast<const bf16x8*>(Qg + (size_t)qcn * ldq + 32 * kk + 8 * fg);
+      if constexpr (QSEL) snext = qs.qrow[e0 + qcn] - b * S;
     }
 
     f32x4 s[2 * KT];
@@ -199,7 +224,9 @@
     const uint32_t rbase = (uint32_t)((b * H + h) * S + qc) * (uint32_t)S;
     const uint32_t thr16 = thresh24 >> 8;
     const bool even_rows = EVENS || (S & 1) == 0;
-    unsigned long long* mrow = keepmask ? keepmask + ((size_t)(b * H + h) * nt + qb) * nt * 4 : nullptr;
+    unsigned long long* mrow = !keepmask ? nullptr
+                             : QSEL ? keepmask + ((size_t)h * ((qs.n_rows >> 4) + (int)(gridDim.x / H)) + (e0 >> 4) + b + qb) * nt * 4
+                                    : keepmask + ((size_t)(b * H + h) * nt + qb) * nt * 4;
     constexpr int MW = (8 * KT + 63) / 64;
     uint32_t mlo[MW], mhi[MW];
 #pragma unroll
@@ -283,8 +310,13 @@
       bf16x4 ob[Cf::NT];
 #pragma unroll
       for (int n = 0; n < Cf::NT; ++n) ob[n] = bf16x4{(bf16)o[n][0], (bf16)o[n][1], (bf16)o[n][2], (bf16)o[n][3]};
+      if constexpr (QSEL) {
+        store_row_widened<Cf::NT>(ctx + (size_t)(e0 + min(q, qlast)) * dmodel + h * DH, fg, q < cnt, ob);
+        if (q < cnt && fg == 0) lse[(size_t)h * qs.n_pad + e0 + q] = mx + __logf(sum);
+      } else {
       store_row_widened<Cf::NT>(ctx + (size_t)(b * S + min(q, S - 1)) * dmodel + h * DH, fg, q < S, ob);
       if (q < S && fg == 0) lse[(size_t)(b * H + h) * S + q] = mx + __logf(sum);
+      }
     }
   }
 }
@@ -1080,23 +1112,330 @@
 #undef PAD_TILE
 }
 
-template <int DH>
+template <int DH, bool DROP>
+__global__ __launch_bounds__(256, 3)
+void attn_qsel_bwd_kernel(const bf16* __restrict__ q_c, int ld_q, const bf16* __restrict__ kv, int ld_kv,
+                          const int* __restrict__ keylen, const int* __restrict__ seq_start, const bf16* __restrict__ ctx,
+                          const bf16* __restrict__ dctx, const float* __restrict__ lse,
+                          const unsigned long long* __restrict__ keepmask, bf16* __restrict__ dq_c, int ld_dq,
+                          bf16* __restrict__ dkv, int ld_dkv, float* __restrict__ dbias_qkv, int B, int S, int H, int dmodel,
+                          int n_rows, int n_pad, float qscale, float inv_keep) {
+  constexpr int NW = 4;
+  constexpr bool MASK = DROP;
+  using Cf = AttnCfg<DH>;
+  extern __shared__ __attribute__((aligned(16))) char smem[];
+  const int tid = threadIdx.x, lane = tid & 63;
+  const int wid = __builtin_amdgcn_readfirstlane(tid >> 6);
+  const int b = blockIdx.x / H, h = blockIdx.x - b * H;
+  const int wrot = (wid + (blockIdx.x >> 3)) & (NW - 1);
+  const int nt = (S + 15) >> 4, nk = (S + 31) >> 5;
+  const int e0 = seq_start[b], cnt = seq_start[b + 1] - e0;
+  const int nqt = (cnt + 15) >> 4, nqk = (cnt + 31) >> 5;
+  const bf16* Kg = kv + (size_t)b * S * ld_kv + h * DH;
+  const bf16* Vg = Kg + dmodel;
+  bf16* dKg = dkv + (size_t)b * S * ld_dkv + h * DH;
+  bf16* dVg = dKg + dmodel;
+  if (b == B - 1) {
+    for (int i = tid; i < (n_pad - n_rows) * Cf::CH; i += NW * 64)
+      *reinterpret_cast<u32x4_t*>(dq_c + (size_t)(n_rows + i / Cf::CH) * ld_dq + h * DH + 8 * (i % Cf::CH)) = u32x4_t{0u, 0u, 0u, 0u};
+  }
+  if (cnt <= 0) {
+    for (int i = tid; i < S * Cf::CH; i += NW * 64) {
+      const size_t o = (size_t)(i / Cf::CH) * ld_dkv + 8 * (i % Cf::CH);
+      *reinterpret_cast<u32x4_t*>(dKg + o) = u32x4_t{0u, 0u, 0u, 0u};
+      *reinterpret_cast<u32x4_t*>(dVg + o) = u32x4_t{0u, 0u, 0u, 0u};
+    }
+    return;
+  }
+  const bf16* Qg = q_c + (size_t)e0 * ld_q + h * DH;
+  const bf16* Og = ctx + (size_t)e0 * dmodel + h * DH;
+  const bf16* dOg = dctx + (size_t)e0 * dmodel + h * DH;
+  bf16* dQg = dq_c + (size_t)e0 * ld_dq + h * DH;
+  const float* lse_bh = lse + (size_t)h * n_pad + e0;
+  const int klen = keylen[b];
+  const unsigned long long* mbh = MASK ? keepmask + ((size_t)h * ((n_rows >> 4) + B) + (e0 >> 4) + b) * nt * 4 : nullptr;
+
+  const int tile_bytes = nk * 32 * Cf::ROWB;
+  char* s0 = smem;
+  char* s1 = smem + tile_bytes;
+  float* sL = reinterpret_cast<float*>(smem + 2 * tile_bytes);
+  float* sD = sL + nk * 32;
+  const int fq = lane & 15, fg = lane >> 4;
+  float* sB = sD + nk * 32;
+  float* sBw = sB + wid * 3 * DH;
+  f32x4 bsum[Cf::NT];
+#pragma unroll
+  for (int n = 0; n < Cf::NT; ++n) bsum[n] = f32x4{0.f, 0.f, 0.f, 0.f};
+  auto bias_acc = [&](int n, const bf16x4& v4) {
+    bsum[n] += f32x4{(float)v4[0], (float)v4[1], (float)v4[2], (float)v4[3]};
+  };
+  auto bias_flush = [&](int part) {
+#pragma unroll
+    for (int n = 0; n < Cf::NT; ++n) {
+      f32x4 x = bsum[n];
+#pragma unroll
+      for (int r = 0; r < 4; ++r) x[r] = row16_sum(x[r]);
+      if (fq == 0) *reinterpret_cast<f32x4*>(sBw + part * DH + 16 * n + 4 * fg) = x;
+      bsum[n] = f32x4{0.f, 0.f, 0.f, 0.f};
+    }
+  };
+
+  int r_off[Cf::KK];
+#pragma unroll
+  for (int kk = 0; kk < Cf::KK; ++kk) r_off[kk] = fq * Cf::ROWB + Cf::swz(4 * kk + fg, fq) * 16;
+  const int trow = 4 * fg + (fq >> 2);
+  int t_off[Cf::NT];
+#pragma unroll
+  for (int n = 0; n < Cf::NT; ++n)
+    t_off[n] = trow * Cf::ROWB + Cf::swz(2 * n + ((fq & 3) >> 1), trow) * 16 + 8 * (fq & 1);
+
+  constexpr float kLog2e = 1.4426950408889634f;
+  constexpr float kMasked = -1.0e30f;
+  stage_rows<DH>(Qg, (size_t)ld_q, cnt, nqk * 32, s0, wid, lane, NW);
+  stage_rows<DH>(dOg, (size_t)dmodel, cnt, nqk * 32, s1, wid, lane, NW);
+  bf16x8 kf[Cf::KK], vf[Cf::KK];
+  auto load_kv = [&](int kb) {
+    const int keyc = min(kb * 16 + fq, S - 1);
+#pragma unroll
+    for (int kk = 0; kk < Cf::KK; ++kk) {
+      kf[kk] = *reinterpret_cast<const bf16x8*>(Kg + (size_t)keyc * ld_kv + 32 * kk + 8 * fg);
+      vf[kk] = *reinterpret_cast<const bf16x8*>(Vg + (size_t)keyc * ld_kv + 32 * kk + 8 * fg);
+    }
+  };
+  if (wrot < nt) load_kv(wrot);
+  const float log2_inv_keep = DROP ? __builtin_amdgcn_logf(inv_keep) : 0.f;
+  const float keep_prob = DROP ? __builtin_amdgcn_rcpf(inv_keep) : 1.f;
+  for (int q = tid; q < nqk * 32; q += NW * 64) {
+    float dsum = 0.f, l = INFINITY;
+    if (q < cnt) {
+      const bf16* op = Og + (size_t)q * dmodel;
+      const bf16* dp = dOg + (size_t)q * dmodel;
+#pragma unroll
+      for (int c = 0; c < DH / 8; ++c) {
+        const bf16x8 ov = *reinterpret_cast<const bf16x8*>(op + 8 * c);
+        const bf16x8 dv = *reinterpret_cast<const bf16x8*>(dp + 8 * c);
+#pragma unroll
+        for (int e = 0; e < 8; ++e) dsum += (float)ov[e] * (float)dv[e];
+      }
+      l = lse_bh[q] * kLog2e - log2_inv_keep;
+    }
+    sD[q] = dsum * keep_prob;
+    sL[q] = l;
+  }
+  __syncthreads();
+  for (int kb0 = wrot; kb0 < nt; kb0 += NW) {
+    const int key = kb0 * 16 + fq;
+    const int keyc = min(key, S - 1);
+    const float kbias = (key < klen) ? 0.f : kMasked;
+    if (kb0 != wrot) load_kv(kb0);
+    f32x4 dv[Cf::NT], dk[Cf::NT];
+#pragma unroll
+    for (int n = 0; n < Cf::NT; ++n) dv[n] = dk[n] = f32x4{0.f, 0.f, 0.f, 0.f};
+    for (int kq = 0; kq < nqk; ++kq) {
+      f32x4 scA[2], dpA[2], dnegA[2];
+#pragma unroll
+      for (int hf = 0; hf < 2; ++hf) {
+        const int t = 2 * kq + hf;
+        dnegA[hf] = f32x4{-sD[16 * t + 4 * fg + 0], -sD[16 * t + 4 * fg + 1], -sD[16 * t + 4 * fg + 2],
+                          -sD[16 * t + 4 * fg + 3]};
+        scA[hf] = f32x4{kbias, kbias, kbias, kbias};
+        dpA[hf] = DROP ? f32x4{0.f, 0.f, 0.f, 0.f} : dnegA[hf];
+      }
+#pragma unroll
+      for (int kk = 0; kk < Cf::KK; ++kk) {
+#pragma unroll
+        for (int hf = 0; hf < 2; ++hf) {
+          const int t = 2 * kq + hf;
+          if (!MASK && t >= nqt) continue;
+          const bf16x8 qf = *reinterpret_cast<const bf16x8*>(s0 + t * 16 * Cf::ROWB + r_off[kk]);
+          const bf16x8 df = *reinterpret_cast<const bf16x8*>(s1 + t * 16 * Cf::ROWB + r_off[kk]);
+          scA[hf] = __builtin_amdgcn_mfma_f32_16x16x32_bf16(qf, kf[kk], scA[hf], 0, 0, 0);
+          dpA[hf] = __builtin_amdgcn_mfma_f32_16x16x32_bf16(df, vf[kk], dpA[hf], 0, 0, 0);
+        }
+      }
+      f32x4 pd2[2], ds2[2];
+#pragma unroll
+      for (int hf = 0; hf < 2; ++hf) {
+        const int t = 2 * kq + hf;
+        if (!MASK && t >= nqt) {
+          pd2[hf] = ds2[hf] = f32x4{0.f, 0.f, 0.f, 0.f};
+          continue;
+        }
+        const f32x4 dneg = dnegA[hf], sc = scA[hf], dp = dpA[hf];
+        uint32_t kbits = 0;
+        if (MASK) {
+          const unsigned long long w = mbh[((size_t)min(t, nqt - 1) * nt + kb0) * 4 + (fq & 3)];
+          kbits = (uint32_t)(w >> (4 * fg + 16 * (fq >> 2)));
+        }
+#pragma unroll
+        for (int r = 0; r < 4; ++r) {
+          const int q = 16 * t + 4 * fg + r;
+          const float p = __builtin_amdgcn_exp2f(__builtin_fmaf(sc[r], kLog2e, -sL[q]));
+          if (DROP) {
+            const float pd = __builtin_bit_cast(float, __builtin_bit_cast(uint32_t, p) & bit_to_mask(kbits, r));
+            pd2[hf][r] = pd;
+            ds2[hf][r] = __builtin_fmaf(pd, dp[r], p * dneg[r]);
+          } else {
+            pd2[hf][r] = p;
+            ds2[hf][r] = p * dp[r];
+          }
+        }
+      }
+      const bf16x8 pfrag = bf16x8{(bf16)pd2[0][0], (bf16)pd2[0][1], (bf16)pd2[0][2], (bf16)pd2[0][3],
+                                  (bf16)pd2[1][0], (bf16)pd2[1][1], (bf16)pd2[1][2], (bf16)pd2[1][3]};
+      const bf16x8 sfrag = bf16x8{(bf16)ds2[0][0], (bf16)ds2[0][1], (bf16)ds2[0][2], (bf16)ds2[0][3],
+                                  (bf16)ds2[1][0], (bf16)ds2[1][1], (bf16)ds2[1][2], (bf16)ds2[1][3]};
+#pragma unroll
+      for (int n = 0; n < Cf::NT; ++n) {
+        const char* pq = s0 + kq * 32 * Cf::ROWB + t_off[n];
+        const char* pdo = s1 + kq * 32 * Cf::ROWB + t_off[n];
+        const bf16x8 qT = cat8(lds_tr16(pq), lds_tr16(pq + 16 * Cf::ROWB));
+        const bf16x8 dT = cat8(lds_tr16(pdo), lds_tr16(pdo + 16 * Cf::ROWB));
+        dv[n] = __builtin_amdgcn_mfma_f32_16x16x32_bf16(dT, pfrag, dv[n], 0, 0, 0);
+        dk[n] = __builtin_amdgcn_mfma_f32_16x16x32_bf16(qT, sfrag, dk[n], 0, 0, 0);
+      }
+    }
+    bf16x4 kb4[Cf::NT], vb4[Cf::NT];
+#pragma unroll
+    for (int n = 0; n < Cf::NT; ++n) {
+      kb4[n] = bf16x4{(bf16)dk[n][0], (bf16)dk[n][1], (bf16)dk[n][2], (bf16)dk[n][3]};
+      vb4[n] = bf16x4{(bf16)dv[n][0], (bf16)dv[n][1], (bf16)dv[n][2], (bf16)dv[n][3]};
+    }
+    const bool ok = key < S;
+    if (dbias_qkv) {
+#pragma unroll
+      for (int n = 0; n < Cf::NT; ++n) bias_acc(n, ok ? vb4[n] : bf16x4{0, 0, 0, 0});
+    }
+    store_row_widened<Cf::NT>(dKg + (size_t)keyc * ld_dkv, fg, ok, kb4);
+    store_row_widened<Cf::NT>(dVg + (size_t)keyc * ld_dkv, fg, ok, vb4);
+  }
+  if (dbias_qkv) bias_flush(2);
+  __syncthreads();
+
+  stage_rows<DH>(Kg, (size_t)ld_kv, S, nk * 32, s0, wid, lane, NW);
+  stage_rows<DH>(Vg, (size_t)ld_kv, S, nk * 32, s1, wid, lane, NW);
+  bf16x8 qf[Cf::KK], df[Cf::KK];
+  auto load_qd = [&](int qb) {
+    const int qc = min(qb * 16 + fq, cnt - 1);
+#pragma unroll
+    for (int kk = 0; kk < Cf::KK; ++kk) {
+      qf[kk] = *reinterpret_cast<const bf16x8*>(Qg + (size_t)qc * ld_q + 32 * kk + 8 * fg);
+      df[kk] = *reinterpret_cast<const bf16x8*>(dOg + (size_t)qc * dmodel + 32 * kk + 8 * fg);
+    }
+  };
+  if (wrot < nqt) load_qd(wrot);
+  __syncthreads();
+
+  for (int qb0 = wrot; qb0 < nqt; qb0 += NW) {
+    const int q = qb0 * 16 + fq;
+    const int qc = min(q, cnt - 1);
+    if (qb0 != wrot) load_qd(qb0);
+    const float lq = sL[q], dq_ = sD[q];
+    int klen_it = klen;
+    asm volatile("" : "+s"(klen_it));
+    f32x4 dq[Cf::NT];
+#pragma unroll
+    for (int n = 0; n < Cf::NT; ++n) dq[n] = f32x4{0.f, 0.f, 0.f, 0.f};
+    for (int kq = 0; kq < nk; ++kq) {
+      f32x4 scB[2], dpB[2];
+#pragma unroll
+      for (int hf = 0; hf < 2; ++hf) {
+        scB[hf] = f32x4{0.f, 0.f, 0.f, 0.f};
+        dpB[hf] = DROP ? f32x4{0.f, 0.f, 0.f, 0.f} : f32x4{-dq_, -dq_, -dq_, -dq_};
+      }
+#pragma unroll
+      for (int kk = 0; kk < Cf::KK; ++kk) {
+#pragma unroll
+        for (int hf = 0; hf < 2; ++hf) {
+          const int t = 2 * kq + hf;
+          if (!MASK && t >= nt) continue;
+          const bf16x8 kfr = *reinterpret_cast<const bf16x8*>(s0 + t * 16 * Cf::ROWB + r_off[kk]);
+          const bf16x8 vfr = *reinterpret_cast<const bf16x8*>(s1 + t * 16 * Cf::ROWB + r_off[kk]);
+          scB[hf] = __builtin_amdgcn_mfma_f32_16x16x32_bf16(kfr, qf[kk], scB[hf], 0, 0, 0);
+          dpB[hf] = __builtin_amdgcn_mfma_f32_16x16x32_bf16(vfr, df[kk], dpB[hf], 0, 0, 0);
+        }
+      }
+      f32x4 ds2[2];
+#pragma unroll
+      for (int hf = 0; hf < 2; ++hf) {
+        const int t = 2 * kq + hf;
+        if (!MASK && t >= nt) {
+          ds2[hf] = f32x4{0.f, 0.f, 0.f, 0.f};
+          continue;
+        }
+        f32x4 sc = scB[hf];
+        const f32x4 dp = dpB[hf];
+        const unsigned long long* mw = MASK ? mbh + ((size_t)qb0 * nt + min(t, nt - 1)) * 4 : nullptr;
+        if (16 * t + 16 > klen_it) {
+          asm volatile("");
+#pragma unroll
+          for (int r = 0; r < 4; ++r) sc[r] = (16 * t + 4 * fg + r < klen_it) ? sc[r] : kMasked;
+        }
+#pragma unroll
+        for (int r = 0; r < 4; ++r) {
+          const float p = __builtin_amdgcn_exp2f(__builtin_fmaf(sc[r], kLog2e, -lq));
+          if (DROP) {
+            float kfac;
+            asm("v_cndmask_b32_e64 %0, 0, 1.0, %1" : "=v"(kfac) : "s"(mw[r]));
+            ds2[hf][r] = p * __builtin_fmaf(dp[r], kfac, -dq_);
+          } else {
+            ds2[hf][r] = p * dp[r];
+          }
+        }
+      }
+      const bf16x8 sfrag = bf16x8{(bf16)ds2[0][0], (bf16)ds2[0][1], (bf16)ds2[0][2], (bf16)ds2[0][3],
+                                  (bf16)ds2[1][0], (bf16)ds2[1][1], (bf16)ds2[1][2], (bf16)ds2[1][3]};
+#pragma unroll
+      for (int n = 0; n < Cf::NT; ++n) {
+        const char* pk = s0 + kq * 32 * Cf::ROWB + t_off[n];
+        const bf16x8 kT = cat8(lds_tr16(pk), lds_tr16(pk + 16 * Cf::ROWB));
+        dq[n] = __builtin_amdgcn_mfma_f32_16x16x32_bf16(kT, sfrag, dq[n], 0, 0, 0);
+      }
+    }
+    bf16x4 qb4[Cf::NT];
+#pragma unroll
+    for (int n = 0; n < Cf::NT; ++n)
+      qb4[n] = bf16x4{(bf16)(dq[n][0] * qscale), (bf16)(dq[n][1] * qscale), (bf16)(dq[n][2] * qscale), (bf16)(dq[n][3] * qscale)};
+    const bool ok = q < cnt;
+    if (dbias_qkv) {
+#pragma unroll
+      for (int n = 0; n < Cf::NT; ++n) bias_acc(n, ok ? qb4[n] : bf16x4{0, 0, 0, 0});
+    }
+    store_row_widened<Cf::NT>(dQg + (size_t)qc * ld_dq, fg, ok, qb4);
+  }
+
+  if (dbias_qkv) {
+    bias_flush(0);
+    __syncthreads();
+    for (int i = tid; i < 3 * DH; i += NW * 64) {
+      const int part = i / DH, c = i - part * DH;
+      if (part != 1) {
+        float tot = 0.f;
+#pragma unroll
+        for (int w = 0; w < NW; ++w) tot += sB[w * 3 * DH + i];
+        atomicAdd(dbias_qkv + part * dmodel + h * DH + c, tot);
+      }
+    }
+  }
+}
+
+template <int DH, bool QSEL = false>
 int launch_fwd(const bf16* qkv, const int* keylen, bf16* ctx, float* lse, unsigned long long* keepmask, int B, int S, int H,
-               int dmodel, uint32_t seed, uint32_t thresh24, float inv_keep, hipStream_t st) {
+               int dmodel, uint32_t seed, uint32_t thresh24, float inv_keep, hipStream_t st, QSelArgs qs = QSelArgs{}) {
   const int nt = (S + 15) / 16, nk = (S + 31) / 32;
   const size_t lds = (size_t)(nt * 16 + nk * 32) * DH * 2;
   const bool wide = 2 * lds > 160 * 1024;
 #define M3P_ATTN_FWD(KT)                                                                                        \
   do {                                                                                                          \
     constexpr int NW0 = (KT == 16) ? 8 : 4;    \
-    auto kern = thresh24 ? attn_fwd_kernel<DH, KT, true, 0, NW0> : attn_fwd_kernel<DH, KT, false, 0, NW0>;       \
-    if (nt == 11 && KT == 6) kern = thresh24 ? ((S & 1) ? attn_fwd_kernel<DH, 6, true, 11> : attn_fwd_kernel<DH, 6, true, 11, 4, true>) \
-                                             : attn_fwd_kernel<DH, 6, false, 11>; \
-    if (wide) kern = thresh24 ? attn_fwd_kernel<DH, KT, true, 0, 8> : attn_fwd_kernel<DH, KT, false, 0, 8>;       \
+    auto kern = thresh24 ? attn_fwd_kernel<DH, KT, true, 0, NW0, false, QSEL> : attn_fwd_kernel<DH, KT, false, 0, NW0, false, QSEL>;       \
+    if (nt == 11 && KT == 6) kern = thresh24 ? ((S & 1) ? attn_fwd_kernel<DH, 6, true, 11, 4, false, QSEL> : attn_fwd_kernel<DH, 6, true, 11, 4, true, QSEL>) \
+                                             : attn_fwd_kernel<DH, 6, false, 11, 4, false, QSEL>; \
+    if (wide) kern = thresh24 ? attn_fwd_kernel<DH, KT, true, 0, 8, false, QSEL> : attn_fwd_kernel<DH, KT, false, 0, 8, false, QSEL>;       \
     hipError_t e = hipFuncSetAttribute((const void*)kern, hipFuncAttributeMaxDynamicSharedMemorySize, (int)lds); \
     if (e != hipSuccess) return (int)e;                                                                         \
     hipLaunchKernelGGL(kern, dim3(B* H), dim3((wide || NW0 == 8) ? 512 : 256), lds, st, qkv, keylen, ctx, lse, keepmask, S, H, dmodel, seed, \
-                       thresh24, inv_keep);                                                                     \
+                       thresh24, inv_keep, qs);                                                                 \
   } while (0)
   if (nk <= 6) M3P_ATTN_FWD(6);
   else if (nk <= 12) M3P_ATTN_FWD(12);
@@ -1155,9 +1494,68 @@
   return M3P_OK;
 }
 
+template <int DH>
+int launch_qsel_bwd(const bf16* q_c, int ld_q, const bf16* kv, int ld_kv, const int* keylen, const int* seq_start, const bf16* ctx,
+                    const bf16* dctx, const float* lse, const unsigned long long* keepmask, bf16* dq_c, int ld_dq, bf16* dkv,
+                    int ld_dkv, float* dbias, int B, int S, int H, int dmodel, int n_rows, int n_pad, float qscale, uint32_t thresh24,
+                    float inv_keep, hipStream_t st) {
+  const int nk = (S + 31) / 32;
+  const size_t lds = (size_t)2 * nk * 32 * DH * 2 + (size_t)2 * nk * 32 * sizeof(float) + 3 * 4 * DH * sizeof(float);
+  auto kern = thresh24 ? attn_qsel_bwd_kernel<DH, true> : attn_qsel_bwd_kernel<DH, false>;
+  hipError_t e = hipFuncSetAttribute((const void*)kern, hipFuncAttributeMaxDynamicSharedMemorySize, (int)lds);
+  if (e != hipSuccess) return (int)e;
+  hipLaunchKernelGGL(kern, dim3(B * H), dim3(256), lds, st, q_c, ld_q, kv, ld_kv, keylen, seq_start, ctx, dctx, lse, keepmask, dq_c,
+                     ld_dq, dkv, ld_dkv, dbias, B, S, H, dmodel, n_rows, n_pad, qscale, inv_keep);
+  M3P_CHECK_LAUNCH();
+  return M3P_OK;
+}
+
+bool qsel_serves(int B, int S, int H, int dh, int n_rows) {
+  return B > 0 && S > 0 && H > 0 && S <= 512 && n_rows >= 0 && (dh == 64 || dh == 32) &&
+         (unsigned long long)B * H * S * S < (1ull << 32);
+}
+
 }
 
 extern "C" {
+
+int m3p_attn_qsel_fwd(const void* q_c, int ld_q, const void* kv, int ld_kv, const int32_t* keylen, const int32_t* qrow,
+                      const int32_t* seq_start, void* ctx_c, float* lse_c, uint64_t* keepwords, int B, int S, int H, int dh,
+                      int n_rows, uint32_t seed, uint32_t thresh24, float inv_keep, void* stream) {
+  if (!qsel_serves(B, S, H, dh, n_rows)) return M3P_ENOTIMPL;
+  const int dmodel = H * dh;
+  if (((uintptr_t)q_c & 15) || ((uintptr_t)kv & 15) || ((uintptr_t)ctx_c & 15) || (ld_q & 7) || (ld_kv & 7) || ld_q < dmodel ||
+      ld_kv < 2 * dmodel || (thresh24 && !keepwords))
+    return M3P_EINVAL;
+  if (n_rows == 0) return M3P_OK;
+  QSelArgs qs{(const bf16*)kv, qrow, seq_start, ld_q, ld_kv, n_rows, (n_rows + M3P_QSEL_ROW_PAD - 1) / M3P_QSEL_ROW_PAD * M3P_QSEL_ROW_PAD};
+  hipStream_t st = (hipStream_t)stream;
+  if (dh == 64)
+    return launch_fwd<64, true>((const bf16*)q_c, keylen, (bf16*)ctx_c, lse_c, (unsigned long long*)keepwords, B, S, H, dmodel, seed, thresh24, inv_keep, st, qs);
+  return launch_fwd<32, true>((const bf16*)q_c, keylen, (bf16*)ctx_c, lse_c, (unsigned long long*)keepwords, B, S, H, dmodel, seed, thresh24, inv_keep, st, qs);
+}
+
+int m3p_attn_qsel_bwd(const void* q_c, int ld_q, const void* kv, int ld_kv, const int32_t* keylen, const int32_t* qrow,
+                      const int32_t* seq_start, const void* ctx_c, const void* dctx_c, const float* lse_c, const uint64_t* keepwords,
+                      void* dq_c, int ld_dq, void* dkv, int ld_dkv, float* dbias_qkv, int B, int S, int H, int dh, int n_rows,
+                      float qscale, uint32_t thresh24, float inv_keep, void* stream) {
+  (void)qrow;
+  if (!qsel_serves(B, S, H, dh, n_rows)) return M3P_ENOTIMPL;
+  const int dmodel = H * dh;
+  if (((uintptr_t)q_c & 15) || ((uintptr_t)kv & 15) || ((uintptr_t)ctx_c & 15) || ((uintptr_t)dctx_c & 15) || ((uintptr_t)dq_c & 15) ||
+      ((uintptr_t)dkv & 15) || (ld_q & 7) || (ld_kv & 7) || (ld_dq & 7) || (ld_dkv & 7) || ld_q < dmodel || ld_dq < dmodel ||
+      ld_kv < 2 * dmodel || ld_dkv < 2 * dmodel || (thresh24 && !keepwords))
+    return M3P_EINVAL;
+  const int n_pad = (n_rows + M3P_QSEL_ROW_PAD - 1) / M3P_QSEL_ROW_PAD * M3P_QSEL_ROW_PAD;
+  hipStream_t st = (hipStream_t)stream;
+  if (dh == 64)
+    return launch_qsel_bwd<64>((const bf16*)q_c, ld_q, (const bf16*)kv, ld_kv, keylen, seq_start, (const bf16*)ctx_c, (const bf16*)dctx_c, lse_c,
+                               (const unsigned long long*)keepwords, (bf16*)dq_c, ld_dq, (bf16*)dkv, ld_dkv, dbias_qkv, B, S, H, dmodel, n_rows,
+                               n_pad, qscale, thresh24, inv_keep, st);
+  return launch_qsel_bwd<32>((const bf16*)q_c, ld_q, (const bf16*)kv, ld_kv, keylen, seq_start, (const bf16*)ctx_c, (const bf16*)dctx_c, lse_c,
+                             (const unsigned long long*)keepwords, (bf16*)dq_c, ld_dq, (bf16*)dkv, ld_dkv, dbias_qkv, B, S, H, dmodel, n_rows,
+                             n_pad, qscale, thresh24, inv_keep, st);
+}
 
 void m3p_debug_attn_variant(int v) { g_attn_variant = v; }
 
diff --git a/m3p_amd/csrc/heads.hip b/m3p_amd/csrc/heads.hip
--- a/m3p_amd/csrc/heads.hip
+++ b/m3p_amd/csrc/heads.hip
@@ -14,7 +14,8 @@
   }
 }
 __global__ __launch_bounds__(256) void place_rows_kernel(const bf16* __restrict__ src, const int32_t* __restrict__ inv,
-                                                         bf16* __restrict__ dst, int rows, int d, int n, uint32_t fill2) {
+                                                         bf16* __restrict__ dst, int rows, int d, int n, uint32_t fill2,
+                                                         int ld_dst) {
   typedef unsigned int u32x4 __attribute__((ext_vector_type(4)));
   const int nchunk = d >> 3;
   const size_t total = (size_t)rows * nchunk;
@@ -24,7 +25,7 @@
     const int j = inv[r];
     u32x4 v = fv;
     if (j >= 0 && j < n) v = *reinterpret_cast<const u32x4*>(src + (size_t)j * d + 8 * c);
-    *reinterpret_cast<u32x4*>(dst + (size_t)r * d + 8 * c) = v;
+    *reinterpret_cast<u32x4*>(dst + (size_t)r * ld_dst + 8 * c) = v;
   }
 }
 __global__ __launch_bounds__(256) void scatter_add_rows_kernel(const bf16* __restrict__ src, const int32_t* __restrict__ idx,
@@ -620,7 +621,20 @@
   const int blocks = (int)((total + 255) / 256 < 8192 ? (total + 255) / 256 : 8192);
   const uint32_t f = fill_bits & 0xFFFFu;
   hipLaunchKernelGGL(place_rows_kernel, dim3(blocks), dim3(256), 0, (hipStream_t)stream, (const bf16*)src, inv, (bf16*)dst, rows, d, n,
-                     f | (f << 16));
+                     f | (f << 16), d);
+  M3P_CHECK_LAUNCH();
+  return M3P_OK;
+}
+
+int m3p_place_rows_ld(const void* src, const int32_t* inv, void* dst, int ld_dst, int rows, int d, int n, uint32_t fill_bits,
+                      void* stream) {
+  if (rows <= 0) return M3P_OK;
+  if ((d % 8) != 0 || (ld_dst % 8) != 0 || ld_dst < d || ((uintptr_t)src & 15) || ((uintptr_t)dst & 15)) return M3P_EINVAL;
+  const size_t total = (size_t)rows * (d / 8);
+  const int blocks = (int)((total + 255) / 256 < 8192 ? (total + 255) / 256 : 8192);
+  const uint32_t f = fill_bits & 0xFFFFu;
+  hipLaunchKernelGGL(place_rows_kernel, dim3(blocks), dim3(256), 0, (hipStream_t)stream, (const bf16*)src, inv, (bf16*)dst, rows, d, n,
+                     f | (f << 16), ld_dst);
   M3P_CHECK_LAUNCH();
   return M3P_OK;
 }
diff --git a/m3p_amd/functional.py b/m3p_amd/functional.py
--- a/m3p_amd/functional.py
+++ b/m3p_amd/functional.py
@@ -426,6 +426,12 @@
 COMPACT_MIN_ROWS = 4096
 
 
+def _qsel_projection_ok(M, n, d):
+    lib = L.load()
+    plan = lib.m3p_gemm_nt_plan(M, 3 * d, d, L.EPI_BIAS)
+    return plan > 0 and plan == lib.m3p_gemm_nt_plan(M, 2 * d, d, L.EPI_BIAS) == lib.m3p_gemm_nt_plan(n, d, d, L.EPI_BIAS)
+
+
 def compact_rows_eligible(n_rows, M):
     if n_rows <= 0:
         return 0
@@ -435,7 +441,7 @@
 
 class OutputRows:
 
-    def __init__(self, flags):
+    def __init__(self, flags, seq_dims=None):
         flags = torch.as_tensor(flags).reshape(-1).cpu()
         if flags.dtype != torch.bool:
             flags = flags != 0
@@ -445,6 +451,13 @@
         self.n_rows = int(sel.numel())
         self.n = compact_rows_eligible(self.n_rows, self.M)
         self.idx = self.idx64 = self.inv = None
+        self.seq_dims, self.seq_start, self.seq_start_dev = None, None, None
+        if seq_dims is not None:
+            B, S = seq_dims
+            assert B * S == self.M
+            start = torch.zeros(B + 1, dtype=torch.int32)
+            start[1:] = torch.cumsum(flags.view(B, S).sum(dim=1), dim=0).to(torch.int32)
+            self.seq_dims, self.seq_start = (int(B), int(S)), start
         if self.n:
             pad = torch.nonzero(~flags).view(-1)[:self.n - self.n_rows]
             idx = torch.cat([sel, pad]).to(torch.int32)
@@ -461,13 +474,16 @@
             flags[:, R:] |= torch.as_tensor(pred_mask).cpu().reshape(S - R, B).t() != 0
         if region_labels is not None and R > 0:
             flags[:, :R] |= torch.as_tensor(region_labels).cpu().reshape(B, R) != -1
-        return cls(flags)
+        return cls(flags, seq_dims=(B, S))
 
     def to(self, device):
         if self.n and self.idx is None:
             from .utils import to_cuda
             with torch.cuda.device(device):
-                self.idx, self.inv = to_cuda(*self._host)
+                if self.seq_start is not None:
+                    self.idx, self.inv, self.seq_start_dev = to_cuda(*self._host, self.seq_start)
+                else:
+                    self.idx, self.inv = to_cuda(*self._host)
             self.idx64 = self.idx.long()
         assert self.idx is None or self.idx.device == torch.device(device), 'an OutputRows serves one pass on one device'
         return self
@@ -579,16 +595,34 @@
         for i in range(nL):
             a, f = 'attentions.%d.' % i, 'ffns.%d.' % i
             ready(('layer', i))
-            qkv = lin(h, i, 'x', 'wqkv', ar.qkv_w16(i), L.EPI_BIAS, bias=ar.qkv_bias(i), scale_cols=d, scale=qscale)
-            ctxt, lse, kmask = ops.attn_fwd(qkv, totlen, B, S, H, dh, seed=seed('attn_p', i), p_drop=p_attn,
-                                            want_mask=True)
+            compact = rows_c is not None and i == nL - 1
+            qsel = compact and rows_c.seq_start is not None and rows_c.seq_dims == (B, S) and ops.attn_qsel_serves(B, S, H, dh)
+            if qsel:
+                res_c = ops.gather_rows(h, rows_c.idx, rows_c.n, d)
+                wqkv, bqkv = ar.qkv_w16(i), ar.qkv_bias(i)
+                if _qsel_projection_ok(M, rows_c.n, d):
+                    kv = ops.gemm_nt(h, wqkv[d:], L.EPI_BIAS, bias=bqkv[d:])
+                    q_c = ops.gemm_nt(res_c, wqkv[:d], L.EPI_BIAS, bias=bqkv[:d], scale_cols=d, scale=qscale)
+                else:
+                    fused = ops.gemm_nt(h, wqkv, L.EPI_BIAS, bias=bqkv, scale_cols=d, scale=qscale)
+                    q_c, kv = ops.gather_rows(fused, rows_c.idx, rows_c.n, 3 * d)[:, :d], fused[:, d:]
+                ctx_q, lse, kmask = ops.attn_qsel_fwd(q_c, kv, totlen, rows_c.idx, rows_c.seq_start_dev, B, S, H, dh, rows_c.n_rows,
+                                                      seed=seed('attn_p', i), p_drop=p_attn)
+                qkv, ctxt = (q_c, kv, res_c), None
+            else:
+                qkv = lin(h, i, 'x', 'wqkv', ar.qkv_w16(i), L.EPI_BIAS, bias=ar.qkv_bias(i), scale_cols=d, scale=qscale)
+                ctxt, lse, kmask = ops.attn_fwd(qkv, totlen, B, S, H, dh, seed=seed('attn_p', i), p_drop=p_attn,
+                                                want_mask=True)
             lse = (lse, kmask)
-            compact = rows_c is not None and i == nL - 1
             Mi, ctx_in, res_in, mask_i, rr, ctx_c = M, ctxt, h, rowmask, {}, None
             if compact:
                 Mi, rr = rows_c.n, dict(rng_rows=rows_c.idx)
-                ctx_in = ctx_c = ops.gather_rows(ctxt, rows_c.idx, Mi, d)
-                res_in = ops.gather_rows(h, rows_c.idx, Mi, d)
+                if qsel:
+                    ctx_in = ctx_c = ctx_q
+                    res_in = res_c
+                else:
+                    ctx_in = ctx_c = ops.gather_rows(ctxt, rows_c.idx, Mi, d)
+                    res_in = ops.gather_rows(h, rows_c.idx, Mi, d)
                 mask_i = rowmask[rows_c.idx64]
             pre1 = lin(ctx_in, i, 'ctx', 'wout', ar.w(a + 'out_lin.weight'), L.EPI_BIAS_DROP_RES, bias=ar.p(a + 'out_lin.bias'),
                        aux=res_in, seed=seed('attn_out', i), p_drop=p_drop, **rr)
@@ -734,6 +768,23 @@
             if dAO is None:
                 dAO = dpre1
             dctx = dgrad(dAO, i, 'dao', 'wout', ar.wt[('out', i)], L.EPI_NONE)
+            if compact and isinstance(qkv, tuple):
+                q_c, kv, res_c = qkv
+                dqkv = torch.empty((M, 3 * d), dtype=BF16, device=dctx.device)
+                dq_c, _ = ops.attn_qsel_bwd(q_c, kv, totlen, rows_c.idx, rows_c.seq_start_dev, ctx_c, dctx, lse[0], B, S, H, dh,
+                                            rows_c.n_rows, dbias_qkv=ar.qkv_bias(i, grad=True), p_drop=p_attn, keepwords=lse[1],
+                                            dkv_out=dqkv[:, d:])
+                ops.place_rows_into(dq_c, rows_c.inv, dqkv[:, :d], 0)
+                gw = ar.qkv_wgrad(i)
+                ops.gemm_wgrad_pair(dq_c, res_c, gw[:d], dAO, ctx_c, ar.g(a + 'out_lin.weight'))
+                ops.gemm_wgrad(dqkv[:, d:], h_in, gw[d:])
+                dpre1 = ops.place_rows(dpre1, rows_c.inv, M, 0)
+                dh_ = dgrad(dqkv, i, 'dqkv', 'wqkv', ar.wt[('qkv', i)], L.EPI_RES, aux=dpre1)
+                del dq_c, dqkv, q_c, kv, res_c, qkv, dctx, dAO, dpre1, dx1
+                ar.touch_layer(i)
+                if hook is not None:
+                    hook.layer_done(i, last)
+                continue
             if compact:
                 ops.gemm_wgrad(dAO, ctx_c, ar.g(a + 'out_lin.weight'))
                 dctx = ops.place_rows(dctx, rows_c.inv, M, 0)
diff --git a/m3p_amd/lib.py b/m3p_amd/lib.py
--- a/m3p_amd/lib.py
+++ b/m3p_amd/lib.py
@@ -47,6 +47,8 @@
     'm3p_layernorm_bwd_rows': (_i, [_p, _p, _p, _p, _p, _p, _p, _p, _p, _p, _p, _p, _i, _i, _u32, _u32, _f, _p, _p]),
     'm3p_attn_fwd': (_i, [_p, _p, _p, _p, _p, _i, _i, _i, _i, _u32, _u32, _f, _p]),
     'm3p_attn_bwd': (_i, [_p, _p, _p, _p, _p, _p, _p, _p, _i, _i, _i, _i, _f, _u32, _u32, _f, _p]),
+    'm3p_attn_qsel_fwd': (_i, [_p, _i, _p, _i, _p, _p, _p, _p, _p, _p, _i, _i, _i, _i, _i, _u32, _u32, _f, _p]),
+    'm3p_attn_qsel_bwd': (_i, [_p, _i, _p, _i, _p, _p, _p, _p, _p, _p, _p, _p, _i, _p, _i, _p, _i, _i, _i, _i, _i, _f, _u32, _f, _p]),
     'm3p_attn_query_fwd': (_i, [_p, _i, _p, C.c_longlong, _i, _p, _p, _i, _i, _i, _i, _i, _i, _i, _p]),
     'm3p_attn_rows_fwd': (_i, [_p, _i, _p, C.c_longlong, _i, _p, _p, _p, _i, _i, _i, _i, _i, _i, _i, _u32, _u32, _f, _p]),
     'm3p_attn_rows_bwd': (_i, [_p, _i, _p, C.c_longlong, _i, _p, _p, _p, _p, _i, _p, _i, _i, _i, _i, _i, _i, _i, _f, _u32, _u32, _f, _p]),
@@ -61,6 +63,7 @@
     'm3p_glu_bwd': (_i, [_p, _i, _p, _p, _i, _i, _p]),
     'm3p_gather_rows': (_i, [_p, _p, _p, _i, _i, _p]),
     'm3p_place_rows': (_i, [_p, _p, _p, _i, _i, _i, _u32, _p]),
+    'm3p_place_rows_ld': (_i, [_p, _p, _p, _i, _i, _i, _i, _u32, _p]),
     'm3p_scatter_add_rows': (_i, [_p, _p, _p, _i, _i, _p]),
     'm3p_scatter_add_token_rows': (_i, [_p, _i, _p, _p, _i, _i, _i, _p]),
     'm3p_ce_fwd_bwd': (_i, [_p, _i, _i, _i, _p, _p, _p, _f, _f, _p]),
diff --git a/m3p_amd/ops.py b/m3p_amd/ops.py
--- a/m3p_amd/ops.py
+++ b/m3p_amd/ops.py
@@ -295,6 +295,61 @@
     return dqkv
 
 
+QSEL_ROW_PAD = 256
+
+
+def _qsel_check(q_c, kv, qrow, seq_start, B, S, H, dh, n_rows):
+    d = H * dh
+    n = (n_rows + QSEL_ROW_PAD - 1) // QSEL_ROW_PAD * QSEL_ROW_PAD
+    _chk_bf16(q_c, kv)
+    assert q_c.shape == (n, d) and q_c.stride(1) == 1 and kv.shape == (B * S, 2 * d) and kv.stride(1) == 1
+    assert qrow.dtype == torch.int32 and qrow.is_cuda and qrow.is_contiguous() and qrow.numel() >= n_rows
+    assert seq_start.dtype == torch.int32 and seq_start.is_cuda and seq_start.is_contiguous() and seq_start.numel() == B + 1
+    return n, d
+
+
+def attn_qsel_serves(B, S, H, dh):
+    return dh in (32, 64) and 0 < S <= 512 and B > 0 and H > 0 and B * H * S * S < (1 << 32)
+
+
+def attn_qsel_fwd(q_c, kv, keylen, qrow, seq_start, B, S, H, dh, n_rows, seed=0, p_drop=0.0):
+    n, d = _qsel_check(q_c, kv, qrow, seq_start, B, S, H, dh, n_rows)
+    assert keylen.dtype == torch.int32
+    ctx_c = torch.empty((n, d), dtype=BF16, device=q_c.device)
+    lse_c = torch.empty((H, n), dtype=torch.float32, device=q_c.device)
+    words = None
+    if p_drop > 0:
+        words = torch.empty((H * (n_rows // 16 + B) * ((S + 15) // 16) * 4,), dtype=torch.int64, device=q_c.device)
+    e0 = _prof_begin(('attn_qsel_fwd', n_rows, S, H * dh))
+    rc = L.load().m3p_attn_qsel_fwd(q_c.data_ptr(), q_c.stride(0), kv.data_ptr(), kv.stride(0), keylen.data_ptr(), qrow.data_ptr(),
+                                    seq_start.data_ptr(), ctx_c.data_ptr(), lse_c.data_ptr(), L.ptr(words), B, S, H, dh, n_rows,
+                                    seed, L.thresh24(p_drop), 1.0 / (1.0 - p_drop) if p_drop > 0 else 1.0, L.stream())
+    L.check(rc, 'm3p_attn_qsel_fwd')
+    _prof_end(e0, ('attn_qsel_fwd', n_rows, S, H * dh))
+    return ctx_c, lse_c, words
+
+
+def attn_qsel_bwd(q_c, kv, keylen, qrow, seq_start, ctx_c, dctx_c, lse_c, B, S, H, dh, n_rows, dbias_qkv=None, p_drop=0.0,
+                  keepwords=None, dkv_out=None):
+    n, d = _qsel_check(q_c, kv, qrow, seq_start, B, S, H, dh, n_rows)
+    _chk_bf16(ctx_c, dctx_c)
+    assert ctx_c.is_contiguous() and dctx_c.is_contiguous() and ctx_c.shape == (n, d) and dctx_c.shape == (n, d)
+    assert lse_c.dtype == torch.float32 and lse_c.is_contiguous() and lse_c.shape == (H, n)
+    assert p_drop == 0 or keepwords is not None, 'attention backward with dropout needs the keep words of the forward pass'
+    dq_c = torch.empty((n, d), dtype=BF16, device=q_c.device)
+    dkv = dkv_out if dkv_out is not None else torch.empty((B * S, 2 * d), dtype=BF16, device=q_c.device)
+    assert dkv.dtype == BF16 and dkv.shape == (B * S, 2 * d) and dkv.stride(1) == 1
+    e0 = _prof_begin(('attn_qsel_bwd', n_rows, S, H * dh))
+    rc = L.load().m3p_attn_qsel_bwd(q_c.data_ptr(), q_c.stride(0), kv.data_ptr(), kv.stride(0), keylen.data_ptr(), qrow.data_ptr(),
+                                    seq_start.data_ptr(), ctx_c.data_ptr(), dctx_c.data_ptr(), lse_c.data_ptr(), L.ptr(keepwords),
+                                    dq_c.data_ptr(), dq_c.stride(0), dkv.data_ptr(), dkv.stride(0), L.ptr(dbias_qkv), B, S, H, dh,
+                                    n_rows, 1.0 / (dh ** 0.5), L.thresh24(p_drop), 1.0 / (1.0 - p_drop) if p_drop > 0 else 1.0,
+                                    L.stream())
+    L.check(rc, 'm3p_attn_qsel_bwd')
+    _prof_end(e0, ('attn_qsel_bwd', n_rows, S, H * dh))
+    return dq_c, dkv
+
+
 def attn_query_fwd(q, kv, klen, B, Tq, H, dh, Lk, causal=False, pos0=0):
     _chk_bf16(q, kv)
     assert q.stride(1) == 1 and kv.dim() == 3 and kv.stride(2) == 1 and kv.shape[0] == B and kv.shape[1] >= Lk
@@ -567,6 +622,17 @@
     return out
 
 
+def place_rows_into(src, inv, out, fill_bits=0):
+    _chk_bf16(src, out)
+    n, d = src.shape
+    rows = out.shape[0]
+    assert src.is_contiguous() and out.shape[1] == d and out.stride(1) == 1
+    assert inv.dtype == torch.int32 and inv.is_cuda and inv.is_contiguous() and inv.numel() == rows
+    L.check(L.load().m3p_place_rows_ld(src.data_ptr(), inv.data_ptr(), out.data_ptr(), out.stride(0), rows, d, n, int(fill_bits),
+                                       L.stream()), 'm3p_place_rows_ld')
+    return out
+
+
 def scatter_add_rows(src, idx, dst_base, n, d):
     L.check(L.load().m3p_scatter_add_rows(src.data_ptr(), idx.data_ptr(), dst_base.data_ptr(), n, d, L.stream()),
             'm3p_scatter_add_rows')
```

Measured after the change: 8120 sequences/s, median of 5. Within noise of the previous version (-0.0%).
